# davawen/Simple-Raytracer

Hardware: AMD Instinct MI355X
Metric: Mray/s at 1920x1080x1024spp (higher is better)
Workload: dtype f32; 1 GPU; BASELINE configs[1]: 7-shape sphere scene 1920x1080 1024spp; width=1920, height=1080, spp=1024, bounces=10, triangles=12, partition=single GPU, gather=none, mode=parity (fp-contract off, IEEE div/sqrt; canvas bit-identical to the CPU oracle)

## Files before the change

include/srt_abi.h:

```cpp
#ifndef SRT_ABI_H
#define SRT_ABI_H

#include "srt_types.h"

#ifdef __cplusplus
extern "C" {
#endif

typedef struct srt_tracer srt_tracer;

enum {
	SRT_OK = 0,
	SRT_ERR_INVALID = 1,
	SRT_ERR_HIP = 2,
	SRT_ERR_STATE = 3
};

typedef struct srt_counters {
	uint64_t paths;
	uint64_t rays;
	uint64_t sky;
	uint64_t tri_tests;
	uint64_t tri_pass_u;
	uint64_t nan_pixels;
// ... 142 lines not shown
int srt_group_reset_denoise_history(srt_group *g);
int srt_group_resolve_denoised(srt_group *g, uint32_t ticks_stopped);
int srt_group_read_denoised(srt_group *g, float *rgba_out);
int srt_group_read_denoise_inputs(srt_group *g, float *normal_depth, float *albedo_hits, float *moments, uint32_t counts[2]);
int srt_group_read_denoise_history(srt_group *g, float *colour_count, float *moments, float *guide, srt_render_data *camera, int *valid);


int srt_render_pipelined(srt_tracer *t, const srt_render_data *options, uint32_t ticks_stopped, uint8_t *argb_out,
                         long long *frame_delivered);
int srt_pipeline_flush(srt_tracer *t, uint8_t *argb_out, long long *frame_delivered);



int srt_denoise_defaults(srt_denoise_params *out);
int srt_set_denoise(srt_tracer *t, const srt_denoise_params *params);
int srt_resolve_denoised(srt_tracer *t, uint32_t ticks_stopped);
int srt_read_denoised(srt_tracer *t, float *rgba_out);
int srt_read_denoise_inputs(srt_tracer *t, float *normal_depth, float *albedo_hits, float *moments, uint32_t counts[2]);



int srt_temporal_defaults(srt_temporal_params *out);
int srt_set_denoise_temporal(srt_tracer *t, const srt_temporal_params *params);
int srt_reset_denoise_history(srt_tracer *t);
int srt_read_denoise_history(srt_tracer *t, float *colour_count, float *moments, float *guide, srt_render_data *camera, int *valid);


enum { SRT_MOTION_STATIC = 0, SRT_MOTION_MOVED = 1, SRT_MOTION_NO_HISTORY = 2 };
#define SRT_MOTION_WORDS 22

int srt_set_denoise_object_motion(srt_tracer *t, int enable);
int srt_read_denoise_shape_ids(srt_tracer *t, uint32_t *current, uint32_t *history);
int srt_read_denoise_motion(srt_tracer *t, uint32_t *table, size_t capacity_shapes, size_t *n_shapes, int *any_moved);
int srt_motion_table_host(const srt_shape *h_shapes, size_t h_n_shapes, const srt_triangle *h_triangles, size_t h_n_triangles,
                          const srt_material *h_materials, size_t h_n_materials, const srt_scene_data *h_scene,
                          const srt_shape *c_shapes, size_t c_n_shapes, const srt_triangle *c_triangles, size_t c_n_triangles,
                          const srt_material *c_materials, size_t c_n_materials, const srt_scene_data *c_scene, uint32_t *table, int *keep);


enum { SRT_MOTION_DEFORMED = 3 };

int srt_set_denoise_vertex_motion(srt_tracer *t, int enable);
int srt_read_denoise_triangle_ids(srt_tracer *t, uint32_t *current, uint32_t *history);
int srt_read_denoise_vertex_tables(srt_tracer *t, float *current, float *history, size_t cap_rows, size_t *n_rows);
int srt_motion_table_deform_host(const srt_shape *h_shapes, size_t h_n_shapes, const srt_triangle *h_triangles, size_t h_n_triangles,
                                 const srt_material *h_materials, size_t h_n_materials, const srt_scene_data *h_scene,
                                 const srt_shape *c_shapes, size_t c_n_shapes, const srt_triangle *c_triangles, size_t c_n_triangles,
                                 const srt_material *c_materials, size_t c_n_materials, const srt_scene_data *c_scene, uint32_t *table, int *keep);


#define SRT_DEMOD_EPS 0.01f
int srt_set_denoise_demodulation(srt_tracer *t, int enable);
int srt_group_set_denoise_demodulation(srt_group *g, int enable);
int srt_last_filter_demodulated(const srt_tracer *t, int *demodulated);
int srt_group_last_filter_demodulated(const srt_group *g, int *demodulated);


int srt_set_denoise_spatial_variance(srt_tracer *t, uint32_t min_samples);
int srt_group_set_denoise_spatial_variance(srt_group *g, uint32_t min_samples);
int srt_last_filter_spatial_variance(const srt_tracer *t, int *ran);
int srt_group_last_filter_spatial_variance(const srt_group *g, int *ran);


int srt_set_denoise_history_illumination(srt_tracer *t, int enable);
int srt_group_set_denoise_history_illumination(srt_group *g, int enable);
int srt_last_setup_history_illumination(srt_tracer *t);
int srt_group_last_setup_history_illumination(srt_group *g);


int srt_set_denoise_history_clamp(srt_tracer *t, float gamma);
int srt_group_set_denoise_history_clamp(srt_group *g, float gamma);
int srt_last_setup_history_clamp(srt_tracer *t);
int srt_group_last_setup_history_clamp(srt_group *g);
int srt_read_denoise_history_bounds(srt_tracer *t, float *mean_weight, float *sigma_taps);


int srt_set_textures(srt_tracer *t, const srt_texture_desc *descs, size_t n);
int srt_set_material_textures(srt_tracer *t, const srt_material_texture *bindings, size_t n_materials);
int srt_set_triangle_uvs(srt_tracer *t, const float *uv, size_t n_triangles);
int srt_set_triangle_materials(srt_tracer *t, const int32_t *materials, size_t n_triangles);
int srt_triangle_materials_check_host(const int32_t *materials, size_t n, size_t scene_triangles, size_t n_materials);
int srt_last_trace_textured(const srt_tracer *t, int *textured);
int srt_last_trace_class(const srt_tracer *t, int *scene_class);
int srt_bernoulli_threshold_host(float p, uint64_t *threshold);
int srt_plane_frame_host(const float normal[3], float T[3], float B[3]);
int srt_texture_check_host(const srt_texture_desc *descs, size_t n_textures, const srt_material_texture *bindings, size_t n_bindings,
                           long long uv_triangles, size_t scene_triangles);

int srt_selftest_math(srt_tracer *t, uint32_t stride, uint64_t out[16]);

int srt_selftest_rare_lanes(srt_tracer *t, int what, const uint32_t *in, uint32_t waves, uint32_t *out_new, uint32_t *out_ref, uint64_t *mismatches);

const char *srt_version(void);

#ifdef __cplusplus
}
#endif

#endif
```

simple-raytracer_amd/csrc/device_intersect.h:

```cpp
#ifndef SRT_DEVICE_INTERSECT_H
#define SRT_DEVICE_INTERSECT_H

#include "device_math.h"
#include "trace_regions.h"

namespace {

#define SRT_AS_CONST __attribute__((address_space(4)))
struct Blk16 {
	float v[16];
};
struct Tri2 {
	float v[18];
};
template <int N, int ALIGN>
__device__ __forceinline__ void ld_uniform(const float *p, float (&out)[N]) {
	const SRT_AS_CONST float *c = (const SRT_AS_CONST float *)__builtin_assume_aligned(p, ALIGN);
#pragma unroll
	for (int i = 0; i < N; i++) out[i] = c[i];
}
__device__ __forceinline__ Blk16 ld_blk16(const float *p) {
	Blk16 b;
	ld_uniform<16, 64>(p, b.v);
	return b;
// ... 40 lines not shown
		for (int i = 0; i < N; i++) dd[i] = disc[i];
		sqrt_rsq_n<N, false>(dd, sq);
#pragma unroll
		for (int i = 0; i < N; i++) {
			const uint32_t k = min(dm_f2u(bq[i] - sq[i]), dm_f2u(bq[i] + sq[i]));
			take_if_closer(dm_u2f(k), idx0 + i, tmin, best);
		}
	}
}

__device__ __forceinline__ void test_planes2(const Blk16 &b, uint32_t count, f3 org, f3 dir, int idx0, float &tmin, int &best) {
#pragma unroll
	for (int i = 0; i < 2; i++) {
		if (i == 1 && count < 2u) break;
		f3 n = mk(b.v[8 * i + 4], b.v[8 * i + 5], b.v[8 * i + 6]);
		float denom = dot3(n, dir);
		float t = dot3(n, mk(b.v[8 * i] - org.x, b.v[8 * i + 1] - org.y, b.v[8 * i + 2] - org.z)) / denom;
		bool hit = !(t < 0.0f);
		if (hit && t < tmin) {
			tmin = t;
			best = idx0 + i;
		}
	}
}

template <int N>
__device__ __forceinline__ void test_spheres_cam(const float4 *__restrict__ cam, f3 dir, unsigned long long actm, int idx0, float &tmin, int &best) {
	float bq[4], disc[4];
	bool slow = is_neg_zero(tmin);
#pragma unroll
	for (int i = 0; i < N; i++) {
		const float4 lc = cam[i];
		bq[i] = dot3(mk(lc.x, lc.y, lc.z), dir);
		disc[i] = bq[i] * bq[i] - lc.w;
		slow = slow || dm_fabs(disc[i]) < 0x1p-96f;
	}
	if (__builtin_expect(any64(slow), 0)) {
#pragma unroll
		for (int i = 0; i < N; i++) {
			const float sq = __builtin_sqrtf(disc[i]);
			float t = bq[i] - sq;
			if (t < 0.0f) t = bq[i] + sq;
			if (!(disc[i] < 0.0f) && !(t < 0.0f) && t < tmin) tmin = t, best = idx0 + i;
		}
	} else {
#pragma unroll
		for (int i = 0; i < N; i++) {
			if ((ballot64(disc[i] >= 0.0f) & actm) != 0ull) {
				const float sq = sqrt_rsq(disc[i]);
				const uint32_t k = min(dm_f2u(bq[i] - sq), dm_f2u(bq[i] + sq));
				take_if_closer(dm_u2f(k), idx0 + i, tmin, best);
			}
		}
	}
}
__device__ __forceinline__ void test_planes2_cam(const float4 *__restrict__ blk, uint32_t count, f3 dir, int idx0, float &tmin, int &best) {
#pragma unroll
	for (int i = 0; i < 2; i++) {
		if (i == 1 && count < 2u) break;
		const float4 nq = blk[2 * i + 1];
		const float num = reinterpret_cast<const float *>(blk + 2 * i)[3];
		const float denom = dot3(mk(nq.x, nq.y, nq.z), dir);
		const float t = num / denom;
		const bool hit = !(t < 0.0f);
		if (hit && t < tmin) {
			tmin = t;
			best = idx0 + i;
		}
	}
}
template <uint32_t K>
__device__ __forceinline__ void cam_records_of_block(float4 *__restrict__ blk, float4 *__restrict__ cam, f3 org, int lane) {
	if constexpr ((K & 3u) == SRT_SHAPE_SPHERE + 1u) {
		if (lane < 4) {
			const float4 s = blk[lane];
			const f3 L = mk(s.x - org.x, s.y - org.y, s.z - org.z);
			const float c = dot3(L, L) - s.w;
			cam[lane] = make_float4(L.x, L.y, L.z, c);
		}
	} else if constexpr ((K & 3u) == SRT_SHAPE_PLANE + 1u) {
		if (lane < 2) {
			const float4 pq = blk[2 * lane], nq = blk[2 * lane + 1];
			reinterpret_cast<float *>(blk + 2 * lane)[3] = dot3(mk(nq.x, nq.y, nq.z), mk(pq.x - org.x, pq.y - org.y, pq.z - org.z));
		}
	}
}
__device__ __forceinline__ bool test_aabb(float lx, float ly, float lz, float hx, float hy, float hz, f3 org, f3 inv, float tmax) {
	float t0 = 0.0f, t1 = tmax;
	float a1 = (lx - org.x) * inv.x, a2 = (hx - org.x) * inv.x;
	t0 = dm_max(t0, dm_min(a1, a2));
	t1 = dm_min(t1, dm_max(a1, a2));
	a1 = (ly - org.y) * inv.y, a2 = (hy - org.y) * inv.y;
	t0 = dm_max(t0, dm_min(a1, a2));
	t1 = dm_min(t1, dm_max(a1, a2));
	a1 = (lz - org.z) * inv.z, a2 = (hz - org.z) * inv.z;
	t0 = dm_max(t0, dm_min(a1, a2));
	t1 = dm_min(t1, dm_max(a1, a2));
	return t0 < t1;
}

template <bool COUNT_TRIS>
__device__ __forceinline__ bool moller_trumbore(float v0x, float v0y, float v0z, float e1x, float e1y, float e1z, float e2x, float e2y,
                                                float e2z, f3 org, f3 dir, bool counted, float &t, uint32_t &n_tri_u SRT_RC_PARAM) {
	f3 e1 = mk(e1x, e1y, e1z), e2 = mk(e2x, e2y, e2z);
	f3 h = cross3(dir, e2);
	float a = dot3(e1, h);
	f3 sv = mk(org.x - v0x, org.y - v0y, org.z - v0z);
	float sh = dot3(sv, h);
	float aa = dm_fabs(a), ash = dm_fabs(sh);
	bool reject = (a == 0.0f) || (ash > aa * 1.001f) || ((sh * a < 0.0f) && (ash >= aa * 0.001f));
	bool ok = false;
	if (!reject) {
		SRT_REGION(EXTEND_TRI_EXACT);
		f3 q = cross3(sv, e1);
		float dv = dot3(dir, q);
		bool reject2 = false;
		if (!COUNT_TRIS) reject2 = ((dv * a < 0.0f) && (dm_fabs(dv) >= aa * 0.001f)) || (dm_fabs(sh + dv) > aa * 1.01f);
		if (!reject2) {
			SRT_REGION(EXTEND_TRI_DIV);
			float f = 1.0f / a;
			float u = f * sh;
			ok = !(u < 0.0f || u > 1.0f);
			if (COUNT_TRIS) n_tri_u += (ok && counted) ? 1u : 0u;
			float v = f * dv;
			ok = ok && !(v < 0.0f || u + v > 1.0f);
			t = f * dot3(e2, q);
			ok = ok && t > 0.0f;
		}
	}
	return ok;
}

template <bool COUNT_TRIS>
__device__ __forceinline__ void test_triangle(float v0x, float v0y, float v0z, float e1x, float e1y, float e1z, float e2x, float e2y,
                                              float e2z, f3 org, f3 dir, int idx, uint32_t j, uint32_t count, float &tmin, int &best,
                                              uint32_t &best_tri, uint32_t &n_tri_u SRT_RC_PARAM) {
	float t = 0.0f;
	if (moller_trumbore<COUNT_TRIS>(v0x, v0y, v0z, e1x, e1y, e1z, e2x, e2y, e2z, org, dir, j < count, t, n_tri_u SRT_RC_ARG) && t < tmin) {
		tmin = t;
		best = idx;
		best_tri = j;
	}
}


template <bool COUNT_TRIS>
__device__ __forceinline__ void test_pair(const Tri2 &t, f3 org, f3 dir, int idx, uint32_t j, uint32_t count, float &tmin, int &best,
                                          uint32_t &best_tri, uint32_t &n_tri_u SRT_RC_PARAM) {
	test_triangle<COUNT_TRIS>(t.v[0], t.v[1], t.v[2], t.v[3], t.v[4], t.v[5], t.v[6], t.v[7], t.v[8], org, dir, idx, j, count, tmin, best, best_tri,
	                          n_tri_u SRT_RC_ARG);
	test_triangle<COUNT_TRIS>(t.v[9], t.v[10], t.v[11], t.v[12], t.v[13], t.v[14], t.v[15], t.v[16], t.v[17], org, dir, idx, j + 1u, count, tmin,
	                          best, best_tri, n_tri_u SRT_RC_ARG);
}

template <bool COUNT_TRIS>
__device__ __forceinline__ void test_triangles(const float *__restrict__ wtris, uint32_t first, uint32_t count, f3 org, f3 dir, int idx,
                                               float &tmin, int &best, uint32_t &best_tri, uint32_t &n_tri_u SRT_RC_PARAM) {
	const float *__restrict__ blk = wtris + (size_t)first * SRT_WTRI_FLOATS;
	const uint32_t npair = ((count + 3u) >> 2) << 1;
	Tri2 a = ld_tri2(blk);
	for (uint32_t b = 0; b < npair; b += 2) {
		SRT_REGION(EXTEND_TRI_LOOP);
		const Tri2 c = ld_tri2(blk + 18u * (b + 1u));
		test_pair<COUNT_TRIS>(a, org, dir, idx, 2u * b, count, tmin, best, best_tri, n_tri_u SRT_RC_ARG);
		a = ld_tri2(blk + 18u * (b + 2u));
		test_pair<COUNT_TRIS>(c, org, dir, idx, 2u * b + 2u, count, tmin, best, best_tri, n_tri_u SRT_RC_ARG);
// ... 131 lines not shown
```

simple-raytracer_amd/csrc/device_types.h:

```cpp
#ifndef SRT_DEVICE_TYPES_H
#define SRT_DEVICE_TYPES_H

#include <stddef.h>
#include <stdint.h>

#include "../../include/srt_types.h"

struct ShapeRun {
	int32_t type;
	uint32_t first_shape;
	uint32_t count;
	uint32_t data_off;
};
struct BlockGroup {
	uint32_t code;
	uint32_t first[3];
};
static_assert(sizeof(BlockGroup) == 16, "BlockGroup 16 B");

struct WinnerRec {
	int32_t type;
	int32_t material;
	float vx, vy, vz, w;
	uint32_t first_wtri;
	float inv_w;
};
static_assert(sizeof(WinnerRec) == 32, "WinnerRec 32 B");

#define SRT_WTRI_FLOATS 9

typedef srt_bvh_node BvhNode;
#define SRT_BVH_FIRST_DWORD 11
#define SRT_BVH_TRI_FLOATS 9
#define SRT_BVH_LEAF_J 28
#define SRT_BVH_NONE 0xffffffffu
#define SRT_BVH_LEAF_BIT 0x80000000u
#define SRT_BVH_INDEX_MASK 0x0fffffffu
#define SRT_BVH_INDEX_MAX 0x01ffffffu
#define SRT_BVH_KEY_INF 0x7f800000u
#define SRT_BVH_TAG_MASK 31u
#define SRT_BVH_TAG_LEAF 16u
#define SRT_BVH_TAG(ref, slot) ((((ref) >> 31) << 4) | ((((ref) >> 28) & 3u) << 2) | (slot))
#define SRT_BVH_STACK_CAP 64
#ifndef SRT_BVH_LEAF_MAX
#define SRT_BVH_LEAF_MAX 3
#endif

#define SRT_REGION_MAX 56
#ifdef SRT_REGION_COUNT
#define SRT_WAVE_CTR_STRIDE (16 + 2 * SRT_REGION_MAX)
#else
#define SRT_WAVE_CTR_STRIDE 16
#endif
#define SRT_WAVE_CTR_SLOTS 8192

enum { SRT_CTR_RAYS = 0, SRT_CTR_SKY, SRT_CTR_TRI, SRT_CTR_TRI_PASS_U, SRT_CTR_NAN, SRT_CTR_PATHS, SRT_CTR_QUEUE, SRT_CTR_WATCHDOG, SRT_CTR_QUEUE2, SRT_CTR_COUNT };

#define SRT_MF_NO_SPECULAR 1
#define SRT_MF_PLAIN_COLORS 2

#define SRT_BLK_CODE(type, count) ((uint32_t)((type) + 1) | ((uint32_t)(count) << 2))
#define SRT_GROUP_CODE(b0, b1, b2) ((b0) | ((b1) << 8) | ((b2) << 16))
#define SRT_GC_PPS SRT_GROUP_CODE(SRT_BLK_CODE(SRT_SHAPE_PLANE, 2), SRT_BLK_CODE(SRT_SHAPE_PLANE, 1), SRT_BLK_CODE(SRT_SHAPE_SPHERE, 4))
#define SRT_GC_SSS SRT_GROUP_CODE(SRT_BLK_CODE(SRT_SHAPE_SPHERE, 4), SRT_BLK_CODE(SRT_SHAPE_SPHERE, 4), SRT_BLK_CODE(SRT_SHAPE_SPHERE, 4))
#define SRT_GC_PPP SRT_GROUP_CODE(SRT_BLK_CODE(SRT_SHAPE_PLANE, 2), SRT_BLK_CODE(SRT_SHAPE_PLANE, 2), SRT_BLK_CODE(SRT_SHAPE_PLANE, 2))
#define SRT_SCENE_CLASS_LIST(X) \
	X(1, SRT_GC_PPS, true)      \
	X(2, SRT_GC_PPS, false)     \
	X(3, SRT_GC_SSS, true)      \
	X(4, SRT_GC_PPP, true)
#define SRT_SCENE_CLASS_GENERAL 0
static constexpr inline uint32_t srt_class_cam_records(uint32_t code) {
	return ((code & 3u) == SRT_SHAPE_SPHERE + 1u ? 4u : 0u) + (((code >> 8) & 3u) == SRT_SHAPE_SPHERE + 1u ? 4u : 0u) +
	       (((code >> 16) & 3u) == SRT_SHAPE_SPHERE + 1u ? 4u : 0u);
}
static constexpr inline size_t srt_class_cam_lds_bytes(uint32_t code) { return 16u * (size_t)srt_class_cam_records(code); }

static inline size_t srt_scene_lds_bytes(size_t num_shapes, size_t num_materials, int num_models, size_t num_runs) {
	size_t scene = num_shapes * sizeof(WinnerRec) + num_materials * sizeof(srt_material);
	if (num_models == 0) scene += num_runs * (sizeof(BlockGroup) + 192);
	return scene <= 4608 ? scene : 0;
}

struct TraceParams {
	srt_render_data rd;
	srt_scene_data sd;
	const BlockGroup *runs;
	const float *run_data;
	const WinnerRec *winners;
	int32_t num_runs;
	int32_t num_materials;
	uint32_t lds_bytes;
	int32_t scene_class;
	const srt_shape *shapes;
	const srt_triangle *triangles;
	const srt_material *materials;
	const float *wtris;
	const float *sky;
	float *canvas;
	float *radiance;
	unsigned long long *counters;
	unsigned long long *wave_counters;
	unsigned long long *queue;
	unsigned long long total_items;
	uint32_t batch_samples;
	uint32_t first_sample;
	uint32_t job_items;
	uint32_t stage_off;
	int32_t sky_w, sky_h;
	float f_width, f_height, f_sky_w, f_sky_h;
	int32_t sun_focus_int;
	int32_t material_flags;
	int32_t num_models;
	int32_t rank, world, rows_per_block, owned_rows;
	int32_t use_bvh;
	const float *bvh_blocks;
	float *scan_queue;
	float inv_f_width, inv_f_height;
	uint32_t width_magic, width_shift;
	uint32_t rpb_magic, rpb_shift;
	uint32_t nbs_magic16;
	uint32_t pool_blocks;
	int32_t unit_materials;
	int32_t all_materials_ok;
};

static inline void srt_magic_u31(uint32_t d, uint32_t *magic, uint32_t *shift) {
	uint32_t l = 0;
	while (l < 32 && ((uint64_t)1 << l) < d) l++;
	*shift = l;
	*magic = (uint32_t)((((uint64_t)1 << 32) * (((uint64_t)1 << l) - d)) / d + 1);
}

struct PrepassParams {
	const srt_shape *shapes;
	const srt_triangle *triangles;
	const uint32_t *wtri_offset;
	float *wtris;
	int32_t num_shapes;
	uint32_t num_triangles;
	const uint32_t *order;
	const uint32_t *dest;
};

struct ReduceParams {
	const float *radiance;
	float *running;
	float *canvas;
	unsigned long long *counters;
	uint32_t num_pixels;
	uint32_t batch_samples;
	int32_t num_samples;
	uint32_t first_batch, last_batch;
	unsigned long long *queue_reset;
// ... 52 lines not shown
void srt_launch_features_ids_tex(const TexFeatureParams &p, uint32_t *shape_ids, void *stream);
void srt_launch_features_tris_tex(const TexFeatureParams &p, uint32_t *shape_ids, uint32_t *tri_ids, void *stream);

void srt_launch_trace(TraceParams p, bool count_triangles, int num_waves, void *stream);
void srt_launch_reduce(const ReduceParams &p, void *stream);
void srt_launch_reduce_moments(const ReduceParams &p, void *stream);
void srt_launch_features(const FeatureParams &p, void *stream);
void srt_launch_features_ids(const FeatureParams &p, uint32_t *shape_ids, void *stream);
void srt_launch_features_tris(const FeatureParams &p, uint32_t *shape_ids, uint32_t *tri_ids, void *stream);
int srt_trace_waves_per_simd(int has_models, int use_bvh);
int srt_trace_has_scene_classes();
int srt_trace_resident_waves_per_cu(const TraceParams &p, bool count_triangles);
int srt_scan_suspend_min(void);
int srt_sub_job_items(int has_models, int use_bvh);
#define SRT_SQ_CAP 192
#define SRT_PK_CAP 256
#define SRT_SCAN_QUEUE_FLOATS (2 * 20 * SRT_SQ_CAP + 15 * SRT_PK_CAP)
#define SRT_POOL_BLOCKS 8192
#define SRT_POOL_CTL_WORDS (16 + 2 * SRT_POOL_BLOCKS)
#define SRT_POOL_REC_FLOATS ((size_t)2 * SRT_POOL_BLOCKS * 20 * 64)
#define SRT_SCAN_SET_FLOATS(waves, pool) ((size_t)SRT_POOL_CTL_WORDS + ((pool) ? SRT_POOL_REC_FLOATS : (size_t)0) + (size_t)(waves) * SRT_SCAN_QUEUE_FLOATS)
void srt_launch_prepass(const PrepassParams &p, uint64_t total_wtris, void *stream);

struct RefitModel {
	uint32_t shape;
	uint32_t first_record;
	uint32_t num_records;
	uint32_t first_tile;
};
struct RefitCostRange {
	uint32_t first_block, num_blocks;
};
struct RefitParams {
	const srt_shape *shapes;
	const srt_triangle *triangles;
	const uint32_t *order, *dest;
	const RefitModel *models;
	uint32_t *extents;
	float *boxes;
	uint32_t *blocks;
	const uint32_t *sched;
};
#define SRT_REFIT_EXT_LO_INIT 0xff7fffffu
#define SRT_REFIT_EXT_HI_INIT 0x00800000u
int srt_launch_refit_extents(const RefitParams &p, uint32_t num_models, uint32_t max_records, void *stream);
int srt_launch_refit_leaves(const RefitParams &p, uint32_t num_models, uint32_t max_records, void *stream);
int srt_launch_refit_level(const RefitParams &p, uint32_t first, uint32_t count, void *stream);
int srt_launch_refit_cost(const float *boxes, const uint8_t *weights, const RefitCostRange *ranges, double *sums, uint32_t num_models, uint32_t max_blocks, void *stream);
#define SRT_BUILD_TILE 1024u
#define SRT_BUILD_SORT_PASSES 4
struct BuildParams {
	const srt_shape *shapes;
	const srt_triangle *triangles;
	const RefitModel *models;
	const uint32_t *extents;
	uint32_t *keys[2];
	uint32_t *vals[2];
	uint32_t *table;
	uint32_t *order;
	const uint32_t *range_first;
	uint32_t *ranges;
};
#define SRT_BUILD_TILES(records) (((uint32_t)(records) + SRT_BUILD_TILE - 1u) / SRT_BUILD_TILE)
int srt_launch_build_keys(const BuildParams &p, uint32_t num_models, uint32_t max_records, void *stream);
int srt_launch_build_sort(const BuildParams &p, uint32_t num_models, uint32_t max_records, void *stream);
#define SRT_BUILD_LOCAL 1024u
#define SRT_BUILD_MEDIAN_MAX_LEVELS 15u
#define SRT_BUILD_MEDIAN_KEY_BITS 17u
#ifdef __HIPCC__
#define SRT_BUILD_HD __host__ __device__
#else
#define SRT_BUILD_HD
#endif
static inline SRT_BUILD_HD uint32_t srt_build_median_levels(uint32_t n) {
	uint32_t levels = 0;
	while (levels <= SRT_BUILD_MEDIAN_MAX_LEVELS && n > (SRT_BUILD_LOCAL << levels)) levels++;
	return levels;
}
static inline SRT_BUILD_HD uint32_t srt_build_median_passes(uint32_t level) { return (SRT_BUILD_MEDIAN_KEY_BITS + level + 7u) / 8u; }
int srt_launch_build_median(const BuildParams &p, uint32_t num_models, uint32_t max_records, void *stream);
void srt_launch_resolve(const ResolveParams &p, void *stream);
void srt_launch_selftest(unsigned long long *out16, uint32_t stride, void *stream);
void srt_launch_selftest_rare(int what, const uint32_t *in, uint32_t waves, uint32_t *out_new, uint32_t *out_ref, unsigned long long *mismatches, void *stream);

#endif
```

simple-raytracer_amd/csrc/kernels.hip:

```cpp
#include <hip/hip_runtime.h>

#include "detmath.h"
#include "device_types.h"
#include "device_math.h"
#include "device_intersect.h"
#include "device_shading.h"

#if SRT_TEXTURED
#define SRT_TRACE_PARAMS TexTraceParams
#define SRT_FEATURE_PARAMS TexFeatureParams
#define srt_trace_kernel srt_trace_tex_kernel
#define srt_features_kernel srt_features_tex_kernel
#define srt_features_ids_kernel srt_features_ids_tex_kernel
#define srt_features_tris_kernel srt_features_tris_tex_kernel
#define srt_launch_trace srt_launch_trace_tex
#define srt_trace_resident_waves_per_cu srt_trace_tex_resident_waves_per_cu
#define srt_launch_features srt_launch_features_tex
#define srt_launch_features_ids srt_launch_features_ids_tex
#define srt_launch_features_tris srt_launch_features_tris_tex
int srt_trace_lds_floats(int has_models, int use_bvh);
#else
#define SRT_TRACE_PARAMS TraceParams
#define SRT_FEATURE_PARAMS FeatureParams
#endif
// ... 12 lines not shown
#endif
#ifndef SRT_HQ_CAP
#define SRT_HQ_CAP 64
#endif
#ifndef SRT_HQ_CAP_MODELS
#define SRT_HQ_CAP_MODELS 64
#endif
#ifndef SRT_SCAN_SUSPEND_MIN
#define SRT_SCAN_SUSPEND_MIN 128
#endif
#ifndef SRT_SCAN_FULL
#define SRT_SCAN_FULL 64
#endif
#ifndef SRT_HQ_CAP_BVH
#define SRT_HQ_CAP_BVH 64
#endif
#ifndef SRT_RING_CAP
#define SRT_RING_CAP 64
#endif
#ifndef SRT_REFILL_MIN
#define SRT_REFILL_MIN 32
#endif

#ifdef SRT_PHASE_CLOCK
#define SRT_CLK_DECL unsigned long long clk_t[8] = {0, 0, 0, 0, 0, 0, 0, 0}, clk_last = __builtin_amdgcn_s_memtime(), clk_start = clk_last
#define SRT_CLK(i)                                                  \
	do {                                                            \
		const unsigned long long now_ = __builtin_amdgcn_s_memtime(); \
		clk_t[i] += now_ - clk_last;                                \
		clk_last = now_;                                            \
	} while (0)
#else
#define SRT_CLK_DECL
#define SRT_CLK(i)
#endif

namespace {
__device__ __forceinline__ void store_radiance(float *__restrict__ radiance, uint32_t item, f3 c) {
	typedef float f3v __attribute__((ext_vector_type(3)));
	f3v v;
	v.x = c.x, v.y = c.y, v.z = c.z;
	float *g = radiance + 3ull * item;
	asm volatile("global_store_dwordx3 %0, %1, off sc1" : : "v"(g), "v"(v) : "memory");
}

__device__ __forceinline__ bool in_mask(unsigned long long m) { return __builtin_amdgcn_inverse_ballot_w64(m); }
__device__ __forceinline__ uint32_t popc64(unsigned long long m) { return (uint32_t)__builtin_popcountll(m); }
__device__ __forceinline__ uint32_t lane_rank(unsigned long long m) {
	return __builtin_amdgcn_mbcnt_hi((uint32_t)(m >> 32), __builtin_amdgcn_mbcnt_lo((uint32_t)m, 0u));
}
__device__ __forceinline__ unsigned long long lanes_below(uint32_t n) { return n >= 64u ? ~0ull : ((1ull << n) - 1ull); }

__device__ __forceinline__ void resolve_ring(const TraceParams &p, const float *__restrict__ ring, uint32_t n, int lane SRT_RC_PARAM) {
	asm volatile("s_waitcnt lgkmcnt(0)" ::: "memory");
	if ((uint32_t)lane < n) {
		SRT_REGION(SKY_RESOLVE);
		constexpr uint32_t RC = SRT_RING_CAP;
		const f3 d = mk(ring[0 * RC + lane], ring[1 * RC + lane], ring[2 * RC + lane]);
		f3 m = mk(ring[3 * RC + lane], ring[4 * RC + lane], ring[5 * RC + lane]);
		f3 c = mk(ring[6 * RC + lane], ring[7 * RC + lane], ring[8 * RC + lane]);
		const uint32_t item = dm_f2u(ring[9 * RC + lane]);
		m = m * sky_box(p, d);
		c = c + m;
		store_radiance(p.radiance, item, c);
	}
	asm volatile("" ::: "memory");
}
}

#ifndef SRT_TRACE_WAVES_PER_SIMD
#define SRT_TRACE_WAVES_PER_SIMD 5
#endif
#ifndef SRT_TRACE_WAVES_PER_SIMD_MODELS
#define SRT_TRACE_WAVES_PER_SIMD_MODELS 5
#endif
#ifndef SRT_TRACE_WAVES_PER_SIMD_BVH
#define SRT_TRACE_WAVES_PER_SIMD_BVH 5
#endif

constexpr uint32_t hq_fields(bool has_models) { return has_models ? 17u : 16u; }

struct GeneralScene {
	static constexpr bool FAST = false, NO_SPEC = false;
	static constexpr uint32_t CODE = 0;
};
template <uint32_t CODE_, bool NO_SPEC_>
struct OneGroupScene {
	static constexpr bool FAST = true, NO_SPEC = NO_SPEC_;
	static constexpr uint32_t CODE = CODE_;
};
template <uint32_t K>
__device__ __forceinline__ void test_block_of_class(const Blk16 &b, int base, f3 org, f3 dir, float &tmin, int &best) {
	if constexpr ((K & 3u) == SRT_SHAPE_SPHERE + 1u) {
		if constexpr (((K >> 2) & 7u) <= 2u) test_spheres<2>(b, org, dir, base, tmin, best);
		else test_spheres<4>(b, org, dir, base, tmin, best);
	} else if constexpr ((K & 3u) == SRT_SHAPE_PLANE + 1u) {
		test_planes2(b, (K >> 2) & 7u, org, dir, base, tmin, best);
	}
}
template <uint32_t K>
__device__ __forceinline__ void test_block_of_class_cam(const float4 *__restrict__ blk, const float4 *__restrict__ cam, int base, f3 dir, unsigned long long actm, float &tmin, int &best) {
	if constexpr ((K & 3u) == SRT_SHAPE_SPHERE + 1u) {
		if constexpr (((K >> 2) & 7u) <= 2u) test_spheres_cam<2>(cam, dir, actm, base, tmin, best);
		else test_spheres_cam<4>(cam, dir, actm, base, tmin, best);
	} else if constexpr ((K & 3u) == SRT_SHAPE_PLANE + 1u) {
		test_planes2_cam(blk, (K >> 2) & 7u, dir, base, tmin, best);
	}
}

template <bool COUNT_TRIS, bool USE_LDS, bool HAS_MODELS, bool USE_BVH>
__global__ __launch_bounds__(64, USE_BVH ? SRT_TRACE_WAVES_PER_SIMD_BVH : HAS_MODELS ? SRT_TRACE_WAVES_PER_SIMD_MODELS : SRT_TRACE_WAVES_PER_SIMD) void srt_trace_kernel(const SRT_TRACE_PARAMS p) {
	using SC = GeneralScene;
#include "trace_body.inc"
}

#if !SRT_TEXTURED && !SRT_DIAG_ON && !defined(SRT_DUMMY_KIND) && !defined(SRT_DEV_KNOBS) && SRT_RING_CAP == 64
#define SRT_SCENE_CLASSES 1
template <uint32_t CODE, bool NO_SPEC>
__global__ __launch_bounds__(64, 6) void srt_trace_scene_kernel(const TraceParams p) {
	constexpr bool COUNT_TRIS = false, USE_LDS = true, HAS_MODELS = false, USE_BVH = false;
	using SC = OneGroupScene<CODE, NO_SPEC>;
#include "trace_body.inc"
}
#else
#define SRT_SCENE_CLASSES 0
#endif

template <bool HAS_MODELS, bool USE_BVH>
__global__ __launch_bounds__(64) void srt_features_kernel(const SRT_FEATURE_PARAMS fp) {
#define SRT_FEATURES_IDS 0
#include "features_body.inc"
#undef SRT_FEATURES_IDS
}

template <bool HAS_MODELS, bool USE_BVH>
__global__ __launch_bounds__(64) void srt_features_ids_kernel(const SRT_FEATURE_PARAMS fp, uint32_t *__restrict__ shape_ids) {
#define SRT_FEATURES_IDS 1
#include "features_body.inc"
#undef SRT_FEATURES_IDS
}

template <bool HAS_MODELS, bool USE_BVH>
__global__ __launch_bounds__(64) void srt_features_tris_kernel(const SRT_FEATURE_PARAMS fp, uint32_t *__restrict__ shape_ids, uint32_t *__restrict__ tri_ids) {
#define SRT_FEATURES_IDS 2
#include "features_body.inc"
#undef SRT_FEATURES_IDS
}

#if !SRT_TEXTURED
int srt_trace_waves_per_simd(int has_models, int use_bvh) {
	return !has_models ? SRT_TRACE_WAVES_PER_SIMD : use_bvh ? SRT_TRACE_WAVES_PER_SIMD_BVH : SRT_TRACE_WAVES_PER_SIMD_MODELS;
}
int srt_scan_suspend_min(void) { return SRT_SCAN_SUSPEND_MIN; }
int srt_sub_job_items(int has_models, int use_bvh) { return !has_models ? SRT_SUB_PLAIN : use_bvh ? SRT_SUB_BVH : SRT_SUB_MODELS; }

int srt_trace_lds_floats(int has_models, int use_bvh) {
	int n = 10 * SRT_RING_CAP + (int)hq_fields(has_models) * (has_models ? (use_bvh ? SRT_HQ_CAP_BVH : SRT_HQ_CAP_MODELS) : SRT_HQ_CAP);
#ifdef SRT_REGION_COUNT
	n += 2 * SRT_REGION_MAX;
#endif
	return n;
}
int srt_trace_has_scene_classes() { return SRT_SCENE_CLASSES; }
#endif

namespace {
typedef void (*TraceKernel)(const SRT_TRACE_PARAMS);
TraceKernel pick_trace_kernel(bool models, bool use_bvh, bool use_lds, bool count_triangles) {
	if (!models) return use_lds ? srt_trace_kernel<false, true, false, false> : srt_trace_kernel<false, false, false, false>;
	if (use_bvh) {
		if (use_lds) return count_triangles ? srt_trace_kernel<true, true, true, true> : srt_trace_kernel<false, true, true, true>;
		return count_triangles ? srt_trace_kernel<true, false, true, true> : srt_trace_kernel<false, false, true, true>;
	}
	if (use_lds) return count_triangles ? srt_trace_kernel<true, true, true, false> : srt_trace_kernel<false, true, true, false>;
	return count_triangles ? srt_trace_kernel<true, false, true, false> : srt_trace_kernel<false, false, true, false>;
}
size_t scene_lds_bytes(const TraceParams &p) {
	return srt_scene_lds_bytes((size_t)p.sd.num_shapes, (size_t)p.num_materials, p.num_models, (size_t)p.num_runs);
}
TraceKernel pick_trace_kernel(const SRT_TRACE_PARAMS &p, bool use_lds, bool count_triangles) {
#if SRT_SCENE_CLASSES
	switch (p.scene_class) {
#define SRT_SCENE_CLASS_CASE(number, code, no_spec) \
	case number: return srt_trace_scene_kernel<code, no_spec>;
		SRT_SCENE_CLASS_LIST(SRT_SCENE_CLASS_CASE)
#undef SRT_SCENE_CLASS_CASE
	default: break;
	}
#endif
	return pick_trace_kernel(p.num_models > 0, p.use_bvh != 0, use_lds, count_triangles);
}
size_t trace_lds_bytes(const SRT_TRACE_PARAMS &p, size_t scene_lds) {
	size_t need = scene_lds + (size_t)srt_trace_lds_floats(p.num_models > 0, p.use_bvh) * sizeof(float);
#if SRT_SCENE_CLASSES
	switch (p.scene_class) {
#define SRT_SCENE_CLASS_CASE(number, code, no_spec) \
	case number: need += srt_class_cam_lds_bytes(code); break;
		SRT_SCENE_CLASS_LIST(SRT_SCENE_CLASS_CASE)
#undef SRT_SCENE_CLASS_CASE
	default: break;
	}
#endif
	return need;
}
}

int srt_trace_resident_waves_per_cu(const SRT_TRACE_PARAMS &p, bool count_triangles) {
	const size_t scene_lds = scene_lds_bytes(p);
	const size_t need = trace_lds_bytes(p, scene_lds);
	int blocks = 0;
	if (hipOccupancyMaxActiveBlocksPerMultiprocessor(&blocks, pick_trace_kernel(p, scene_lds != 0, count_triangles), 64, need) != hipSuccess ||
	    blocks <= 0) {
		(void)hipGetLastError();
		blocks = 4 * srt_trace_waves_per_simd(p.num_models > 0, p.use_bvh);
	}
	return blocks;
}

void srt_launch_trace(SRT_TRACE_PARAMS p, bool count_triangles, int num_waves, void *stream) {
	if (p.total_items == 0 || num_waves <= 0) return;
	dim3 grid((unsigned)num_waves), block(64);
	const size_t scene_lds = scene_lds_bytes(p);
	p.lds_bytes = (uint32_t)scene_lds;
	p.stage_off = (uint32_t)(scene_lds / sizeof(float4));
	const size_t need = trace_lds_bytes(p, scene_lds);
	hipLaunchKernelGGL(pick_trace_kernel(p, scene_lds != 0, count_triangles), grid, block, need, (hipStream_t)stream, p);
}

void srt_launch_features(const SRT_FEATURE_PARAMS &p, void *stream) {
	if (p.num_pixels == 0 || p.feature_samples == 0) return;
	typedef void (*FeatureKernel)(const SRT_FEATURE_PARAMS);
	const bool models = p.tp.num_models > 0, bvh = p.tp.use_bvh != 0;
	const FeatureKernel k = !models ? srt_features_kernel<false, false> : bvh ? srt_features_kernel<true, true> : srt_features_kernel<true, false>;
	hipLaunchKernelGGL(k, dim3((p.num_pixels + 63u) / 64u), dim3(64), 0, (hipStream_t)stream, p);
}

void srt_launch_features_ids(const SRT_FEATURE_PARAMS &p, uint32_t *shape_ids, void *stream) {
	if (p.num_pixels == 0 || p.feature_samples == 0) return;
	typedef void (*FeatureKernel)(const SRT_FEATURE_PARAMS, uint32_t *);
	const bool models = p.tp.num_models > 0, bvh = p.tp.use_bvh != 0;
	const FeatureKernel k = !models ? srt_features_ids_kernel<false, false> : bvh ? srt_features_ids_kernel<true, true> : srt_features_ids_kernel<true, false>;
	hipLaunchKernelGGL(k, dim3((p.num_pixels + 63u) / 64u), dim3(64), 0, (hipStream_t)stream, p, shape_ids);
}

void srt_launch_features_tris(const SRT_FEATURE_PARAMS &p, uint32_t *shape_ids, uint32_t *tri_ids, void *stream) {
	if (p.num_pixels == 0 || p.feature_samples == 0) return;
	typedef void (*FeatureKernel)(const SRT_FEATURE_PARAMS, uint32_t *, uint32_t *);
	const bool models = p.tp.num_models > 0, bvh = p.tp.use_bvh != 0;
	const FeatureKernel k = !models ? srt_features_tris_kernel<false, false> : bvh ? srt_features_tris_kernel<true, true> : srt_features_tris_kernel<true, false>;
	hipLaunchKernelGGL(k, dim3((p.num_pixels + 63u) / 64u), dim3(64), 0, (hipStream_t)stream, p, shape_ids, tri_ids);
}
```

simple-raytracer_amd/csrc/scene_prep.cpp:

```cpp
#include "scene_prep.h"

#include <algorithm>
#include <chrono>
#include <cmath>
#include <cstdio>
#include <cstring>
#include <deque>
#include <utility>

uint64_t bernoulli_threshold(float pr) {
	uint64_t lo = 0, hi = (uint64_t)1 << 32;
	while (lo < hi) {
		const uint64_t mid = (lo + hi) >> 1;
		const float u = (float)(uint32_t)mid * 2.3283064365386963e-10f;
		if (pr > u) lo = mid + 1;
		else hi = mid;
	}
	return lo;
}

int prepare_scene(const AccelPolicy &policy, BvhCache *&cache, int scan_suspend_min, std::string &err, ScenePrep &sp, const srt_shape *shapes, size_t n_shapes,
                  const srt_triangle *triangles, size_t n_triangles, const srt_material *materials, size_t n_materials, const srt_scene_data *scene) {
	auto fail = [&err](int code, const char *msg) {
		err = msg;
		return code;
	};
	if (!scene) return fail(SRT_ERR_INVALID, "srt_update_scene: scene is NULL");
	if ((n_shapes && !shapes) || (n_triangles && !triangles) || (n_materials && !materials))
		return fail(SRT_ERR_INVALID, "srt_update_scene: NULL array with non-zero count");
	if (n_shapes > 0x7fffffffu || n_triangles > 0xffffffffu) return fail(SRT_ERR_INVALID, "srt_update_scene: too many records");

	std::vector<ShapeRun> runs;
	std::vector<float> &data = sp.data;
	std::vector<WinnerRec> &winners = sp.winners;
	winners.assign(n_shapes ? n_shapes : 1, WinnerRec());
	std::vector<uint32_t> &offs = sp.offs;
	offs.assign(n_shapes ? n_shapes : 1, 0u);
	uint64_t &total_wtris = sp.total_wtris, &max_tris = sp.max_tris;
	int &num_models = sp.num_models;
	const bool use_bvh = sp.use_bvh = policy.accel == SRT_ACCEL_BVH;
	std::vector<uint32_t> &bvh_blocks = sp.bvh_blocks;
	std::vector<uint32_t> &bvh_order = sp.bvh_order, &bvh_dest = sp.bvh_dest;
	uint64_t bvh_leaves = 0, bvh_depth = 0, bvh_reused = 0, bvh_refitted = 0, bvh_canonical_nodes = 0;
	std::deque<BvhCacheEntry> fresh;
	std::vector<std::pair<bool, size_t>> plan;
	std::vector<std::pair<uint64_t, uint64_t>> range_hashes;
	std::vector<std::pair<const BvhCacheEntry *, uint32_t>> stale_plan;
	if (use_bvh && !cache) cache = new BvhCache();
	if (cache)
		for (BvhCacheEntry &e : cache->entries) e.claimed = false;
	if (!use_bvh && cache) cache->entries.clear();
	const auto build_t0 = std::chrono::steady_clock::now();
	auto range_hash = [&](const srt_model &m) {
		for (const auto &rh : range_hashes)
			if (rh.first == (((uint64_t)m.triangle_index << 32) | m.num_triangles)) return rh.second;
		const uint64_t th = hash_triangles(triangles + m.triangle_index, m.num_triangles);
		range_hashes.emplace_back(((uint64_t)m.triangle_index << 32) | m.num_triangles, th);
		return th;
	};
	auto find_same_triangles = [&](const srt_model &m, uint64_t th) {
		BvhCacheEntry *kept = nullptr;
		for (BvhCacheEntry &e : cache->entries) {
			if (e.claimed || e.count != m.num_triangles || e.tri_hash != th) continue;
			const bool exact = e.same_transform(m);
			if (!exact && kept) continue;
			if (!e.same_triangles(m, triangles, th)) continue;
			kept = &e;
			if (exact) break;
		}
		return kept;
	};
	const bool deform_on = use_bvh && policy.deform.mode == SRT_DEFORM_REFIT;
	struct Match {
		BvhCacheEntry *ent = nullptr;
		bool deformed = false;
	};
	std::vector<Match> matched;
	uint64_t deform_kept = 0, deform_rebuilt = 0;
	if (deform_on) {
		matched.assign(n_shapes, Match());
		auto wants_entry = [&](size_t i) {
			const srt_model &m = shapes[i].shape.model;
			return shapes[i].type == SRT_SHAPE_MODEL && m.num_triangles > 0 && (uint64_t)m.triangle_index + m.num_triangles <= n_triangles;
		};
		for (size_t i = 0; i < n_shapes; i++) {
			if (!wants_entry(i)) continue;
			const srt_model &m = shapes[i].shape.model;
			if ((matched[i].ent = find_same_triangles(m, range_hash(m)))) matched[i].ent->claimed = true;
		}
		for (size_t i = 0; i < n_shapes; i++) {
			if (!wants_entry(i) || matched[i].ent) continue;
			const srt_model &m = shapes[i].shape.model;
			BvhCacheEntry *kept = nullptr;
			for (BvhCacheEntry &e : cache->entries) {
				if (e.claimed || e.count != m.num_triangles || e.triangle_index != m.triangle_index) continue;
				if (!kept || e.same_transform(m)) kept = &e;
				if (e.same_transform(m)) break;
			}
			if (kept) kept->claimed = true, matched[i].ent = kept, matched[i].deformed = true;
		}
	}
// ... 89 lines not shown
						memcpy(ent->transform, m.transform, sizeof ent->transform);
						bvh_refitted++;
					}
					plan.emplace_back(true, (size_t)(kept - cache->entries.data()));
				} else {
					fresh.emplace_back();
					ent = &fresh.back();
					device_built = policy.build.mode == SRT_BUILD_DEVICE && m.num_triangles >= policy.build.min_triangles;
					if (device_built) *ent = cache->balanced_topology(m.num_triangles);
					else ent->build(m, triangles);
					ent->count = m.num_triangles;
					ent->triangle_index = m.triangle_index;
					ent->tri_hash = th;
					memcpy(ent->transform, m.transform, sizeof ent->transform);
					ent->tris.assign(triangles + m.triangle_index, triangles + m.triangle_index + m.num_triangles);
					plan.emplace_back(false, fresh.size() - 1);
				}
				const uint32_t b0 = (uint32_t)(bvh_blocks.size() / 32), r0 = (uint32_t)total_wtris;
				const BvhBuilder::Wide &wd = ent->wide;
				if ((uint64_t)b0 + wd.blocks.size() / 32 > SRT_BVH_INDEX_MAX) return fail(SRT_ERR_INVALID, "srt_update_scene: too many BVH blocks");
				if (wd.need > SRT_BVH_STACK_CAP) return fail(SRT_ERR_INVALID, "srt_update_scene: BVH deeper than the walk's stack");
				bvh_blocks.insert(bvh_blocks.end(), wd.blocks.begin(), wd.blocks.end());
				for (uint32_t ib : wd.inner) bvh_blocks[32 * (size_t)(b0 + ib) + SRT_BVH_FIRST_DWORD] += b0;
				bvh_dest.resize(r0 + (size_t)m.num_triangles);
				for (uint32_t r = 0; r < m.num_triangles; r++) bvh_dest[r0 + r] = wd.dest[r] + (b0 << 2);
				bvh_canonical_nodes += ent->nodes.size();
				bvh_order.insert(bvh_order.end(), ent->order.begin(), ent->order.end());
				link = wd.root == SRT_BVH_NONE ? SRT_BVH_NONE : wd.root + b0;
				if (ent->stale) {
					ent->wide.ensure_schedule();
					sp.refit_models.push_back({(uint32_t)i, r0, m.num_triangles, 0u});
					stale_plan.emplace_back(ent, b0);
					if (m.num_triangles > sp.refit_max_records) sp.refit_max_records = m.num_triangles;
					if (device_built) {
						sp.build_models.push_back({(uint32_t)i, r0, m.num_triangles, sp.build_tiles});
						sp.build_tiles += SRT_BUILD_TILES(m.num_triangles);
						sp.build_entry.push_back(plan.size() - 1);
						if (m.num_triangles > sp.build_max_records) sp.build_max_records = m.num_triangles;
					}
					if (deform_on) {
						const uint32_t nb = (uint32_t)(wd.blocks.size() / 32);
						sp.refit_cost_ranges.push_back({b0, nb});
						sp.refit_cost_entry.push_back(plan.size() - 1);
						sp.refit_cost_built.push_back(ent->cost_built);
						sp.refit_cost_fresh.push_back(device_built ? 1 : 0);
						sp.refit_weights.resize((size_t)b0 + nb, 0);
						for (const BvhBuilder::Wide::Job &j : wd.jobs) sp.refit_weights[b0 + j.self] = (uint8_t)j.nk;
						for (uint32_t d : wd.dest) sp.refit_weights[b0 + (d >> 2)]++;
					}
				} else if (deform_on) {
					sp.deform_worst_ratio = std::max(sp.deform_worst_ratio, BvhBuilder::cost_ratio(ent->cost_now, ent->cost_built));
				}
				bvh_leaves += ent->leaves;
				if (ent->depth > bvh_depth) bvh_depth = ent->depth;
			}
			data.insert(data.end(), {m.bounding_min.x, m.bounding_min.y, m.bounding_min.z, u2f(link), m.bounding_max.x, m.bounding_max.y,
			                         m.bounding_max.z, u2f(use_bvh ? 0u : m.num_triangles)});
			wr.first_wtri = (uint32_t)total_wtris;
			offs[i] = (uint32_t)total_wtris;
			total_wtris += use_bvh ? (uint64_t)m.num_triangles : (((uint64_t)m.num_triangles + 3u) & ~3ull);
			if (m.num_triangles > max_tris) max_tris = m.num_triangles;
			num_models++;
		}
	}
	pad_run();
	std::vector<BlockGroup> &groups = sp.groups;
	groups.assign((runs.size() + 2) / 3, BlockGroup());
	uint32_t n_big = 0;
	for (size_t b = 0; b < runs.size(); b++) {
		BlockGroup &g = groups[b / 3];
		if (b % 3 == 0) memset(&g, 0, sizeof g);
		const uint32_t big = runs[b].data_off >> 31;
		g.code |= (((uint32_t)runs[b].type + 1u) | (runs[b].count << 2) | (big << 5) | ((big ? (n_big++ & 1u) : 0u) << 6)) << (8 * (b % 3));
		g.first[b % 3] = runs[b].first_shape;
	}
	data.resize(groups.size() * 48 + 16, 0.0f);
	sp.one_group_code = 0;
	if (groups.size() == 1 && num_models == 0) {
		uint32_t next = 0;
		bool packed = true;
		for (size_t b = 0; b < runs.size(); b++) packed = packed && runs[b].first_shape == next, next += runs[b].count;
		if (packed && next == n_shapes) sp.one_group_code = groups[0].code;
	}
	if (!stale_plan.empty()) {
		size_t top = 0;
		for (const auto &st : stale_plan) top = std::max(top, st.first->wide.level_off.size());
		sp.refit_levels.assign(1, 0u);
		for (size_t h = 1; h < top; h++) {
			for (const auto &st : stale_plan) {
				const BvhBuilder::Wide &wd = st.first->wide;
				if (h >= wd.level_off.size()) continue;
				for (uint32_t k = wd.level_off[h - 1]; k < wd.level_off[h]; k++) sp.refit_sched.push_back(wd.sched[k] + st.second);
			}
			sp.refit_levels.push_back((uint32_t)sp.refit_sched.size());
		}
		for (size_t k = 0; k < sp.build_models.size(); k++)
			sp.build_extents.insert(sp.build_extents.end(), {SRT_REFIT_EXT_LO_INIT, SRT_REFIT_EXT_LO_INIT, SRT_REFIT_EXT_LO_INIT, SRT_REFIT_EXT_HI_INIT, SRT_REFIT_EXT_HI_INIT, SRT_REFIT_EXT_HI_INIT});
		for (size_t k = 0; k < stale_plan.size(); k++)
			sp.refit_extents.insert(sp.refit_extents.end(), {SRT_REFIT_EXT_LO_INIT, SRT_REFIT_EXT_LO_INIT, SRT_REFIT_EXT_LO_INIT, SRT_REFIT_EXT_HI_INIT, SRT_REFIT_EXT_HI_INIT, SRT_REFIT_EXT_HI_INIT});
	}
	const uint64_t build_us =
	    (uint64_t)std::chrono::duration_cast<std::chrono::microseconds>(std::chrono::steady_clock::now() - build_t0).count();

	std::vector<srt_material> &dev_mats = sp.dev_mats;
	dev_mats.assign(materials, materials + n_materials);
	auto schlick_r0 = [](float mu) {
		float r0 = (float)((1.0 - (double)mu) / (1.0 + (double)mu));
		return r0 * r0;
	};
	bool unit_materials = true;
	for (const auto &m : dev_mats)
		if (bernoulli_threshold(m.metallic) >> 32 || bernoulli_threshold(m.specular) >> 32 || bernoulli_threshold(m.transmittance) >> 32) unit_materials = false;
	sp.unit_materials = unit_materials;
	{
		bool no_specular = unit_materials, plain = true;
		for (const auto &m : dev_mats) {
			if (bernoulli_threshold(m.specular) != 0) no_specular = false;
			for (float c : {m.color.x, m.color.y, m.color.z})
				if (!std::isfinite(c) || (c == 0.0f && std::signbit(c))) plain = false;
		}
		sp.material_flags = (no_specular ? SRT_MF_NO_SPECULAR : 0) | (plain ? SRT_MF_PLAIN_COLORS : 0);
	}
	for (auto &m : dev_mats) {
		if (unit_materials) {
			const uint32_t tm = (uint32_t)bernoulli_threshold(m.metallic), ts = (uint32_t)bernoulli_threshold(m.specular), tt = (uint32_t)bernoulli_threshold(m.transmittance);
			memcpy(&m.metallic, &tm, 4), memcpy(&m.specular, &ts, 4), memcpy(&m.transmittance, &tt, 4);
		}
		const float inv_ior = 1.0f / m.refraction_index;
		m._pad[0] = inv_ior;
		m._pad[1] = schlick_r0(inv_ior);
		m.color._pad = schlick_r0(m.refraction_index);
	}
	sp.bvh_info[0] = bvh_canonical_nodes, sp.bvh_info[1] = bvh_leaves, sp.bvh_info[2] = bvh_depth, sp.bvh_info[3] = use_bvh ? build_us : 0;
	sp.bvh_info[4] = use_bvh ? plan.size() - bvh_reused - bvh_refitted : 0, sp.bvh_info[5] = bvh_reused, sp.bvh_info[6] = bvh_refitted;
	sp.deform_info[0] = deform_kept, sp.deform_info[1] = deform_rebuilt;
	if (deform_on) sp.refit_weights.resize(bvh_blocks.size() / 32, 0);
	if (use_bvh) {
		std::vector<BvhCacheEntry> next_cache;
		next_cache.reserve(plan.size());
		for (const auto &pl : plan) next_cache.push_back(std::move(pl.first ? cache->entries[pl.second] : fresh[pl.second]));
		cache->entries = std::move(next_cache);
	}
	sp.all_materials_ok = true;
	for (size_t i = 0; i < n_shapes; i++)
		if (shapes[i].material < 0) sp.all_materials_ok = false;
	return SRT_OK;
}

extern "C" int srt_bernoulli_threshold_host(float p, uint64_t *threshold_out) {
	if (!threshold_out) return SRT_ERR_INVALID;
	*threshold_out = bernoulli_threshold(p);
	return SRT_OK;
}
```

simple-raytracer_amd/csrc/scene_prep.h:

```cpp
#ifndef SRT_SCENE_PREP_H
#define SRT_SCENE_PREP_H

#include <string>
#include <vector>

#include "bvh_host.h"

struct ScenePrep {
	std::vector<BlockGroup> groups;
	std::vector<float> data;
	std::vector<WinnerRec> winners;
	std::vector<uint32_t> offs, bvh_blocks, bvh_order, bvh_dest;
	std::vector<srt_material> dev_mats;
	uint64_t total_wtris = 0, max_tris = 0;
	int num_models = 0;
	bool use_bvh = false, unit_materials = false, all_materials_ok = true;
	int material_flags = 0;
	uint32_t one_group_code = 0;
	uint64_t bvh_info[7] = {0, 0, 0, 0, 0, 0, 0};
	std::vector<RefitModel> refit_models;
	std::vector<uint32_t> refit_extents, refit_sched, refit_levels;
	uint32_t refit_max_records = 0;
	uint64_t deform_info[2] = {0, 0};
	std::vector<RefitCostRange> refit_cost_ranges;
	std::vector<uint8_t> refit_weights;
	std::vector<size_t> refit_cost_entry;
	std::vector<double> refit_cost_built;
	double deform_worst_ratio = 0.0;
	std::vector<uint8_t> refit_cost_fresh;
	std::vector<RefitModel> build_models;
	std::vector<uint32_t> build_extents;
	std::vector<size_t> build_entry;
	uint32_t build_max_records = 0, build_tiles = 0;
};

struct BuildPolicy {
	int mode = SRT_BUILD_HOST;
	uint32_t min_triangles = 0;
	int order = SRT_BUILD_ORDER_MORTON;
};

struct DeformPolicy {
	int mode = SRT_DEFORM_REBUILD;
	float rebuild_ratio = 0.0f;
};

struct AccelPolicy {
	int accel = SRT_ACCEL_NONE;
	int refit = SRT_REFIT_HOST;
	DeformPolicy deform;
	BuildPolicy build;
};

int prepare_scene(const AccelPolicy &policy, BvhCache *&cache, int scan_suspend_min, std::string &err, ScenePrep &sp, const srt_shape *shapes, size_t n_shapes,
                  const srt_triangle *triangles, size_t n_triangles, const srt_material *materials, size_t n_materials, const srt_scene_data *scene);

uint64_t bernoulli_threshold(float pr);

#endif
```

simple-raytracer_amd/csrc/selftest.hip:

```cpp
#include <hip/hip_runtime.h>

#include "device_math.h"
#include "device_shading.h"

namespace {
__device__ __forceinline__ bool same_float(float a, float b) { return (a != a && b != b) || dm_f2u(a) == dm_f2u(b); }
__device__ __forceinline__ unsigned long long canon_bits(float a) { return (a != a) ? 0x7fc00000ull : (unsigned long long)dm_f2u(a); }
__device__ __forceinline__ uint32_t mix32(uint32_t &h) {
	h = h * 747796405u + 2891336453u;
	uint32_t r = ((h >> ((h >> 28) + 4u)) ^ h) * 277803737u;
	return (r >> 22) ^ r;
}
__device__ __forceinline__ float rand_float_exp(uint32_t &h, uint32_t lo, uint32_t span) {
	const uint32_t m = mix32(h), e = lo + mix32(h) % span;
	return dm_u2f((m & 0x807fffffu) | (e << 23));
}
__device__ __forceinline__ bool same_f3(f3 a, f3 b) { return same_float(a.x, b.x) && same_float(a.y, b.y) && same_float(a.z, b.z); }
}

struct SelftestSizes {
	float w[8], inv_w[8];
};
__global__ __launch_bounds__(256) void srt_selftest_kernel(unsigned long long *out, uint32_t stride, const SelftestSizes sz) {
	unsigned long long bad_sqrt = 0, bad_log = 0, bad_cos = 0, s_log = 0, s_cos = 0, s_sqrt = 0, s_atan = 0, s_pow = 0;
	unsigned long long bad_div = 0, bad_norm = 0, bad_rn = 0, bad_fold = 0, bad_rsq = 0, bad_cam = 0, bad_sign = 0, bad_powi = 0;
	const int pw_n = 1 + (int)(blockIdx.x & 31u);
	const unsigned long long total = (0x100000000ull + stride - 1) / stride;
	for (unsigned long long i = blockIdx.x * (unsigned long long)blockDim.x + threadIdx.x; i < total;
	     i += (unsigned long long)gridDim.x * blockDim.x) {
		const uint32_t r = (uint32_t)(i * stride);
		const float asbits = dm_u2f(r);
		bad_sqrt += same_float(sqrt_ieee(asbits), __builtin_sqrtf(asbits)) ? 0 : 1;
		const float u = (float)r * 2.3283064365386963e-10f;
		const float lg = dm_logf(u);
		bad_log += same_float(log_unit(u), lg) ? 0 : 1;
		const float th = 6.28318548f * u;
		const float cs = dm_cosf(th);
		bad_cos += same_float(cos_2pi(th), cs) ? 0 : 1;
		s_log += canon_bits(lg);
		s_cos += canon_bits(cs);
		s_sqrt += canon_bits(dm_sqrtf(u));
		s_atan += canon_bits(dm_atan2pif(u - 0.5f, 0.37f - u));
		s_pow += canon_bits(dm_powf(u, 25.0f));
		const float cnt = (float)r;
		bad_fold += (same_float(log_count(cnt), log_unit(u)) && same_float((6.28318548f * 2.3283064365386963e-10f) * cnt, th)) ? 0 : 1;
		const float arg = -2.0f * lg;
		{
			float rho = sqrt_rsq_zero_ok(-2.0f * log_unit_biased<159, false>(cnt));
			rho = cnt == 0.0f ? DM_INF_F : rho;
			bad_rn += same_float(rho, __builtin_sqrtf(arg)) ? 0 : 1;
		}
		bad_sign += same_float(sign_fast(asbits), dm_sign(asbits)) ? 0 : 1;
		bad_powi += (same_float(powi_uniform(u, pw_n), dm_powi(u, pw_n)) && same_float(powi_uniform(-u, pw_n), dm_powi(-u, pw_n)) &&
		             same_float(powi_uniform(asbits, pw_n), dm_powi(asbits, pw_n)))
		                ? 0
		                : 1;
		if (r >= 0x0f800000u && r < 0x7f800000u) bad_rsq += same_float(sqrt_rsq(asbits), __builtin_sqrtf(asbits)) ? 0 : 1;
		{
			const float W = sz.w[r & 7u];
			const float a = (float)((r >> 3) % (uint32_t)W) + u;
			bad_cam += same_float(div_by_rcp(a, W, sz.inv_w[r & 7u]), a / W) ? 0 : 1;
		}
		uint32_t h = r ^ 0x9e3779b9u;
		f3 a = mk(rand_float_exp(h, 127 - 64, 118), rand_float_exp(h, 127 - 64, 118), rand_float_exp(h, 127 - 64, 118));
		if ((r & 15u) == 3u) a.x = 0.0f;
		if ((r & 31u) == 5u) a.y = -0.0f;
		if ((r & 0xfffu) == 7u) a.z = dm_u2f(mix32(h));
		float b = rand_float_exp(h, 127 - 44, 88);
		if ((r & 0xffffu) == 11u) b = dm_u2f(0x7fc00000u | (mix32(h) & 0x3fffffu));
		bad_div += same_f3(div3(a, b), a / b) ? 0 : 1;
		{
			const float ab = dm_fabs(b);
			const float y = (ab >= 0x1p-40f && ab <= 0x1p40f) ? 1.0f / b : 0.0f;
			bad_div += same_f3(div3_by_rcp(a, b, y), a / b) ? 0 : 1;
		}
		const f3 nv = normalize3(mk(u - 0.5f, 0.37f - u, (float)(r & 0xffffu) * 1e-3f - 30.0f));
		bad_norm += canon_bits(nv.x) + canon_bits(nv.y) + canon_bits(nv.z);
	}
	atomicAdd(&out[0], bad_sqrt);
	atomicAdd(&out[1], bad_log);
	atomicAdd(&out[2], bad_cos);
	atomicAdd(&out[3], s_log);
	atomicAdd(&out[4], s_cos);
	atomicAdd(&out[5], s_sqrt);
	atomicAdd(&out[6], s_atan);
	atomicAdd(&out[7], s_pow);
	atomicAdd(&out[8], bad_div);
	atomicAdd(&out[9], bad_norm);
	atomicAdd(&out[10], bad_rn);
	atomicAdd(&out[11], bad_fold);
	atomicAdd(&out[12], bad_rsq);
	atomicAdd(&out[13], bad_cam);
	atomicAdd(&out[14], bad_sign);
	atomicAdd(&out[15], bad_powi);
}

void srt_launch_selftest(unsigned long long *out, uint32_t stride, void *stream) {
	SelftestSizes sz;
	const float w[8] = {1920.f, 1080.f, 256.f, 3840.f, 2160.f, 960.f, 37.f, 16777216.f};
	for (int i = 0; i < 8; i++) sz.w[i] = w[i], sz.inv_w[i] = 1.0f / w[i];
	hipLaunchKernelGGL(srt_selftest_kernel, dim3(2048), dim3(256), 0, (hipStream_t)stream, out, stride, sz);
}

__global__ __launch_bounds__(64) void srt_selftest_rare_kernel(int what, const uint32_t *__restrict__ in, uint32_t *__restrict__ out_new,
                                                               uint32_t *__restrict__ out_ref, unsigned long long *mismatches) {
	const size_t lane = (size_t)blockIdx.x * 64u + threadIdx.x;
	const uint32_t *__restrict__ w = in + lane * 8u;
	f3 a = mk(0.0f, 0.0f, 0.0f), b = a;
	uint32_t ta = 0u, tb = 0u;
	if (what == 0) {
		uint32_t sa = w[0], sb = w[0];
		a = random_normal3(sa), b = random_normal3_lane(sb);
		ta = sa, tb = sb;
	} else {
		const f3 v = mk(dm_u2f(w[0]), dm_u2f(w[1]), dm_u2f(w[2]));
		const float d = dm_u2f(w[3]);
		a = mul_sign_wave(v, d), b = v * sign_fast(d);
	}
	const uint32_t ra[4] = {dm_f2u(a.x), dm_f2u(a.y), dm_f2u(a.z), ta}, rb[4] = {dm_f2u(b.x), dm_f2u(b.y), dm_f2u(b.z), tb};
	unsigned long long bad = 0;
#pragma unroll
	for (int k = 0; k < 4; k++) {
		out_new[lane * 4u + k] = ra[k], out_ref[lane * 4u + k] = rb[k];
		bad += ra[k] != rb[k] ? 1u : 0u;
	}
	if (bad) atomicAdd(mismatches, bad);
}

void srt_launch_selftest_rare(int what, const uint32_t *in, uint32_t waves, uint32_t *out_new, uint32_t *out_ref, unsigned long long *mismatches, void *stream) {
	if (waves == 0) return;
	hipLaunchKernelGGL(srt_selftest_rare_kernel, dim3(waves), dim3(64), 0, (hipStream_t)stream, what, in, out_new, out_ref, mismatches);
}
```

simple-raytracer_amd/csrc/srt_abi.hip:

```cpp
#include <hip/hip_runtime.h>

#include <cstdlib>
#include <cstring>
#include <new>
#include <string>
#include <vector>

#include "../../include/srt_abi.h"
#include "detmath.h"
#include "device_types.h"

#include "scene_prep.h"
#include "srt_internal.h"
#include "trace_plan.h"

namespace {

thread_local std::string g_create_error;

int num_blocks(int height, int rpb) { return (height + rpb - 1) / rpb; }

int clear_canvas_impl(srt_tracer *t) {
	const int rc = srt_temporal_commit(t);
	if (rc) return rc;
// ... 244 lines not shown

static int upload_scene_begin(srt_tracer *t, const ScenePrep &sp, const srt_shape *shapes, size_t n_shapes, const srt_triangle *triangles,
                              size_t n_triangles, size_t n_materials) {
	const std::vector<BlockGroup> &groups = sp.groups;
	const std::vector<float> &data = sp.data;
	const std::vector<WinnerRec> &winners = sp.winners;
	const std::vector<uint32_t> &offs = sp.offs, &bvh_blocks = sp.bvh_blocks, &bvh_order = sp.bvh_order, &bvh_dest = sp.bvh_dest;
	const std::vector<srt_material> &dev_mats = sp.dev_mats;
	const bool use_bvh = sp.use_bvh;
	const uint64_t total_wtris = sp.total_wtris, max_tris = sp.max_tris;
	const int num_models = sp.num_models;
	if (const int trc = srt_texture_check_scene(t, n_triangles, n_materials)) return trc;
	SRT_HIP(t, hipSetDevice(t->device));
	SRT_HIP(t, hipStreamSynchronize(t->stream));
	srt_texture_scene(t, shapes, n_shapes, n_triangles);
	SRT_HIP(t, t->shapes.reserve(n_shapes));
	SRT_HIP(t, t->runs.reserve(groups.size()));
	SRT_HIP(t, t->run_data.reserve(data.size()));
	SRT_HIP(t, t->winners.reserve(n_shapes));
	SRT_HIP(t, t->wtri_offset.reserve(n_shapes));
	SRT_HIP(t, t->triangles.reserve(n_triangles));
	SRT_HIP(t, t->materials.reserve(n_materials));
	if (use_bvh) {
		SRT_HIP(t, t->bvh_blocks.reserve(bvh_blocks.size()));
		SRT_HIP(t, t->bvh_order.reserve(bvh_order.size()));
		SRT_HIP(t, t->bvh_dest.reserve(bvh_dest.size()));
		if (!bvh_blocks.empty())
			SRT_HIP(t, hipMemcpyAsync(t->bvh_blocks.ptr, bvh_blocks.data(), bvh_blocks.size() * sizeof(uint32_t), hipMemcpyHostToDevice, t->stream));
		if (!bvh_order.empty()) {
			SRT_HIP(t, hipMemcpyAsync(t->bvh_order.ptr, bvh_order.data(), bvh_order.size() * sizeof(uint32_t), hipMemcpyHostToDevice, t->stream));
			SRT_HIP(t, hipMemcpyAsync(t->bvh_dest.ptr, bvh_dest.data(), bvh_dest.size() * sizeof(uint32_t), hipMemcpyHostToDevice, t->stream));
		}
	} else {
		SRT_HIP(t, t->wtris.reserve((size_t)total_wtris * SRT_WTRI_FLOATS + 64));
	}
	if (n_shapes) {
		SRT_HIP(t, hipMemcpyAsync(t->shapes.ptr, shapes, n_shapes * sizeof(srt_shape), hipMemcpyHostToDevice, t->stream));
		SRT_HIP(t, hipMemcpyAsync(t->winners.ptr, winners.data(), n_shapes * sizeof(WinnerRec), hipMemcpyHostToDevice, t->stream));
		SRT_HIP(t, hipMemcpyAsync(t->wtri_offset.ptr, offs.data(), n_shapes * sizeof(uint32_t), hipMemcpyHostToDevice, t->stream));
	}
	if (!groups.empty())
		SRT_HIP(t, hipMemcpyAsync(t->runs.ptr, groups.data(), groups.size() * sizeof(BlockGroup), hipMemcpyHostToDevice, t->stream));
	SRT_HIP(t, hipMemcpyAsync(t->run_data.ptr, data.data(), data.size() * sizeof(float), hipMemcpyHostToDevice, t->stream));
	if (n_triangles)
		SRT_HIP(t, hipMemcpyAsync(t->triangles.ptr, triangles, n_triangles * sizeof(srt_triangle), hipMemcpyHostToDevice, t->stream));
	if (n_materials)
		SRT_HIP(t, hipMemcpyAsync(t->materials.ptr, dev_mats.data(), n_materials * sizeof(srt_material), hipMemcpyHostToDevice, t->stream));

	if (const int brc = srt_accel_before_prepass(t, sp)) return brc;
	if (num_models > 0 && total_wtris > 0) {
		if (!use_bvh) SRT_HIP(t, hipMemsetAsync(t->wtris.ptr, 0, ((size_t)total_wtris * SRT_WTRI_FLOATS + 64) * sizeof(float), t->stream));
		for (size_t base = 0; base < n_shapes; base += 65535) {
			PrepassParams pp;
			pp.shapes = t->shapes.ptr + base;
			pp.triangles = t->triangles.ptr;
			pp.wtri_offset = t->wtri_offset.ptr + base;
			pp.wtris = use_bvh ? reinterpret_cast<float *>(t->bvh_blocks.ptr) : t->wtris.ptr;
			pp.order = use_bvh ? t->bvh_order.ptr : nullptr;
			pp.dest = use_bvh ? t->bvh_dest.ptr : nullptr;
			size_t cnt = n_shapes - base;
			pp.num_shapes = (int32_t)(cnt > 65535 ? 65535 : cnt);
			pp.num_triangles = (uint32_t)n_triangles;
			srt_launch_prepass(pp, max_tris, t->stream);
		}
		SRT_HIP(t, hipGetLastError());
	}
	return srt_accel_behind_prepass(t, sp);
}

static int upload_scene_end(srt_tracer *t, const ScenePrep &sp, size_t n_shapes, size_t n_materials, const srt_scene_data *scene) {
	SRT_HIP(t, hipSetDevice(t->device));
	SRT_HIP(t, hipStreamSynchronize(t->stream));
	t->sd = *scene;
	t->sd.num_shapes = (int32_t)n_shapes;
	t->num_models = sp.num_models;
	t->scan_tris = sp.use_bvh ? 0 : sp.total_wtris;
	t->bvh_active = sp.use_bvh && sp.num_models > 0;
	t->bvh_num_blocks = sp.use_bvh ? sp.bvh_blocks.size() / 32 : 0;
	for (int k = 0; k < 7; k++) t->bvh_info[k] = sp.bvh_info[k];
	t->all_materials_ok = sp.all_materials_ok;
	t->unit_materials = sp.unit_materials;
	t->material_flags = sp.material_flags;
	t->one_group_code = sp.one_group_code;
	t->num_runs = (int)sp.groups.size();
	t->num_materials = n_materials;
	t->scene_set = true;
	return srt_texture_sync(t);
}

static int prepare_scene_of(srt_tracer *t, ScenePrep &sp, const srt_shape *shapes, size_t n_shapes, const srt_triangle *triangles, size_t n_triangles,
                            const srt_material *materials, size_t n_materials, const srt_scene_data *scene) {
	std::string err;
	if (const int crc = srt_accel_deform_consume(t, t->bvh_cache)) return crc;
	if (const int brc = srt_accel_build_consume(t, t->bvh_cache)) return brc;
	const int rc = prepare_scene(t->policy, t->bvh_cache, srt_scan_suspend_min(), err, sp, shapes, n_shapes, triangles, n_triangles, materials, n_materials, scene);
	return rc == SRT_OK ? SRT_OK : fail(t, rc, err);
}

static int update_scene_impl(srt_tracer *t, const srt_shape *shapes, size_t n_shapes, const srt_triangle *triangles, size_t n_triangles,
                             const srt_material *materials, size_t n_materials, const srt_scene_data *scene) {
	if (!t) return SRT_ERR_INVALID;
	ScenePrep sp;
	int rc = prepare_scene_of(t, sp, shapes, n_shapes, triangles, n_triangles, materials, n_materials, scene);
	if (rc == SRT_OK) rc = upload_scene_begin(t, sp, shapes, n_shapes, triangles, n_triangles, n_materials);
	if (rc == SRT_OK) rc = upload_scene_end(t, sp, n_shapes, n_materials, scene);
	return rc;
}

int srt_update_scene_many(srt_tracer *const *members, size_t n_members, const srt_shape *shapes, size_t n_shapes, const srt_triangle *triangles,
                          size_t n_triangles, const srt_material *materials, size_t n_materials, const srt_scene_data *scene, size_t *failed_member) {
	if (failed_member) *failed_member = 0;
	if (!members || n_members == 0 || !members[0]) return SRT_ERR_INVALID;
	try {
		ScenePrep sp;
		int rc = prepare_scene_of(members[0], sp, shapes, n_shapes, triangles, n_triangles, materials, n_materials, scene);
		if (rc != SRT_OK) return rc;
		size_t begun = 0;
		for (; begun < n_members && rc == SRT_OK; begun++) {
			if (failed_member) *failed_member = begun;
			members[begun]->policy = members[0]->policy;
			rc = upload_scene_begin(members[begun], sp, shapes, n_shapes, triangles, n_triangles, n_materials);
		}
		if (rc != SRT_OK) {
			for (size_t i = 0; i + 1 < begun; i++) (void)upload_scene_end(members[i], sp, n_shapes, n_materials, scene);
			return rc;
		}
		for (size_t i = 0; i < n_members; i++) {
			if (failed_member) *failed_member = i;
			const int r = upload_scene_end(members[i], sp, n_shapes, n_materials, scene);
			if (r != SRT_OK && rc == SRT_OK) rc = r;
		}
		return rc;
	} catch (const std::bad_alloc &) {
		return fail(members[0], SRT_ERR_INVALID, "out of host memory");
	} catch (...) {
		return SRT_ERR_INVALID;
	}
}

int srt_clear_canvas(srt_tracer *t) {
	if (!t) return SRT_ERR_INVALID;
	SRT_HIP(t, hipSetDevice(t->device));
	return clear_canvas_impl(t);
}

static int scene_class(const srt_tracer *t, const srt_render_data *options, bool textured) {
	if (!srt_trace_has_scene_classes()) return SRT_SCENE_CLASS_GENERAL;
	if (!t->scene_set || t->num_models != 0 || t->num_runs != 1 || t->one_group_code == 0) return SRT_SCENE_CLASS_GENERAL;
	if (srt_scene_lds_bytes((size_t)t->sd.num_shapes, t->num_materials, 0, 1) == 0) return SRT_SCENE_CLASS_GENERAL;
	if (!t->all_materials_ok || !t->unit_materials) return SRT_SCENE_CLASS_GENERAL;
	if (options->num_bounces <= 0 || options->show_normals || textured || t->count_tris) return SRT_SCENE_CLASS_GENERAL;
	const bool no_spec = (t->material_flags & (SRT_MF_NO_SPECULAR | SRT_MF_PLAIN_COLORS)) == (SRT_MF_NO_SPECULAR | SRT_MF_PLAIN_COLORS);
#define SRT_SCENE_CLASS_MATCH(number, code, class_no_spec) \
	if (t->one_group_code == (code) && no_spec == class_no_spec) return number;
	SRT_SCENE_CLASS_LIST(SRT_SCENE_CLASS_MATCH)
#undef SRT_SCENE_CLASS_MATCH
	return SRT_SCENE_CLASS_GENERAL;
}

int srt_last_trace_class(const srt_tracer *t, int *scene_class_out) {
	if (!t || !scene_class_out) return SRT_ERR_INVALID;
	*scene_class_out = t->last_trace_class;
	return SRT_OK;
}

int srt_trace(srt_tracer *t, const srt_render_data *options) { return srt_trace_fused(t, options, nullptr, 0u); }


struct Dispatch {
	bool textured, timed, denoise;
	size_t pixels;
	int ns;
	uint8_t *fused_argb;
	uint32_t batch, n_batches;
	size_t radiance_stride;
	int slots;
	bool scan_queue;
	size_t scan_set_floats;
	uint32_t pool_blocks;
};

static int launch_resolve(srt_tracer *t, const float *canvas, uint32_t num_pixels, uint32_t ticks_stopped, uint8_t *argb) {
	ResolveParams rp;
	rp.canvas = canvas;
	rp.argb = argb;
	rp.num_steps = ticks_stopped;
	rp.num_pixels = num_pixels;
	srt_launch_resolve(rp, t->stream);
	SRT_HIP(t, hipGetLastError());
	return SRT_OK;
}

static TraceParams trace_params_of(const srt_tracer *t, const srt_render_data *options, bool textured) {
	TraceParams p;
	memset(&p, 0, sizeof p);
	p.rd = *options;
	if (t->scene_set) {
		p.sd = t->sd;
	} else {
		memset(&p.sd, 0, sizeof p.sd);
	}
	p.runs = t->runs.ptr;
	p.run_data = t->run_data.ptr;
	p.winners = t->winners.ptr;
	p.num_runs = t->scene_set ? t->num_runs : 0;
	p.num_materials = t->scene_set ? (int32_t)t->num_materials : 0;
	p.shapes = t->shapes.ptr;
	p.triangles = t->triangles.ptr;
	p.materials = t->materials.ptr;
	p.wtris = t->wtris.ptr;
	p.sky = t->sky.ptr;
	p.canvas = t->canvas;
	p.counters = t->counters.ptr;
	p.wave_counters = t->wave_counters.ptr;
	p.sky_w = t->sky_w;
	p.sky_h = t->sky_h;
	p.f_width = (float)options->width;
	p.f_height = (float)options->height;
	p.inv_f_width = 1.0f / p.f_width;
	p.inv_f_height = 1.0f / p.f_height;
	srt_magic_u31(options->width > 0 ? (uint32_t)options->width : 1u, &p.width_magic, &p.width_shift);
	srt_magic_u31(t->rows_per_block > 0 ? (uint32_t)t->rows_per_block : 1u, &p.rpb_magic, &p.rpb_shift);
	p.all_materials_ok = t->scene_set && t->all_materials_ok ? 1 : 0;
	p.unit_materials = t->scene_set && t->unit_materials ? 1 : 0;
	p.material_flags = t->scene_set ? t->material_flags : 0;
	p.scene_class = scene_class(t, options, textured);
	p.f_sky_w = (float)t->sky_w;
	p.f_sky_h = (float)t->sky_h;
	p.sun_focus_int = dm_pow_small_int(p.sd.sun_focus);
	p.num_models = t->num_models;
	p.use_bvh = t->bvh_active ? 1 : 0;
	p.bvh_blocks = reinterpret_cast<const float *>(t->bvh_blocks.ptr);
	p.rank = t->rank;
	p.world = t->world;
	p.rows_per_block = t->rows_per_block;
	p.owned_rows = t->owned_rows;
	return p;
}

static ReduceParams reduce_params_of(const srt_tracer *t, const Dispatch &d, uint32_t ticks_stopped) {
	ReduceParams rp;
	rp.radiance = t->radiance.ptr;
	rp.running = t->running.ptr;
	rp.canvas = t->canvas;
	rp.counters = t->counters.ptr;
	rp.num_pixels = (uint32_t)d.pixels;
	rp.num_samples = d.ns;
	rp.queue_reset = nullptr;
	rp.argb = nullptr;
	rp.num_steps = ticks_stopped;
	return rp;
}

static void launch_reduce(srt_tracer *t, ReduceParams &rp, bool denoise, uint8_t *argb) {
	if (denoise) {
		rp.moments = t->gd_on ? gd_moments(t) : t->dn_mom.ptr;
		srt_launch_reduce_moments(rp, t->stream);
	} else {
		rp.argb = argb;
		srt_launch_reduce(rp, t->stream);
	}
}

static int reserve_radiance(srt_tracer *t, Dispatch &d) {
	const size_t pixels = d.pixels;
	const int ns = d.ns;
	if (t->radiance_budget == 0) {
		size_t free_b = 0, total_b = 0;
		SRT_HIP(t, hipMemGetInfo(&free_b, &total_b));
		size_t budget = free_b / 2;
		const size_t cap = (size_t)96 << 30;
		if (budget > cap) budget = cap;
		if (t->radiance_budget_env) budget = t->radiance_budget_env;
		t->radiance_budget = budget;
	}
	const char *env_pairs = dev_env("SRT_SCAN_PAIRS");
	uint32_t batch = plan_batch(pixels, ns, t->radiance_budget, t->scan_tris, env_pairs ? atof(env_pairs) : 0.0, dev_int("SRT_FORCE_BATCH"));
	while (batch) {
		const size_t buffers = batch < (uint32_t)ns ? 2 : 1;
		hipError_t e = t->radiance.reserve(buffers * plan_radiance_stride(pixels, batch));
		if (e == hipSuccess) break;
		(void)hipGetLastError();
		if (e != hipErrorOutOfMemory || batch == 1)
			return fail(t, SRT_ERR_HIP, std::string("srt_trace: radiance buffer: ") + hipGetErrorString(e));
		batch = plan_batch_halved(batch);
		t->radiance_budget = pixels * 12 * (size_t)batch;
	}
	d.batch = batch;
	d.n_batches = plan_num_batches(ns, batch);
	d.radiance_stride = plan_radiance_stride(pixels, batch);
	if (d.n_batches > 1) SRT_HIP(t, t->running.reserve(pixels * 4));
	return SRT_OK;
}

static int wave_slots(srt_tracer *t, const TraceParams &p, bool textured) {
	int per_cu = textured ? srt_trace_tex_resident_waves_per_cu(srt_with_textures<TexTraceParams>(t, p), t->count_tris) : srt_trace_resident_waves_per_cu(p, t->count_tris);
	if (const char *env = dev_env("SRT_WAVES_PER_CU")) {
		const int v = atoi(env);
		if (v > 0 && v < per_cu) per_cu = v;
	}
	t->last_waves_per_cu = per_cu;
	const int slots = t->num_cus * per_cu;
	return slots > SRT_WAVE_CTR_SLOTS ? SRT_WAVE_CTR_SLOTS : slots;
}

static int reserve_scan_stacks(srt_tracer *t, Dispatch &d) {
	d.scan_queue = t->num_models > 0 && !t->bvh_active;
	const size_t scan_waves = plan_scan_waves(d.slots, d.pixels, d.batch);
	d.pool_blocks = d.scan_queue && !dev_env("SRT_NO_SCAN_POOL") ? (uint32_t)SRT_POOL_BLOCKS : 0u;
// ... 38 lines not shown
			int pr_low = 0, pr_high = 0;
			(void)hipDeviceGetStreamPriorityRange(&pr_low, &pr_high);
			const int pr = (k == 1 && pr_high < pr_low) ? pr_low - 1 : pr_low;
			SRT_HIP(t, hipStreamCreateWithPriority(&t->batch_stream[k], hipStreamNonBlocking, pr));
		}
		if (!t->ev_batch_traced[k]) SRT_HIP(t, hipEventCreateWithFlags(&t->ev_batch_traced[k], hipEventDisableTiming));
		if (!t->ev_batch_reduced[k]) SRT_HIP(t, hipEventCreateWithFlags(&t->ev_batch_reduced[k], hipEventDisableTiming));
	}
	if (!t->ev_batch_fork) SRT_HIP(t, hipEventCreateWithFlags(&t->ev_batch_fork, hipEventDisableTiming));
	SRT_HIP(t, hipEventRecord(t->ev_batch_fork, t->stream));
	for (int k = 0; k < 2; k++) SRT_HIP(t, hipStreamWaitEvent(t->batch_stream[k], t->ev_batch_fork, 0));
	return SRT_OK;
}

static int launch_batch(srt_tracer *t, const Dispatch &d, uint32_t b, TraceParams &p, ReduceParams &rp) {
	const bool overlap = d.n_batches > 1;
	const BatchSlice bs = plan_batch_slice(b, d.n_batches, d.pixels, d.ns, d.batch);
	const int par = bs.parity;
	hipStream_t ts = overlap ? t->batch_stream[par] : t->stream;
	p.radiance = t->radiance.ptr + (size_t)par * d.radiance_stride;
	p.queue = t->counters.ptr + (par ? SRT_CTR_QUEUE2 : SRT_CTR_QUEUE);
	p.wave_counters = t->wave_counters.ptr + (size_t)par * SRT_WAVE_CTR_SLOTS * SRT_WAVE_CTR_STRIDE;
	p.scan_queue = d.scan_queue ? t->scan_queue.ptr + (size_t)par * d.scan_set_floats : nullptr;
	p.pool_blocks = d.pool_blocks;
	if (overlap && b >= 2) SRT_HIP(t, hipStreamWaitEvent(ts, t->ev_batch_reduced[par], 0));
	p.batch_samples = bs.samples;
	p.first_sample = bs.first_sample;
	p.total_items = bs.total_items;
	const LaunchPlan lp = plan_launch(p.total_items, bs.samples, (unsigned long long)srt_sub_job_items(t->num_models > 0, t->bvh_active), t->num_cus, d.slots,
	                                  t->num_models > 0, t->bvh_active, dev_int("SRT_ITEMS_PER_WAVE"), dev_int("SRT_JOB_CAP_SUBS"));
	p.nbs_magic16 = lp.nbs_magic16;
	p.job_items = lp.job_items;
	if (t->queue_dirty[par]) SRT_HIP(t, hipMemsetAsync(p.queue, 0, sizeof(unsigned long long), ts));
	t->queue_dirty[par] = true;
	if (p.pool_blocks) SRT_HIP(t, hipMemsetAsync(p.scan_queue, 0, (size_t)SRT_POOL_CTL_WORDS * sizeof(uint32_t), ts));
	if (d.timed) SRT_HIP(t, hipEventRecord(t->ev_k[2 * b], ts));
	t->last_grid = lp.num_waves;
	if (d.textured) srt_launch_trace_tex(srt_with_textures<TexTraceParams>(t, p), t->count_tris, lp.num_waves, ts);
	else srt_launch_trace(p, t->count_tris, lp.num_waves, ts);
	SRT_HIP(t, hipGetLastError());
	if (d.timed) SRT_HIP(t, hipEventRecord(t->ev_k[2 * b + 1], ts));
	if (overlap) {
		SRT_HIP(t, hipEventRecord(t->ev_batch_traced[par], ts));
		SRT_HIP(t, hipStreamWaitEvent(t->stream, t->ev_batch_traced[par], 0));
	}
	t->ev_k_used = 2 * (size_t)(b + 1);
	rp.radiance = p.radiance;
	rp.batch_samples = bs.samples;
	rp.first_batch = (b == 0);
	rp.last_batch = (b == d.n_batches - 1);
	rp.queue_reset = p.queue;
	launch_reduce(t, rp, d.denoise, rp.last_batch ? d.fused_argb : nullptr);
	SRT_HIP(t, hipGetLastError());
	t->queue_dirty[par] = false;
	if (overlap) SRT_HIP(t, hipEventRecord(t->ev_batch_reduced[par], t->stream));
	return SRT_OK;
}

static int denoise_tail(srt_tracer *t, const Dispatch &d, const TraceParams &p, uint32_t ticks_stopped) {
	int rc = srt_denoise_after_trace(t, p, d.ns);
	if (rc == SRT_OK && d.fused_argb && t->dn_on) rc = srt_denoise_filter(t, ticks_stopped, d.fused_argb);
	if (rc) return rc;
	if (d.fused_argb && !t->dn_on) return launch_resolve(t, t->canvas, (uint32_t)d.pixels, ticks_stopped, d.fused_argb);
	return SRT_OK;
}

int srt_trace_fused(srt_tracer *t, const srt_render_data *options, uint8_t *fused_argb, uint32_t ticks_stopped) {
	if (!t) return SRT_ERR_INVALID;
	if (!options) return fail(t, SRT_ERR_INVALID, "srt_trace: options is NULL");
	if (options->width != t->width || options->height != t->height)
		return fail(t, SRT_ERR_INVALID, "srt_trace: options width/height differ from the handle's (no resize, tracer.hpp:61-66)");
	if (t->sky_w <= 0) return fail(t, SRT_ERR_STATE, "srt_trace: no skybox set (srt_set_skybox)");
	SRT_HIP(t, hipSetDevice(t->device));
	if (const int trc = srt_texture_sync(t)) return trc;
	Dispatch d{};
	d.textured = t->tex_active && !options->show_normals;
	t->last_trace_textured = d.textured;
	d.timed = !fused_argb || t->timers_in_render;
	d.denoise = t->dn_on || t->gd_on;
	d.pixels = owned_pixels(t);
	d.ns = options->num_samples;
	d.fused_argb = fused_argb;
	TraceParams p = trace_params_of(t, options, d.textured);
	t->last_trace_class = p.scene_class;
	if (const int rc = reserve_radiance(t, d)) return rc;
	d.slots = wave_slots(t, p, d.textured);
	if (const int rc = reserve_scan_stacks(t, d)) return rc;
	ReduceParams rp = reduce_params_of(t, d, ticks_stopped);
	if (const int rc = reserve_timer_events(t, d.n_batches)) return rc;
	t->ev_k_used = 0;
	if (d.timed) SRT_HIP(t, hipEventRecord(t->ev_t0, t->stream));
	if (d.n_batches == 0) {
		rp.batch_samples = 0;
		rp.first_batch = rp.last_batch = 1;
		launch_reduce(t, rp, d.denoise, fused_argb);
	}
	t->batches_overlapped = d.n_batches > 1;
	if (t->batches_overlapped)
		if (const int rc = fork_batch_streams(t)) return rc;
	for (uint32_t b = 0; b < d.n_batches; b++)
		if (const int rc = launch_batch(t, d, b, p, rp)) return rc;
	if (d.denoise)
		if (const int rc = denoise_tail(t, d, p, ticks_stopped)) return rc;
	if (d.timed) SRT_HIP(t, hipEventRecord(t->ev_t1, t->stream));
	t->have_trace_ev = d.timed;
	t->have_kernel_ev = d.timed && d.n_batches > 0;
	return SRT_OK;
}

static int resolve_impl(srt_tracer *t, const float *canvas, uint32_t num_pixels, uint32_t ticks_stopped, uint8_t *argb) {
	SRT_HIP(t, hipSetDevice(t->device));
	SRT_HIP(t, hipEventRecord(t->ev_r0, t->stream));
	if (const int rc = launch_resolve(t, canvas, num_pixels, ticks_stopped, argb)) return rc;
	SRT_HIP(t, hipEventRecord(t->ev_r1, t->stream));
	t->have_resolve_ev = true;
	return SRT_OK;
}

int srt_resolve(srt_tracer *t, uint32_t ticks_stopped) {
	if (!t) return SRT_ERR_INVALID;
	return resolve_impl(t, t->canvas, (uint32_t)owned_pixels(t), ticks_stopped, t->argb.ptr);
}

int srt_resolve_external(srt_tracer *t, const void *device_canvas, uint32_t num_pixels, uint32_t ticks_stopped,
                         void *device_argb) {
	if (!t) return SRT_ERR_INVALID;
	if (!device_canvas || !device_argb) return fail(t, SRT_ERR_INVALID, "srt_resolve_external: NULL buffer");
	return resolve_impl(t, static_cast<const float *>(device_canvas), num_pixels, ticks_stopped, static_cast<uint8_t *>(device_argb));
}

int srt_synchronize(srt_tracer *t) {
	if (!t) return SRT_ERR_INVALID;
	SRT_HIP(t, hipSetDevice(t->device));
	SRT_HIP(t, hipStreamSynchronize(t->stream));
	return SRT_OK;
}

int srt_render(srt_tracer *t, const srt_render_data *options, uint32_t ticks_stopped, uint8_t *argb_out) {
	if (!t) return SRT_ERR_INVALID;
	if (!argb_out) return fail(t, SRT_ERR_INVALID, "srt_render: argb_out is NULL");
	const int rc = srt_render_async(t, options, ticks_stopped, argb_out);
	if (rc) return rc;
	SRT_HIP(t, hipStreamSynchronize(t->stream));
	return SRT_OK;
}

int srt_render_async(srt_tracer *t, const srt_render_data *options, uint32_t ticks_stopped, uint8_t *argb_out) {
	if (!t) return SRT_ERR_INVALID;
	if (!argb_out) return fail(t, SRT_ERR_INVALID, "srt_render_async: argb_out is NULL");
	int rc = srt_trace_fused(t, options, t->argb.ptr, ticks_stopped);
	if (rc) return rc;
	t->have_resolve_ev = false;
	SRT_HIP(t, hipMemcpyAsync(argb_out, t->argb.ptr, owned_pixels(t) * 4, hipMemcpyDeviceToHost, t->stream));
	return SRT_OK;
}

int srt_read_canvas(srt_tracer *t, float *rgba_out) {
	if (!t) return SRT_ERR_INVALID;
	if (!rgba_out) return fail(t, SRT_ERR_INVALID, "srt_read_canvas: NULL");
	SRT_HIP(t, hipSetDevice(t->device));
	SRT_HIP(t, hipMemcpyAsync(rgba_out, t->canvas, owned_pixels(t) * 16, hipMemcpyDeviceToHost, t->stream));
	SRT_HIP(t, hipStreamSynchronize(t->stream));
	return SRT_OK;
}

int srt_read_argb(srt_tracer *t, uint8_t *argb_out) {
	if (!t) return SRT_ERR_INVALID;
// ... 126 lines not shown
}

int srt_bind_stream(srt_tracer *t, void *hip_stream) {
	if (!t) return SRT_ERR_INVALID;
	SRT_HIP(t, hipSetDevice(t->device));
	SRT_HIP(t, hipStreamSynchronize(t->stream));
	t->stream = hip_stream ? static_cast<hipStream_t>(hip_stream) : t->own_stream;
	return SRT_OK;
}

int srt_set_partition(srt_tracer *t, int rank, int world, int rows_per_block) {
	if (!t) return SRT_ERR_INVALID;
	if (world < 1 || rank < 0 || rank >= world || rows_per_block < 1)
		return fail(t, SRT_ERR_INVALID, "srt_set_partition: need 0 <= rank < world and rows_per_block >= 1");
	if (t->gd_on) return fail(t, SRT_ERR_STATE, "srt_set_partition: the handle's group has its denoiser on (srt_group_set_denoise(g, NULL) first)");
	if (world > 1 && t->tp_on) return fail(t, SRT_ERR_STATE, "srt_set_partition: temporal reprojection works on the full frame only (srt_set_denoise_temporal(t, NULL) first)");
	if (world > 1 && t->dn_on) return fail(t, SRT_ERR_STATE, "srt_set_partition: the denoiser works on the full frame only (srt_set_denoise(t, NULL) first)");
	SRT_HIP(t, hipSetDevice(t->device));
	SRT_HIP(t, hipStreamSynchronize(t->stream));
	const int padded = srt_partition_padded_rows(t->height, world, rows_per_block);
	const size_t need = (size_t)padded * t->width * 4;
	if (t->canvas == t->canvas_own.ptr) {
		SRT_HIP(t, t->canvas_own.reserve(need));
		t->canvas = t->canvas_own.ptr;
		t->canvas_bytes = t->canvas_own.cap * sizeof(float);
	} else if (t->canvas_bytes < need * sizeof(float)) {
		return fail(t, SRT_ERR_INVALID, "srt_set_partition: bound canvas too small for padded_rows*width*16");
	}
	SRT_HIP(t, t->argb.reserve((size_t)padded * t->width * 4));
	t->rank = rank;
	t->world = world;
	t->rows_per_block = rows_per_block;
	t->owned_rows = srt_partition_owned_rows(t->height, rank, world, rows_per_block);
	SRT_HIP(t, hipMemsetAsync(t->argb.ptr, 0, t->argb.cap, t->stream));
	return clear_canvas_impl(t);
}

int srt_selftest_math(srt_tracer *t, uint32_t stride, uint64_t out[16]) {
	if (!t) return SRT_ERR_INVALID;
	if (!out || stride == 0) return fail(t, SRT_ERR_INVALID, "srt_selftest_math: bad arguments");
	SRT_HIP(t, hipSetDevice(t->device));
	unsigned long long *d = nullptr;
	SRT_HIP(t, hipMalloc(reinterpret_cast<void **>(&d), 16 * sizeof(unsigned long long)));
	hipError_t e = hipMemsetAsync(d, 0, 16 * sizeof(unsigned long long), t->stream);
	if (e == hipSuccess) {
		srt_launch_selftest(d, stride, t->stream);
		e = hipGetLastError();
	}
	unsigned long long h[16] = {0};
	if (e == hipSuccess) e = hipMemcpyAsync(h, d, sizeof h, hipMemcpyDeviceToHost, t->stream);
	if (e == hipSuccess) e = hipStreamSynchronize(t->stream);
	(void)hipFree(d);
	if (e != hipSuccess) return fail(t, SRT_ERR_HIP, std::string("srt_selftest_math: ") + hipGetErrorString(e));
	for (int i = 0; i < 16; i++) out[i] = h[i];
	return SRT_OK;
}

int srt_selftest_rare_lanes(srt_tracer *t, int what, const uint32_t *in, uint32_t waves, uint32_t *out_new, uint32_t *out_ref, uint64_t *mismatches) {
	if (!t) return SRT_ERR_INVALID;
	if (!in || !out_new || !out_ref || !mismatches || what < 0 || what > 1 || waves == 0 || waves > 65536u)
		return fail(t, SRT_ERR_INVALID, "srt_selftest_rare_lanes: bad arguments");
	SRT_HIP(t, hipSetDevice(t->device));
	const size_t lanes = (size_t)waves * 64u, in_bytes = lanes * 8u * sizeof(uint32_t), out_bytes = lanes * 4u * sizeof(uint32_t);
	char *d = nullptr;
	SRT_HIP(t, hipMalloc(reinterpret_cast<void **>(&d), in_bytes + 2 * out_bytes + sizeof(unsigned long long)));
	uint32_t *d_in = reinterpret_cast<uint32_t *>(d), *d_new = reinterpret_cast<uint32_t *>(d + in_bytes), *d_ref = reinterpret_cast<uint32_t *>(d + in_bytes + out_bytes);
	unsigned long long *d_bad = reinterpret_cast<unsigned long long *>(d + in_bytes + 2 * out_bytes), h_bad = 0;
	hipError_t e = hipMemcpyAsync(d_in, in, in_bytes, hipMemcpyHostToDevice, t->stream);
	if (e == hipSuccess) e = hipMemsetAsync(d_new, 0, 2 * out_bytes + sizeof(unsigned long long), t->stream);
	if (e == hipSuccess) {
		srt_launch_selftest_rare(what, d_in, waves, d_new, d_ref, d_bad, t->stream);
		e = hipGetLastError();
	}
	if (e == hipSuccess) e = hipMemcpyAsync(out_new, d_new, out_bytes, hipMemcpyDeviceToHost, t->stream);
	if (e == hipSuccess) e = hipMemcpyAsync(out_ref, d_ref, out_bytes, hipMemcpyDeviceToHost, t->stream);
	if (e == hipSuccess) e = hipMemcpyAsync(&h_bad, d_bad, sizeof h_bad, hipMemcpyDeviceToHost, t->stream);
	if (e == hipSuccess) e = hipStreamSynchronize(t->stream);
	(void)hipFree(d);
	if (e != hipSuccess) return fail(t, SRT_ERR_HIP, std::string("srt_selftest_rare_lanes: ") + hipGetErrorString(e));
	*mismatches = h_bad;
	return SRT_OK;
}

int srt_debug_counters(srt_tracer *t, uint64_t out[18]) {
	if (!t || !out) return SRT_ERR_INVALID;
	SRT_HIP(t, hipSetDevice(t->device));
	std::vector<unsigned long long> w;
	if (const int rc = read_wave_counters(t, w, nullptr)) return rc;
	for (int k = 0; k < 18; k++) out[k] = 0;
	for (size_t i = 0; i < (size_t)2 * SRT_WAVE_CTR_SLOTS; i++) {
		for (int k = 0; k < 8; k++) out[k] += w[i * SRT_WAVE_CTR_STRIDE + k];
		for (int k = 8; k < 16; k++) out[k + 2] += w[i * SRT_WAVE_CTR_STRIDE + k];
	}
	out[8] = (uint64_t)t->last_waves_per_cu;
	out[9] = (uint64_t)t->last_grid;
	return SRT_OK;
}

int srt_debug_region_counters(srt_tracer *t, uint64_t *out, int capacity, int *written) {
	if (!t || !out || !written || capacity < 0) return SRT_ERR_INVALID;
	*written = 0;
#ifdef SRT_REGION_COUNT
	SRT_HIP(t, hipSetDevice(t->device));
	std::vector<unsigned long long> w;
	if (const int rc = read_wave_counters(t, w, nullptr)) return rc;
	const int n = capacity < 2 * SRT_REGION_MAX ? capacity : 2 * SRT_REGION_MAX;
	for (int k = 0; k < n; k++) out[k] = 0;
	for (size_t i = 0; i < (size_t)2 * SRT_WAVE_CTR_SLOTS; i++)
		for (int k = 0; k < n; k++) out[k] += w[i * SRT_WAVE_CTR_STRIDE + 16 + k];
	*written = n;
#endif
	return SRT_OK;
}

int srt_set_count_triangles(srt_tracer *t, int enable) {
	if (!t) return SRT_ERR_INVALID;
	t->count_tris = enable != 0;
	return SRT_OK;
}

}
```

simple-raytracer_amd/csrc/srt_internal.h:

```cpp
#ifndef SRT_INTERNAL_H
#define SRT_INTERNAL_H

#include <hip/hip_runtime.h>

#include <cstring>
#include <string>
#include <vector>

#include "../../include/srt_abi.h"
#include "device_types.h"
#include "scene_prep.h"

template <class T>
struct DevBuf {
	T *ptr = nullptr;
	size_t cap = 0;
	hipError_t reserve(size_t n) {
		if (n < 1) n = 1;
		if (n <= cap) return hipSuccess;
		if (ptr) (void)hipFree(ptr);
		ptr = nullptr;
		cap = 0;
		hipError_t e = hipMalloc(reinterpret_cast<void **>(&ptr), n * sizeof(T));
		if (e == hipSuccess) cap = n;
// ... 66 lines not shown
	DevBuf<float> refit_boxes;
	uint64_t refit_info[4] = {0, 0, 0, 0};
	TimedSpan refit_span;
	uint64_t deform_info[4] = {0, 0, 0, 0};
	DevBuf<RefitCostRange> deform_ranges;
	DevBuf<uint8_t> deform_weights;
	DevBuf<double> deform_sums;
	PinnedReadback<double> deform_sums_back;
	std::vector<size_t> deform_entry;
	std::vector<double> deform_built, deform_ratio;
	std::vector<uint8_t> deform_fresh;
	double deform_worst_host = 0.0;
	DevBuf<RefitModel> build_models;
	DevBuf<uint32_t> build_extents, build_keys[2], build_vals[2], build_table;
	DevBuf<uint32_t> build_ranges_dev;
	std::vector<uint32_t> build_ranges_host;
	uint64_t build_info[4] = {0, 0, 0, 0};
	PinnedReadback<uint32_t> build_order_back;
	std::vector<size_t> build_entry;
	std::vector<RefitModel> build_ranges;
	TimedSpan build_span;
	void release() {
		refit_models.release(), refit_extents.release(), refit_sched.release(), refit_boxes.release(), refit_span.release();
		deform_ranges.release(), deform_weights.release(), deform_sums.release(), deform_sums_back.release();
		build_models.release(), build_extents.release(), build_table.release(), build_ranges_dev.release();
		for (int k = 0; k < 2; k++) build_keys[k].release(), build_vals[k].release();
		build_order_back.release(), build_span.release();
	}
};

struct SrtCollect;

struct srt_tracer {
	int width = 0, height = 0, device = 0;
	SrtCollect *collect = nullptr;
	hipStream_t own_stream = nullptr, stream = nullptr;
	DevBuf<float> canvas_own;
	float *canvas = nullptr;
	size_t canvas_bytes = 0;
	DevBuf<uint8_t> argb;
	DevBuf<srt_shape> shapes;
	DevBuf<BlockGroup> runs;
	DevBuf<float> run_data;
	DevBuf<WinnerRec> winners;
	int num_runs = 0;
	size_t num_materials = 0;
	DevBuf<srt_triangle> triangles;
	DevBuf<srt_material> materials;
	DevBuf<float> wtris;
	DevBuf<uint32_t> wtri_offset;
	DevBuf<float> sky;
	DevBuf<uint32_t> bvh_blocks;
	DevBuf<uint32_t> bvh_order, bvh_dest;
	AccelPolicy policy;
	bool bvh_active = false;
	uint64_t bvh_info[7] = {0, 0, 0, 0, 0, 0, 0};
	size_t bvh_num_blocks = 0;
	AccelDevice upkeep;
	struct BvhCache *bvh_cache = nullptr;
	DevBuf<unsigned long long> counters;
	DevBuf<unsigned long long> wave_counters;
	DevBuf<float> scan_queue;
	DevBuf<float> radiance;
	DevBuf<float> running;
	size_t radiance_budget = 0;
	size_t radiance_budget_env = 0;
	int num_cus = 0;
	int last_waves_per_cu = 0, last_grid = 0;
	std::vector<hipEvent_t> ev_k;
	hipStream_t batch_stream[2] = {nullptr, nullptr};
	bool timers_in_render = false;
	bool queue_dirty[2] = {false, false};
	hipEvent_t ev_batch_traced[2] = {nullptr, nullptr}, ev_batch_reduced[2] = {nullptr, nullptr}, ev_batch_fork = nullptr;
	bool batches_overlapped = false;
	size_t ev_k_used = 0;
	float last_trace_kernel_ms = 0.f, last_reduce_ms = 0.f;
	int sky_w = 0, sky_h = 0;
	srt_scene_data sd{};
	int num_models = 0;
	bool all_materials_ok = false;
	bool unit_materials = false;
	int material_flags = 0;
	uint32_t one_group_code = 0;
	uint64_t scan_tris = 0;
	bool scene_set = false;
	bool count_tris = false;
	int rank = 0, world = 1, rows_per_block = 8, owned_rows = 0;
	bool dn_on = false;
	bool dn_filtered = false;
	srt_denoise_params dn{};
	uint32_t dn_T = 0, dn_P = 0, dn_F = 0;
	DevBuf<float> dn_nd, dn_ah, dn_mom;
	DevBuf<float> dn_guide;
	DevBuf<float> dn_col;
	int dn_out = 0;
	bool dn_demod = false;
	bool last_filter_demod = false;
	uint32_t dn_sv_min = 0;
	bool last_filter_sv = false;
	srt_render_data dn_cam{};
	bool tp_on = false;
	srt_temporal_params tp{};
	DevBuf<float> tp_set[2];
	int tp_cur = 0;
	bool tp_valid = false;
	bool tp_fresh = false;
	srt_render_data tp_cam{};
	bool tp_illum = false;
	bool last_setup_illum = false;
	float tp_clamp = 0.f;
	DevBuf<float> tp_bounds;
	bool tp_bounds_ran = false;
	bool last_setup_clamp = false;
	std::vector<uint8_t> scene_bytes;
	bool om_on = false;
	DevBuf<uint32_t> om_ids[2];
	int om_cur = 0;
	bool om_mixed = false;
	bool om_any_moved = false;
	std::vector<uint8_t> om_hist_scene;
	std::vector<uint32_t> om_table;
	DevBuf<uint32_t> om_table_dev;
	bool vm_on = false;
	bool om_any_deformed = false;
	DevBuf<uint32_t> vm_tri[2];
	DevBuf<float> vm_rows[2];
	std::vector<uint32_t> vm_first;
	DevBuf<uint32_t> vm_first_dev;
	uint64_t vm_scene_ver = 1, vm_ver[2] = {0, 0};
	bool gd_on = false;
	int gd_feature_samples = 0;
	DevBuf<float> gd_pack;
	float *gd_prev_canvas = nullptr;
	size_t gd_prev_bytes = 0;
	std::vector<TexDesc> tex_images;
	std::vector<srt_material_texture> tex_bindings;
	std::vector<float> tex_uv_host;
	bool tex_has_uvs = false;
	std::vector<int32_t> tex_tm_host;
	bool tex_has_tm = false;
	std::vector<PlaneFrame> tex_frames_host;
	size_t tex_scene_triangles = 0;
	DevBuf<float> tex_texels, tex_uvs;
	DevBuf<TexDesc> tex_descs;
	DevBuf<srt_material_texture> tex_bind_dev;
	DevBuf<PlaneFrame> tex_frames;
	DevBuf<int32_t> tex_tm;
	bool tex_dirty = false;
	bool tex_tm_active = false;
	bool tex_active = false;
	bool last_trace_textured = false;
	int last_trace_class = 0;
	hipEvent_t ev_t0 = nullptr, ev_t1 = nullptr, ev_r0 = nullptr, ev_r1 = nullptr;
	bool have_trace_ev = false, have_resolve_ev = false, have_kernel_ev = false;
	std::string err;
};

int srt_fail(srt_tracer *t, int code, const std::string &msg);
static inline int fail(srt_tracer *t, int code, const std::string &msg) { return srt_fail(t, code, msg); }
static inline size_t owned_pixels(const srt_tracer *t) { return (size_t)t->owned_rows * (size_t)t->width; }
static inline size_t full_pixels(const srt_tracer *t) { return (size_t)t->width * (size_t)t->height; }

static inline size_t gd_plane_pixels(int width, int height, int world, int rpb) { return (size_t)srt_partition_padded_rows(height, world, rpb) * (size_t)width; }
static inline size_t gd_slot_floats(size_t plane_pixels) { return 12 * plane_pixels + ((plane_pixels + 3) & ~(size_t)3); }
static inline float *gd_normal_depth(const srt_tracer *t) { return t->gd_pack.ptr + 4 * gd_plane_pixels(t->width, t->height, t->world, t->rows_per_block); }
static inline float *gd_albedo_hits(const srt_tracer *t) { return t->gd_pack.ptr + 8 * gd_plane_pixels(t->width, t->height, t->world, t->rows_per_block); }
static inline float *gd_moments(const srt_tracer *t) { return t->gd_pack.ptr + 12 * gd_plane_pixels(t->width, t->height, t->world, t->rows_per_block); }

#define SRT_HIP(t, call)                                                                              \
	do {                                                                                              \
		hipError_t e_ = (call);                                                                       \
		if (e_ != hipSuccess)                                                                         \
			return fail((t), SRT_ERR_HIP, std::string(#call) + ": " + hipGetErrorString(e_));         \
	} while (0)


void srt_collect_release(srt_tracer *t);
int srt_accel_deform_consume(srt_tracer *t, BvhCache *cache);
int srt_accel_build_consume(srt_tracer *t, BvhCache *cache);
int srt_accel_before_prepass(srt_tracer *t, const ScenePrep &sp);
int srt_accel_behind_prepass(srt_tracer *t, const ScenePrep &sp);
int srt_texture_check_scene(srt_tracer *t, size_t n_triangles, size_t n_materials);
void srt_texture_scene(srt_tracer *t, const srt_shape *shapes, size_t n_shapes, size_t n_triangles);
int srt_texture_sync(srt_tracer *t);
TexParams srt_texture_params(const srt_tracer *t);
void srt_texture_release(srt_tracer *t);
template <class Tex, class Base>
static inline Tex srt_with_textures(const srt_tracer *t, const Base &base) {
	Tex x;
	memset(&x, 0, sizeof x);
	static_cast<Base &>(x) = base;
	x.tx = srt_texture_params(t);
	return x;
}
int srt_denoise_clear(srt_tracer *t);
int srt_denoise_after_trace(srt_tracer *t, const TraceParams &p, int num_samples);
int srt_denoise_filter(srt_tracer *t, uint32_t ticks_stopped, uint8_t *argb);
void srt_denoise_count(srt_tracer *t, const srt_render_data &rd, int feature_samples);
int srt_denoise_member(srt_tracer *t, int feature_samples);
void srt_scene_bytes(std::vector<uint8_t> &bytes, const srt_shape *shapes, size_t n_shapes, const srt_triangle *triangles, size_t n_triangles,
                     const srt_material *materials, size_t n_materials, const srt_scene_data *scene);
struct TemporalStaged {
	const float4 *guide;
	const float4 *cc;
	const float2 *m;
};
int srt_temporal_setup(srt_tracer *t, float4 *col, uint32_t *argb, TemporalStaged *staged);
int srt_temporal_commit(srt_tracer *t);
void srt_temporal_drop(srt_tracer *t);
int srt_motion_update_scene(srt_tracer *t, const std::vector<uint8_t> &bytes, int rc);
int srt_vertex_table_sync(srt_tracer *t);
extern "C" int srt_trace_fused(srt_tracer *t, const srt_render_data *options, uint8_t *fused_argb, uint32_t ticks_stopped);
extern "C" int srt_update_scene_many(srt_tracer *const *members, size_t n_members, const srt_shape *shapes, size_t n_shapes, const srt_triangle *triangles,
                          size_t n_triangles, const srt_material *materials, size_t n_materials, const srt_scene_data *scene, size_t *failed_member);

#endif
```

simple-raytracer_amd/csrc/trace_body.inc:

```
	extern __shared__ float4 lds[];
	constexpr bool FAST = SC::FAST;
	static_assert(!FAST || (USE_LDS && !HAS_MODELS && !USE_BVH && !COUNT_TRIS), "scene classes exist for sphere / plane scenes staged in LDS");
	constexpr uint32_t FK0 = SC::CODE & 255u, FK1 = (SC::CODE >> 8) & 255u, FK2 = (SC::CODE >> 16) & 255u;
	constexpr int FN0 = (int)((FK0 >> 2) & 7u), FN1 = (int)((FK1 >> 2) & 7u), FN2 = (int)((FK2 >> 2) & 7u), FN = FN0 + FN1 + FN2;
	constexpr uint32_t SUB = USE_BVH ? SRT_SUB_BVH : HAS_MODELS ? SRT_SUB_MODELS : SRT_SUB_PLAIN;
	const int width = p.rd.width;
	const int lane = threadIdx.x;
	const int ns = p.rd.num_samples;
	const int nb = p.rd.num_bounces;
	const int n_shapes = FAST ? FN : p.sd.num_shapes;
	const bool all_materials_ok = FAST || p.all_materials_ok != 0;
	const bool unit_materials = FAST || p.unit_materials != 0;
	const bool no_specular = FAST ? SC::NO_SPEC : (p.material_flags & (SRT_MF_NO_SPECULAR | SRT_MF_PLAIN_COLORS)) == (SRT_MF_NO_SPECULAR | SRT_MF_PLAIN_COLORS);
	const BlockGroup *__restrict__ runs = p.runs;
	const float *__restrict__ run_data = p.run_data;
	const float *__restrict__ wtris = p.wtris;

	if (FAST) {
		const float4 *__restrict__ gw = reinterpret_cast<const float4 *>(p.winners);
		const float4 *__restrict__ gm = reinterpret_cast<const float4 *>(p.materials);
		const float4 *__restrict__ gd4 = reinterpret_cast<const float4 *>(p.run_data);
		static_assert(2 * FN <= 64, "one pass stages the winner records");
		if (lane < 2 * FN) lds[lane] = gw[lane];
		if (lane < 12) lds[2 * FN + lane] = gd4[lane];
		for (int i = threadIdx.x; i < 4 * p.num_materials; i += 64) lds[2 * FN + 12 + i] = gm[i];
		__syncthreads();
	} else if (USE_LDS) {
		const float4 *__restrict__ gw = reinterpret_cast<const float4 *>(p.winners);
		const float4 *__restrict__ gm = reinterpret_cast<const float4 *>(p.materials);
		for (int i = threadIdx.x; i < 2 * n_shapes; i += 64) lds[i] = gw[i];
		for (int i = threadIdx.x; i < 4 * p.num_materials; i += 64) lds[2 * n_shapes + i] = gm[i];
		if (!HAS_MODELS) {
			const float4 *__restrict__ gh4 = reinterpret_cast<const float4 *>(p.runs);
			const float4 *__restrict__ gd4 = reinterpret_cast<const float4 *>(p.run_data);
			float4 *__restrict__ dst = lds + 2 * n_shapes + 4 * p.num_materials;
			for (int i = threadIdx.x; i < p.num_runs; i += 64) dst[i] = gh4[i];
			for (int i = threadIdx.x; i < 12 * p.num_runs; i += 64) dst[p.num_runs + i] = gd4[i];
		}
		__syncthreads();
	}
	uint32_t gh_code = 0;
	int gh_f0 = 0, gh_f1 = 0, gh_f2 = 0;
	if (!FAST && USE_LDS && !HAS_MODELS && p.num_runs > 0) {
		const float4 hv = lds[2 * n_shapes + 4 * p.num_materials];
		gh_code = (uint32_t)__builtin_amdgcn_readfirstlane((int)f2u(hv.x));
		gh_f0 = __builtin_amdgcn_readfirstlane((int)f2u(hv.y)), gh_f1 = __builtin_amdgcn_readfirstlane((int)f2u(hv.z));
		gh_f2 = __builtin_amdgcn_readfirstlane((int)f2u(hv.w));
	}

	const uint32_t total_items = (uint32_t)p.total_items;
	const uint32_t nbs = p.batch_samples;
	const unsigned long long own_chunks_end = (unsigned long long)gridDim.x * p.job_items;
	uint32_t chunk_cur = 0, chunk_end = 0;
	if ((unsigned long long)blockIdx.x * p.job_items < (unsigned long long)total_items) {
		chunk_cur = blockIdx.x * p.job_items;
		chunk_end = (total_items - chunk_cur < p.job_items) ? total_items : chunk_cur + p.job_items;
	}
	bool queue_dry = (total_items == 0);
	uint32_t sj_next = 0, sj_end = 0, sj_off = 0, sj_qpix = 0;
	float *__restrict__ ring = reinterpret_cast<float *>(lds + p.stage_off);
	float *__restrict__ hq = ring + 10u * (uint32_t)SRT_RING_CAP;
	constexpr uint32_t HQ = USE_BVH ? SRT_HQ_CAP_BVH : HAS_MODELS ? SRT_HQ_CAP_MODELS : SRT_HQ_CAP;
	constexpr uint32_t CS1 = srt_class_cam_records(FK0), CS2 = srt_class_cam_records(FK0 | (FK1 << 8));
	float4 *__restrict__ cam_rec = reinterpret_cast<float4 *>(hq + hq_fields(HAS_MODELS) * HQ);
	if (FAST) {
		const auto &c = SRT_COLD(p);
		const f3 cam_org = mk(c.rd.camera_to_world[3].x, c.rd.camera_to_world[3].y, c.rd.camera_to_world[3].z);
		cam_records_of_block<FK0>(lds + 2 * FN, cam_rec, cam_org, lane);
		cam_records_of_block<FK1>(lds + 2 * FN + 4, cam_rec + CS1, cam_org, lane);
		cam_records_of_block<FK2>(lds + 2 * FN + 8, cam_rec + CS2, cam_org, lane);
		__syncthreads();
	}
	bool cam_phase = false;
	unsigned long long w_cam = 0;
#ifdef SRT_REGION_COUNT
	uint32_t *region_ctr = reinterpret_cast<uint32_t *>(hq + hq_fields(HAS_MODELS) * HQ);
	for (int i = lane; i < 2 * SRT_REGION_MAX; i += 64) region_ctr[i] = 0u;
	__syncthreads();
#endif
	constexpr bool SUSPEND = HAS_MODELS && !USE_BVH;
	constexpr uint32_t SQ = (uint32_t)SRT_SQ_CAP, PK = (uint32_t)SRT_PK_CAP;
	float *__restrict__ sq_base = SUSPEND ? const_cast<float *>((const float *)SRT_COLD(p).scan_queue) + (size_t)SRT_POOL_CTL_WORDS + (SRT_COLD(p).pool_blocks != 0u ? SRT_POOL_REC_FLOATS : (size_t)0) + (size_t)blockIdx.x * (size_t)SRT_SCAN_QUEUE_FLOATS : nullptr;
	float *__restrict__ pk = sq_base + 2u * 20u * SQ;
	uint32_t sq_count0 = 0, sq_count1 = 0, pk_count = 0;
	const bool use_pool = SUSPEND && SRT_COLD(p).pool_blocks != 0u;
	bool pool_leave = false, pool_last = false;
	uint32_t w_pool_taken = 0, w_pool_given = 0, w_pool_last_taken = 0;
	uint32_t ring_count = 0, hq_head = 0, hq_count = 0;

	f3 org = mk(0.f, 0.f, 0.f), dir = mk(0.f, 0.f, 0.f), mask = mk(1.f, 1.f, 1.f), color = mk(0.f, 0.f, 0.f);
	uint32_t seed = 0;
	uint32_t item = 0;
	int bounce = 0;
	int best = -1;
	uint32_t best_tri = 0;
	BvhStackEntry bvh_stack[USE_BVH ? SRT_BVH_STACK_CAP + 1 : 1];
	const float4 *__restrict__ bvh_blocks = reinterpret_cast<const float4 *>(p.bvh_blocks);
	unsigned long long actm = 0ull;
	unsigned long long resm = 0ull;
	float tmin = DM_INF_F;
	uint32_t pos = 0;
	unsigned long long w_rays = 0;
	uint32_t w_sky = 0, w_paths = 0, w_iter = 0, w_shade = 0;
	uint32_t w_scans = 0, w_scan_lanes = 0;
	uint32_t n_tri = 0, n_tri_u = 0;
	uint32_t idle_spins = 0;
	constexpr uint32_t SHADE_THR = ((uint32_t)SRT_SHADE_MIN - 1u) < HQ ? ((uint32_t)SRT_SHADE_MIN - 1u) : HQ;
	uint32_t shade_thr = queue_dry ? 0u : SHADE_THR;

	SRT_CLK_DECL;
	SRT_REGION(PROLOGUE);
	for (;;) {
		SRT_REGION(LOOP_HEAD);
		unsigned long long hitm = 0ull, missm = 0ull, finm = 0ull;
		uint32_t susp = 0u;
		int key = -1;
		if (SRT_DIAG_ON) w_iter++;
		SRT_CLK(6);
#ifdef SRT_DUMMY_KIND
#include "issue_probe.h"
#endif
		if (actm != 0ull) {
			constexpr bool MASKED = HAS_MODELS;
			if (!FAST && nb <= 0) {
				finm = actm;
			} else {
				w_rays += SUSPEND ? popc64(actm & ~resm) : popc64(actm);
				const bool resumed = SUSPEND ? in_mask(resm) : false;
				if (!MASKED || in_mask(actm)) {
					SRT_REGION(EXTEND_SETUP);
					{
						if (!SUSPEND || !resumed) {
							tmin = DM_INF_F;
							best = -1;
							best_tri = 0;
							pos = 0;
						}
						bool part = true;
						uint32_t sq_pushed0 = 0, sq_pushed1 = 0;
						f3 inv = mk(0.f, 0.f, 0.f);
						if (HAS_MODELS) inv = mk(1.0f / dir.x, 1.0f / dir.y, 1.0f / dir.z);

					auto test_block = [&](const Blk16 &b, uint32_t code, int base, uint32_t bidx, int slot) {
						const uint32_t type1 = code & 3u;
						const bool on = !SUSPEND || (part && bidx >= pos);
						if (type1 == SRT_SHAPE_SPHERE + 1u) {
							if (on) {
								if (((code >> 2) & 7u) <= 2u) {
									SRT_REGION_SLOT(EXTEND_SPHERES2, slot);
									test_spheres<2>(b, org, dir, base, tmin, best);
								} else {
									SRT_REGION_SLOT(EXTEND_SPHERES4, slot);
									test_spheres<4>(b, org, dir, base, tmin, best);
								}
							}
						} else if (type1 == SRT_SHAPE_PLANE + 1u) {
							if (on) {
								SRT_REGION_SLOT(EXTEND_PLANES, slot);
								test_planes2(b, (code >> 2) & 7u, org, dir, base, tmin, best);
							}
						} else if (HAS_MODELS && type1 == SRT_SHAPE_MODEL + 1u) {
							SRT_REGION_SLOT(EXTEND_MODEL, slot);
							const bool enter0 = on && test_aabb(b.v[0], b.v[1], b.v[2], b.v[4], b.v[5], b.v[6], org, inv, tmin);
							bool scan0 = enter0;
							if (SUSPEND && ((code >> 5) & 1u)) {
								const unsigned long long want = ballot64(enter0);
								const uint32_t n_want = (uint32_t)__popcll(want);
								const uint32_t sid = (code >> 6) & 1u;
								const uint32_t held = sid ? sq_count1 + sq_pushed1 : sq_count0 + sq_pushed0;
								const bool now = held + n_want > SQ || any64(enter0 && resumed && pos == bidx);
								if (!now) {
									if (enter0) {
										SRT_REGION(EXTEND_SUSPEND);
										float *__restrict__ sq = sq_base + sid * (20u * SQ);
										const uint32_t e = held + __builtin_amdgcn_mbcnt_hi((uint32_t)(want >> 32), __builtin_amdgcn_mbcnt_lo((uint32_t)want, 0u));
										sq[0 * SQ + e] = org.x, sq[1 * SQ + e] = org.y, sq[2 * SQ + e] = org.z;
										sq[3 * SQ + e] = dir.x, sq[4 * SQ + e] = dir.y, sq[5 * SQ + e] = dir.z;
										sq[6 * SQ + e] = mask.x, sq[7 * SQ + e] = mask.y, sq[8 * SQ + e] = mask.z;
										sq[9 * SQ + e] = color.x, sq[10 * SQ + e] = color.y, sq[11 * SQ + e] = color.z;
										sq[12 * SQ + e] = dm_u2f(seed), sq[13 * SQ + e] = dm_u2f((uint32_t)bounce), sq[14 * SQ + e] = dm_u2f(item);
										sq[15 * SQ + e] = tmin, sq[16 * SQ + e] = dm_u2f((uint32_t)best), sq[17 * SQ + e] = dm_u2f(best_tri);
										sq[18 * SQ + e] = dm_u2f(bidx);
										part = false;
										susp = 1u + sid;
									}
									if (sid) sq_pushed1 += n_want;
									else sq_pushed0 += n_want;
									scan0 = false;
								}
							}
							if (SUSPEND && !COUNT_TRIS && ((code >> 5) & 1u)) {
								const unsigned long long sb = ballot64(scan0);
								if (scan0) {
									w_scan_lanes++;
									if ((sb & ((1ull << lane) - 1ull)) == 0ull) w_scans++;
								}
							}
							if (scan0) {
								if (USE_BVH) {
									walk_bvh<COUNT_TRIS>(bvh_blocks, bvh_stack, f2u(b.v[3]), org, dir, base, tmin, best, best_tri, n_tri, n_tri_u SRT_RC_ARG);
								} else {
									if (COUNT_TRIS) n_tri += f2u(b.v[7]);
									test_triangles<COUNT_TRIS>(wtris, f2u(b.v[3]), f2u(b.v[7]), org, dir, base, tmin, best, best_tri, n_tri_u SRT_RC_ARG);
								}
							}
							if (((code >> 2) & 7u) > 1u && on && test_aabb(b.v[8], b.v[9], b.v[10], b.v[12], b.v[13], b.v[14], org, inv, tmin)) {
								if (USE_BVH) {
									walk_bvh<COUNT_TRIS>(bvh_blocks, bvh_stack, f2u(b.v[11]), org, dir, base + 1, tmin, best, best_tri, n_tri, n_tri_u SRT_RC_ARG);
								} else {
									if (COUNT_TRIS) n_tri += f2u(b.v[15]);
									test_triangles<COUNT_TRIS>(wtris, f2u(b.v[11]), f2u(b.v[15]), org, dir, base + 1, tmin, best, best_tri, n_tri_u SRT_RC_ARG);
								}
							}
						}
					};
					const int n_groups = FAST ? 0 : p.num_runs;
					if (FAST) {
						const float4 *__restrict__ lb = lds + 2 * FN;
						auto ld_lds = [&](int k) {
							Blk16 b;
							const float4 q0 = lb[4 * k], q1 = lb[4 * k + 1], q2 = lb[4 * k + 2], q3 = lb[4 * k + 3];
							b.v[0] = q0.x, b.v[1] = q0.y, b.v[2] = q0.z, b.v[3] = q0.w, b.v[4] = q1.x, b.v[5] = q1.y, b.v[6] = q1.z, b.v[7] = q1.w;
							b.v[8] = q2.x, b.v[9] = q2.y, b.v[10] = q2.z, b.v[11] = q2.w, b.v[12] = q3.x, b.v[13] = q3.y, b.v[14] = q3.z, b.v[15] = q3.w;
							return b;
						};
						if (cam_phase) {
							w_cam += (1ull << 36) + popc64(actm);
							test_block_of_class_cam<FK0>(lb, cam_rec, 0, dir, actm, tmin, best);
							if (FK1 != 0u) test_block_of_class_cam<FK1>(lb + 4, cam_rec + CS1, FN0, dir, actm, tmin, best);
							if (FK2 != 0u) test_block_of_class_cam<FK2>(lb + 8, cam_rec + CS2, FN0 + FN1, dir, actm, tmin, best);
						} else {
							test_block_of_class<FK0>(ld_lds(0), 0, org, dir, tmin, best);
							if (FK1 != 0u) test_block_of_class<FK1>(ld_lds(1), FN0, org, dir, tmin, best);
							if (FK2 != 0u) test_block_of_class<FK2>(ld_lds(2), FN0 + FN1, org, dir, tmin, best);
						}
					}
					for (int g = 0; g < n_groups; g++) {
						SRT_REGION(EXTEND_GROUP);
						float gh[4];
						ld_uniform<4, 16>(reinterpret_cast<const float *>(runs + g), gh);
						const uint32_t code = f2u(gh[0]);
						const float *__restrict__ gd = run_data + 48 * g;
						if (!HAS_MODELS && USE_LDS) {
							const float4 *__restrict__ lgh = lds + 2 * n_shapes + 4 * p.num_materials;
							const float4 *__restrict__ lb = lgh + n_groups + 12 * g;
							const uint32_t lcode = gh_code;
							const int f0 = gh_f0, f1 = gh_f1, f2 = gh_f2;
							auto ld_lds = [&](int k) {
								Blk16 b;
								const float4 q0 = lb[4 * k], q1 = lb[4 * k + 1], q2 = lb[4 * k + 2], q3 = lb[4 * k + 3];
								b.v[0] = q0.x, b.v[1] = q0.y, b.v[2] = q0.z, b.v[3] = q0.w, b.v[4] = q1.x, b.v[5] = q1.y, b.v[6] = q1.z, b.v[7] = q1.w;
								b.v[8] = q2.x, b.v[9] = q2.y, b.v[10] = q2.z, b.v[11] = q2.w, b.v[12] = q3.x, b.v[13] = q3.y, b.v[14] = q3.z, b.v[15] = q3.w;
								return b;
							};
							test_block(ld_lds(0), lcode & 255u, f0, 0u, 0);
							if ((lcode >> 8) & 255u) test_block(ld_lds(1), (lcode >> 8) & 255u, f1, 0u, 1);
							if ((lcode >> 16) & 255u) test_block(ld_lds(2), (lcode >> 16) & 255u, f2, 0u, 2);
							int ng = n_groups;
							asm volatile("" : "+s"(ng));
							if (ng > 1) {
								const float4 hv = lgh[g + 1 < n_groups ? g + 1 : 0];
								gh_code = (uint32_t)__builtin_amdgcn_readfirstlane((int)f2u(hv.x));
								gh_f0 = __builtin_amdgcn_readfirstlane((int)f2u(hv.y)), gh_f1 = __builtin_amdgcn_readfirstlane((int)f2u(hv.z));
								gh_f2 = __builtin_amdgcn_readfirstlane((int)f2u(hv.w));
							}
						} else if (!HAS_MODELS) {
							const Blk16 b0 = ld_blk16(gd), b1 = ld_blk16(gd + 16), b2 = ld_blk16(gd + 32);
							test_block(b0, code & 255u, (int)f2u(gh[1]), 0u, 0);
							test_block(b1, (code >> 8) & 255u, (int)f2u(gh[2]), 0u, 1);
							test_block(b2, (code >> 16) & 255u, (int)f2u(gh[3]), 0u, 2);
						} else {
							test_block(ld_blk16(gd), code & 255u, (int)f2u(gh[1]), 3u * g, 0);
							if ((code >> 8) & 255u) test_block(ld_blk16(gd + 16), (code >> 8) & 255u, (int)f2u(gh[2]), 3u * g + 1u, 1);
							if ((code >> 16) & 255u) test_block(ld_blk16(gd + 32), (code >> 16) & 255u, (int)f2u(gh[3]), 3u * g + 2u, 2);
						}
					}
					SRT_REGION(EXTEND_FINISH);
						if (!SUSPEND || part) {
							key = best;
							if (!all_materials_ok) {
								key = -1;
								if (best >= 0) key = USE_LDS ? (int)f2u(reinterpret_cast<const float *>(lds)[8 * best + 1]) : p.winners[best].material;
							}
							if (!MASKED) org = org + dir * tmin;
							else if (key >= 0) org = org + dir * tmin;
						}
					}
				}
				hitm = ballot64(key >= 0) & actm;
				missm = actm & ~hitm;
				if (SUSPEND) {
					const unsigned long long s0 = ballot64(susp == 1u), s1 = ballot64(susp == 2u);
					sq_count0 += popc64(s0), sq_count1 += popc64(s1);
					missm &= ~(s0 | s1);
					resm = 0ull;
				}
			}
			actm = 0ull;
		}

		SRT_CLK(0);
		if (missm != 0ull) {
			SRT_REGION(SKY_PUSH);
			constexpr uint32_t RC = SRT_RING_CAP;
			const uint32_t n_miss = popc64(missm);
			const uint32_t rank = lane_rank(missm);
			if (ring_count + n_miss > RC) {
				resolve_ring(p, ring, ring_count, lane SRT_RC_ARG);
				ring_count = 0;
// ... 438 lines not shown
				if (in_mask(takem)) {
					item = sj_next + r;
					off = sj_off + r;
					qpix = sj_qpix;
				}
				sj_next += take, sj_off += take;
				given += take;
				w_paths += take;
			}
			const unsigned long long gotm = ballot64(rank < given) & freem;
			actm |= gotm;
			if (FAST) cam_phase = n_act == 0u;
			if (in_mask(gotm)) {
				SRT_REGION(CAMERA);
				const auto &c = SRT_COLD(p);
				static_assert(SUB <= 128u, "off / nbs by the 16-bit reciprocal is exact for off < 256 and nbs < 128 only (tests/csrc/magic_check.cpp)");
				const uint32_t dq = (nbs >= SUB) ? (off >= nbs ? 1u : 0u) : (off * c.nbs_magic16) >> 16;
				const uint32_t q = qpix + dq;
				const uint32_t sample = c.first_sample + (off - dq * nbs);
				const uint32_t lrow = (__umulhi(q, c.width_magic) + q) >> c.width_shift;
				const int px = (int)(q - lrow * (uint32_t)width);
				int py = (int)lrow;
				if (c.world != 1) {
					const uint32_t lb = (__umulhi(lrow, c.rpb_magic) + lrow) >> c.rpb_shift;
					py = (int)((lb * (uint32_t)c.world + (uint32_t)c.rank) * (uint32_t)c.rows_per_block + (lrow - lb * (uint32_t)c.rows_per_block));
				}
				const uint32_t id = (uint32_t)px + (uint32_t)py * (uint32_t)width;
				seed = (sample + id * (uint32_t)ns) * c.rd.time * 5304u;
				float ndc_x = div_by_rcp((float)px + random_float(seed), c.f_width, c.inv_f_width);
				float ndc_y = div_by_rcp((float)py + random_float(seed), c.f_height, c.inv_f_height);
				float sx = ((2.f * ndc_x - 1.f) * c.rd.aspect_ratio) * c.rd.fov_scale;
				float sy = (1.f - 2.f * ndc_y) * c.rd.fov_scale;
				const f3 c0 = mk(c.rd.camera_to_world[0].x, c.rd.camera_to_world[0].y, c.rd.camera_to_world[0].z);
				const f3 c1 = mk(c.rd.camera_to_world[1].x, c.rd.camera_to_world[1].y, c.rd.camera_to_world[1].z);
				const f3 c2 = mk(c.rd.camera_to_world[2].x, c.rd.camera_to_world[2].y, c.rd.camera_to_world[2].z);
				org = mk(c.rd.camera_to_world[3].x, c.rd.camera_to_world[3].y, c.rd.camera_to_world[3].z);
				dir = normalize3(mat_cols_by_vec(c0, c1, c2, org, mk(sx, sy, -1.0f), 0.0f));
				mask = mk(1.f, 1.f, 1.f);
				color = mk(0.f, 0.f, 0.f);
				bounce = 0;
			}
		}

		SRT_CLK(5);
		SRT_REGION(LOOP_TAIL);
		if (queue_dry) {
			if (actm == 0ull && hq_count == 0u && (sq_count0 | sq_count1 | pk_count) == 0u) {
				if (!use_pool || pool_leave || pool_last) break;
				if (++idle_spins > (1u << 20)) {
					if (lane == 0) atomicAdd((unsigned long long *)SRT_COLD(p).counters + SRT_CTR_WATCHDOG, 1ull);
					break;
				}
			} else {
				idle_spins = 0;
			}
		}
	}
	SRT_REGION(EPILOGUE);
	if (ring_count != 0u) resolve_ring(p, ring, ring_count, lane SRT_RC_ARG);

	unsigned long long t3 = COUNT_TRIS ? n_tri : w_scans, t4 = COUNT_TRIS ? n_tri_u : w_scan_lanes;
	if (COUNT_TRIS || SUSPEND) {
		for (int off = 32; off > 0; off >>= 1) {
			t3 += __shfl_down(t3, off);
			t4 += __shfl_down(t4, off);
		}
	}
	if (lane == 0) {
		unsigned long long *__restrict__ w = (unsigned long long *)SRT_COLD(p).wave_counters + (size_t)blockIdx.x * SRT_WAVE_CTR_STRIDE;
		w[0] += w_rays;
		w[1] += w_sky;
		w[2] += w_paths;
		if (COUNT_TRIS) {
			w[3] += t3;
			w[4] += t4;
		} else if (SUSPEND) {
			w[8] += t3;
			w[9] += t4;
#ifndef SRT_PHASE_CLOCK
			w[10] += w_pool_taken, w[11] += w_pool_given, w[12] += (unsigned long long)w_pool_taken * w_pool_taken, w[13] += w_pool_last_taken;
#endif
		}
		if (FAST) w[5] += w_cam;
		w[6] += w_iter;
		w[7] += w_shade;
#ifdef SRT_PHASE_CLOCK
		for (int i = 0; i < 7; i++) w[8 + i] += clk_t[i];
		w[15] += __builtin_amdgcn_s_memtime() - clk_start;
#endif
	}
#ifdef SRT_REGION_COUNT
	__syncthreads();
	{
		unsigned long long *__restrict__ w = (unsigned long long *)SRT_COLD(p).wave_counters + (size_t)blockIdx.x * SRT_WAVE_CTR_STRIDE + 16;
		for (int i = lane; i < 2 * SRT_REGION_MAX; i += 64) w[i] += region_ctr[i];
	}
#endif
```

simple-raytracer_amd/tracer.py:

```python
import ctypes as C
from pathlib import Path

import numpy as np

from . import build as B
from . import records as R

PKG = Path(__file__).resolve().parent
import os

LIB_PATH = Path(os.environ["SRT_LIB"]) if os.environ.get("SRT_LIB") else PKG / "lib" / "libsrt_hip.so"

ABI_SYMBOLS = [
    "srt_create", "srt_destroy", "srt_last_error", "srt_set_skybox", "srt_update_scene", "srt_clear_canvas",
    "srt_render", "srt_render_async", "srt_trace", "srt_set_radiance_budget", "srt_resolve", "srt_resolve_external", "srt_synchronize", "srt_read_canvas", "srt_read_argb",
    "srt_get_counters", "srt_set_count_triangles", "srt_reset_counters", "srt_last_kernel_ms", "srt_set_kernel_timers", "srt_last_trace_kernel_ms", "srt_last_trace_launches",
    "srt_device_buffers", "srt_bind_canvas", "srt_bind_stream", "srt_set_partition",
    "srt_partition_owned_rows", "srt_partition_padded_rows", "srt_partition_global_row",
    "srt_partition_unpermute", "srt_selftest_math", "srt_selftest_rare_lanes", "srt_version", "srt_set_acceleration", "srt_acceleration_info", "srt_bvh_build_host", "srt_bvh_wide_host", "srt_debug_counters", "srt_debug_region_counters",
    "srt_comm_unique_id", "srt_comm_init", "srt_gather", "srt_resolve_gathered", "srt_gathered_buffers", "srt_read_gathered",
    "srt_group_create", "srt_group_destroy", "srt_group_last_error", "srt_group_size", "srt_group_tracer", "srt_group_set_skybox",
    "srt_group_set_acceleration", "srt_group_update_scene", "srt_group_clear_canvas", "srt_group_trace_and_gather", "srt_group_render",
    "srt_group_read_canvas", "srt_group_get_counters", "srt_render_pipelined", "srt_pipeline_flush", "srt_unpermute_device",
    "srt_denoise_defaults", "srt_set_denoise", "srt_resolve_denoised", "srt_read_denoised", "srt_read_denoise_inputs",
    "srt_temporal_defaults", "srt_set_denoise_temporal", "srt_reset_denoise_history", "srt_read_denoise_history",
    "srt_set_denoise_object_motion", "srt_read_denoise_shape_ids", "srt_read_denoise_motion", "srt_motion_table_host",
    "srt_set_denoise_vertex_motion", "srt_read_denoise_triangle_ids", "srt_read_denoise_vertex_tables", "srt_motion_table_deform_host",
    "srt_set_textures", "srt_set_material_textures", "srt_set_triangle_uvs", "srt_last_trace_textured", "srt_plane_frame_host",
    "srt_texture_check_host", "srt_group_set_textures", "srt_group_set_material_textures", "srt_group_set_triangle_uvs",
    "srt_last_trace_class", "srt_bernoulli_threshold_host",
    "srt_set_triangle_materials", "srt_group_set_triangle_materials", "srt_triangle_materials_check_host",
    "srt_group_set_denoise", "srt_group_set_denoise_temporal", "srt_group_reset_denoise_history", "srt_group_resolve_denoised",
    "srt_group_read_denoised", "srt_group_read_denoise_inputs", "srt_group_read_denoise_history", "srt_partition_planes_floats",
    "srt_unpermute_planes_device",
    "srt_set_denoise_demodulation", "srt_group_set_denoise_demodulation", "srt_last_filter_demodulated",
    "srt_group_last_filter_demodulated",
    "srt_set_denoise_spatial_variance", "srt_group_set_denoise_spatial_variance", "srt_last_filter_spatial_variance",
    "srt_group_last_filter_spatial_variance",
    "srt_set_denoise_history_illumination", "srt_group_set_denoise_history_illumination", "srt_last_setup_history_illumination",
    "srt_group_last_setup_history_illumination",
    "srt_set_denoise_history_clamp", "srt_group_set_denoise_history_clamp", "srt_last_setup_history_clamp",
    "srt_group_last_setup_history_clamp", "srt_read_denoise_history_bounds",
    "srt_bvh_refit_wide_host", "srt_set_acceleration_refit", "srt_group_set_acceleration_refit", "srt_acceleration_refit_info",
    "srt_last_refit_kernel_ms", "srt_read_bvh_blocks", "srt_bvh_wide_order_host",
    "srt_set_acceleration_deform", "srt_group_set_acceleration_deform", "srt_acceleration_deform_info",
    "srt_bvh_refit_deformed_wide_host", "srt_bvh_wide_cost_host",
    "srt_set_acceleration_build", "srt_group_set_acceleration_build", "srt_acceleration_build_info", "srt_last_build_kernel_ms",
    "srt_bvh_morton_order_host", "srt_bvh_morton_wide_host",
    "srt_set_acceleration_build_order", "srt_group_set_acceleration_build_order", "srt_bvh_median_order_host", "srt_bvh_median_wide_host",
]

ACCEL_NONE, ACCEL_BVH = 0, 1
REFIT_HOST, REFIT_DEVICE = 0, 1
DEFORM_REBUILD, DEFORM_REFIT = 0, 1
BUILD_HOST, BUILD_DEVICE = 0, 1
BUILD_ORDER_MORTON, BUILD_ORDER_MEDIAN = 0, 1
BUILD_LOCAL = 1024
MOTION_STATIC, MOTION_MOVED, MOTION_NO_HISTORY, MOTION_DEFORMED = 0, 1, 2, 3
MOTION_WORDS = 22
NO_SHAPE = 0xFFFFFFFF
FILTER_LINEAR, FILTER_NEAREST = 0, 1
MAX_TEXTURES = 64


class TextureDesc(C.Structure):
    _fields_ = [("rgba", C.c_void_p), ("width", C.c_int32), ("height", C.c_int32)]


def _texture_descs(images):
    keep = [np.ascontiguousarray(im, np.float32) for im in images]
    for im in keep:
        assert im.ndim == 3 and im.shape[2] == 4
    descs = (TextureDesc * max(len(keep), 1))()
    for k, im in enumerate(keep):
        descs[k].rgba, descs[k].width, descs[k].height = im.ctypes.data, im.shape[1], im.shape[0]
    return keep, descs


def _uv_array(uv):
    if uv is None:
        return None, 0
    uv = np.ascontiguousarray(uv, np.float32).reshape(-1, 3, 2)
    return uv, len(uv)


def _tm_array(tm):
    if tm is None:
        return None
    tm = np.ascontiguousarray(tm, np.int32).reshape(-1)
    return tm if len(tm) else None


def triangle_materials_check_host(materials, scene_triangles, n_materials):
    lib = load_library()
    tm = None if materials is None else np.ascontiguousarray(materials, np.int32).reshape(-1)
    return lib.srt_triangle_materials_check_host(_ptr(tm) if tm is not None else None, 0 if tm is None else len(tm), int(scene_triangles), int(n_materials))


def plane_frame_host(normal):
    lib = load_library()
    n = np.ascontiguousarray(normal, np.float32).reshape(3)
    T, B = np.zeros(3, np.float32), np.zeros(3, np.float32)
    return (T, B) if lib.srt_plane_frame_host(_ptr(n), _ptr(T), _ptr(B)) else None


def bernoulli_threshold_host(p):
    out = C.c_uint64(0)
    if load_library().srt_bernoulli_threshold_host(C.c_float(float(np.float32(p))), C.byref(out)):
        raise SrtError("srt_bernoulli_threshold_host failed")
    return int(out.value)


def texture_check_host(n_textures, bindings=None, uv_triangles=None, scene_triangles=0, images=None):
    lib = load_library()
    descs, keep = None, None
    if images is not None:
        keep = np.zeros(4, np.float32)
        descs = (TextureDesc * max(len(images), 1))()
        for k, (has_texels, w, h) in enumerate(images):
            descs[k].rgba, descs[k].width, descs[k].height = (keep.ctypes.data if has_texels else None), w, h
    b = R.as_records(bindings if bindings is not None else [], R.MATERIAL_TEXTURE)
    return lib.srt_texture_check_host(descs, n_textures, _ptr(b) if len(b) else None, len(b),
                                      -1 if uv_triangles is None else int(uv_triangles), scene_triangles)


def _motion_rows(table):
    table = np.ascontiguousarray(table, np.uint32).reshape(-1, MOTION_WORDS)
    f = table[:, 1:].copy().view(np.float32)
    return {"state": table[:, 0].astype(np.int64), "A": f[:, :12].reshape(-1, 3, 4), "B": f[:, 12:].reshape(-1, 3, 3)}


def motion_table_host(history, current, deform=False):
    lib = load_library()
    args, keep = [], []
    for shapes, triangles, materials, sd in (history, current):
        recs = [R.as_records(shapes, R.SHAPE), R.as_records(triangles, R.TRIANGLE), R.as_records(materials, R.MATERIAL)]
        sd = R.as_records(sd, R.SCENE_DATA)
        keep += recs + [sd]
        for r in recs:
            args += [_ptr(r) if len(r) else None, len(r)]
        args.append(_ptr(sd))
    n = len(keep[4])
    table = np.zeros((max(n, 1), MOTION_WORDS), np.uint32)
    kept = C.c_int(0)
    fn = lib.srt_motion_table_deform_host if deform else lib.srt_motion_table_host
    rc = fn(*args, _ptr(table), C.byref(kept))
    if rc:
        raise SrtError(f"srt_motion_table_host failed ({rc})")
    if not kept.value:
        return None
    out = _motion_rows(table[:n])
    if deform:
        out["first_row"] = table[:n, 1].astype(np.int64)
    return out


BVH_NODE = np.dtype({"names": ["lo", "skip", "hi", "leaf"], "formats": [(np.float32, (3,)), np.uint32, (np.float32, (3,)), np.uint32],
                     "offsets": [0, 12, 16, 28], "itemsize": 32})
BVH_END = 0xFFFFFFFF


def bvh_build_host(model_shape, triangles):
    lib = load_library()
    shape = np.zeros(1, R.SHAPE)
    shape[0] = model_shape
    tris = R.as_records(triangles, R.TRIANGLE)
    n = C.c_size_t(0)
    rc = lib.srt_bvh_build_host(_ptr(shape), _ptr(tris), len(tris), None, 0, None, 0, C.byref(n))
    if rc:
        raise SrtError(f"srt_bvh_build_host failed ({rc})")
    nodes = np.zeros(n.value, BVH_NODE)
    order = np.zeros(int(shape[0]["num_triangles"]), np.uint32)
    rc = lib.srt_bvh_build_host(_ptr(shape), _ptr(tris), len(tris), _ptr(nodes), len(nodes), _ptr(order), len(order), C.byref(n))
    if rc:
        raise SrtError(f"srt_bvh_build_host failed ({rc})")
    return nodes, order


BVH_NONE = 0xFFFFFFFF
BVH_LEAF_BIT = 0x80000000
BVH_INDEX_MASK = 0x0FFFFFFF
BVH_STACK_CAP = 64


def bvh_wide_host(model_shape, triangles, force_balanced=False):
    lib = load_library()
# ... 276 lines not shown
        lib.srt_group_last_error.restype = C.c_char_p
        lib.srt_group_size.argtypes = [vp]
        lib.srt_group_tracer.argtypes = [vp, i]
        lib.srt_group_tracer.restype = vp
        lib.srt_group_set_skybox.argtypes = [vp, vp, i, i]
        lib.srt_group_set_acceleration.argtypes = [vp, i]
        lib.srt_group_update_scene.argtypes = [vp, vp, sz, vp, sz, vp, sz, vp]
        lib.srt_group_clear_canvas.argtypes = [vp]
        lib.srt_group_trace_and_gather.argtypes = [vp, vp]
        lib.srt_group_render.argtypes = [vp, vp, C.c_uint32, vp]
        lib.srt_group_read_canvas.argtypes = [vp, vp]
        lib.srt_group_get_counters.argtypes = [vp, C.POINTER(Counters)]
        if hasattr(lib, "srt_group_set_denoise"):
            lib.srt_group_set_denoise.argtypes = [vp, C.POINTER(DenoiseParams)]
            lib.srt_group_set_denoise_temporal.argtypes = [vp, C.POINTER(TemporalParams)]
            lib.srt_group_reset_denoise_history.argtypes = [vp]
            lib.srt_group_resolve_denoised.argtypes = [vp, C.c_uint32]
            lib.srt_group_read_denoised.argtypes = [vp, vp]
            lib.srt_group_read_denoise_inputs.argtypes = [vp, vp, vp, vp, C.POINTER(C.c_uint32)]
            lib.srt_group_read_denoise_history.argtypes = [vp, vp, vp, vp, vp, C.POINTER(C.c_int)]
            lib.srt_partition_planes_floats.argtypes = [i, i, i, i]
            lib.srt_partition_planes_floats.restype = C.c_longlong
            lib.srt_unpermute_planes_device.argtypes = [vp, vp, vp, vp, vp, i, i, i, i]
        lib.srt_render_pipelined.argtypes = [vp, vp, C.c_uint32, vp, C.POINTER(C.c_longlong)]
        lib.srt_pipeline_flush.argtypes = [vp, vp, C.POINTER(C.c_longlong)]
    if hasattr(lib, "srt_set_denoise"):
        lib.srt_denoise_defaults.argtypes = [C.POINTER(DenoiseParams)]
        lib.srt_set_denoise.argtypes = [vp, C.POINTER(DenoiseParams)]
        lib.srt_resolve_denoised.argtypes = [vp, C.c_uint32]
        lib.srt_read_denoised.argtypes = [vp, vp]
        lib.srt_read_denoise_inputs.argtypes = [vp, vp, vp, vp, C.POINTER(C.c_uint32)]
    if hasattr(lib, "srt_set_denoise_temporal"):
        lib.srt_temporal_defaults.argtypes = [C.POINTER(TemporalParams)]
        lib.srt_set_denoise_temporal.argtypes = [vp, C.POINTER(TemporalParams)]
        lib.srt_reset_denoise_history.argtypes = [vp]
        lib.srt_read_denoise_history.argtypes = [vp, vp, vp, vp, vp, C.POINTER(C.c_int)]
    if hasattr(lib, "srt_set_denoise_object_motion"):
        lib.srt_set_denoise_object_motion.argtypes = [vp, C.c_int]
        lib.srt_read_denoise_shape_ids.argtypes = [vp, vp, vp]
        lib.srt_read_denoise_motion.argtypes = [vp, vp, sz, C.POINTER(sz), C.POINTER(C.c_int)]
        lib.srt_motion_table_host.argtypes = [vp, sz, vp, sz, vp, sz, vp] * 2 + [vp, C.POINTER(C.c_int)]
    if hasattr(lib, "srt_set_denoise_vertex_motion"):
        lib.srt_set_denoise_vertex_motion.argtypes = [vp, C.c_int]
        lib.srt_read_denoise_triangle_ids.argtypes = [vp, vp, vp]
        lib.srt_read_denoise_vertex_tables.argtypes = [vp, vp, vp, sz, C.POINTER(sz)]
        lib.srt_motion_table_deform_host.argtypes = [vp, sz, vp, sz, vp, sz, vp] * 2 + [vp, C.POINTER(C.c_int)]
    if hasattr(lib, "srt_set_denoise_demodulation"):
        lib.srt_set_denoise_demodulation.argtypes = [vp, C.c_int]
        lib.srt_group_set_denoise_demodulation.argtypes = [vp, C.c_int]
        lib.srt_last_filter_demodulated.argtypes = [vp, C.POINTER(C.c_int)]
        lib.srt_group_last_filter_demodulated.argtypes = [vp, C.POINTER(C.c_int)]
    if hasattr(lib, "srt_set_denoise_spatial_variance"):
        lib.srt_set_denoise_spatial_variance.argtypes = [vp, C.c_uint32]
        lib.srt_group_set_denoise_spatial_variance.argtypes = [vp, C.c_uint32]
        lib.srt_last_filter_spatial_variance.argtypes = [vp, C.POINTER(C.c_int)]
        lib.srt_group_last_filter_spatial_variance.argtypes = [vp, C.POINTER(C.c_int)]
    if hasattr(lib, "srt_set_denoise_history_illumination"):
        lib.srt_set_denoise_history_illumination.argtypes = [vp, C.c_int]
        lib.srt_group_set_denoise_history_illumination.argtypes = [vp, C.c_int]
        lib.srt_last_setup_history_illumination.argtypes = [vp]
        lib.srt_group_last_setup_history_illumination.argtypes = [vp]
    if hasattr(lib, "srt_set_denoise_history_clamp"):
        lib.srt_set_denoise_history_clamp.argtypes = [vp, C.c_float]
        lib.srt_group_set_denoise_history_clamp.argtypes = [vp, C.c_float]
        lib.srt_last_setup_history_clamp.argtypes = [vp]
        lib.srt_group_last_setup_history_clamp.argtypes = [vp]
        lib.srt_read_denoise_history_bounds.argtypes = [vp, vp, vp]
    if hasattr(lib, "srt_set_textures"):
        lib.srt_set_textures.argtypes = [vp, vp, sz]
        lib.srt_set_material_textures.argtypes = [vp, vp, sz]
        lib.srt_set_triangle_uvs.argtypes = [vp, vp, sz]
        lib.srt_last_trace_textured.argtypes = [vp, C.POINTER(C.c_int)]
        lib.srt_plane_frame_host.argtypes = [vp, vp, vp]
        lib.srt_texture_check_host.argtypes = [vp, sz, vp, sz, C.c_longlong, sz]
        lib.srt_group_set_textures.argtypes = [vp, vp, sz]
        lib.srt_group_set_material_textures.argtypes = [vp, vp, sz]
        lib.srt_group_set_triangle_uvs.argtypes = [vp, vp, sz]
    if hasattr(lib, "srt_set_triangle_materials"):
        lib.srt_set_triangle_materials.argtypes = [vp, vp, sz]
        lib.srt_group_set_triangle_materials.argtypes = [vp, vp, sz]
        lib.srt_triangle_materials_check_host.argtypes = [vp, sz, sz, sz]
    if hasattr(lib, "srt_last_trace_class"):
        lib.srt_last_trace_class.argtypes = [vp, C.POINTER(C.c_int)]
    if hasattr(lib, "srt_bernoulli_threshold_host"):
        lib.srt_bernoulli_threshold_host.argtypes = [C.c_float, C.POINTER(C.c_uint64)]
    return lib


def _ptr(a):
    return a.ctypes.data_as(C.c_void_p)


class _Denoise:

    def set_denoise(self, enable=True, **kw):
        if not enable:
            self._check(self._dn("set_denoise", None))
            return
        d = DenoiseParams()
        self._check(self.lib.srt_denoise_defaults(C.byref(d)))
        for k, v in kw.items():
            if k not in d.as_dict() or k == "enable":
                raise TypeError(f"set_denoise: unknown parameter {k}")
            setattr(d, k, v)
        self._check(self._dn("set_denoise", C.byref(d)))

    def resolve_denoised(self, ticks_stopped):
        self._check(self._dn("resolve_denoised", ticks_stopped))

    def read_denoised(self):
        out = np.zeros((self.height, self.width, 4), np.float32)
        self._check(self._dn("read_denoised", _ptr(out)))
        return out

    def read_denoise_inputs(self):
        nd = np.zeros((self.height, self.width, 4), np.float32)
        ah = np.zeros((self.height, self.width, 4), np.float32)
        m = np.zeros((self.height, self.width), np.float32)
        counts = (C.c_uint32 * 2)()
        self._check(self._dn("read_denoise_inputs", _ptr(nd), _ptr(ah), _ptr(m), counts))
        return {"normal_depth": nd, "albedo_hits": ah, "moments": m, "T": int(counts[0]), "P": int(counts[1])}

    def set_denoise_temporal(self, enable=True, **kw):
        if not enable:
            self._check(self._dn("set_denoise_temporal", None))
            return
        d = TemporalParams()
        self._check(self.lib.srt_temporal_defaults(C.byref(d)))
        for k, v in kw.items():
            if k not in ("history_limit", "normal_threshold", "depth_threshold"):
                raise TypeError(f"set_denoise_temporal: unknown parameter {k}")
            setattr(d, k, v)
        self._check(self._dn("set_denoise_temporal", C.byref(d)))

    def set_denoise_demodulation(self, enable=True):
        self._check(self._dn("set_denoise_demodulation", 1 if enable else 0))

    def last_filter_demodulated(self):
        out = C.c_int(0)
        self._check(self._dn("last_filter_demodulated", C.byref(out)))
        return bool(out.value)

    def set_denoise_spatial_variance(self, min_samples=8):
        self._check(self._dn("set_denoise_spatial_variance", int(min_samples)))

    def last_filter_spatial_variance(self):
        out = C.c_int(0)
        self._check(self._dn("last_filter_spatial_variance", C.byref(out)))
        return bool(out.value)

    def set_denoise_history_illumination(self, enable=True):
        self._check(self._dn("set_denoise_history_illumination", 1 if enable else 0))

    def last_setup_history_illumination(self):
        return bool(self._dn("last_setup_history_illumination"))

    def set_denoise_history_clamp(self, gamma=1.0):
        self._check(self._dn("set_denoise_history_clamp", float(gamma)))

    def last_setup_history_clamp(self):
        return bool(self._dn("last_setup_history_clamp"))

    def reset_denoise_history(self):
        self._check(self._dn("reset_denoise_history"))

    def read_denoise_history(self):
        cc = np.zeros((self.height, self.width, 4), np.float32)
        m = np.zeros((self.height, self.width, 2), np.float32)
        g = np.zeros((self.height, self.width, 2, 4), np.float32)
        cam = np.zeros((), R.RENDER_DATA)
        valid = C.c_int(0)
        self._check(self._dn("read_denoise_history", _ptr(cc), _ptr(m), _ptr(g), _ptr(cam), C.byref(valid)))
        return {"valid": bool(valid.value), "colour": cc[..., :3], "count": cc[..., 3], "m1": m[..., 0], "m2": m[..., 1], "guide": g,
                "camera": cam}


class Tracer(_Denoise):

    def __init__(self, width, height, device=0, lib=None):
        self.lib = lib if lib is not None else load_library()
        self._h = C.c_void_p()
        rc = self.lib.srt_create(width, height, device, C.byref(self._h))
        if rc:
            raise SrtError(self.lib.srt_last_error(None).decode())
        self.width, self.height = width, height
        self.options = R.render_data(width, height, num_samples=4, num_bounces=10)
        self.scene_data = R.scene_data(0)
        self.owned_rows = height

    def _check(self, rc):
        if rc:
            e = SrtError(self.lib.srt_last_error(self._h).decode())
            e.code = rc
            raise e

    def close(self):
        if getattr(self, "_h", None) is not None and self._h.value:
            self.lib.srt_destroy(self._h)
            self._h = C.c_void_p()

    def __del__(self):
        try:
            self.close()
        except Exception:
            pass

    def set_skybox(self, rgba):
        rgba = np.ascontiguousarray(rgba, np.float32)
        assert rgba.ndim == 3 and rgba.shape[2] == 4
        self._check(self.lib.srt_set_skybox(self._h, _ptr(rgba), rgba.shape[1], rgba.shape[0]))

    def set_textures(self, images):
        keep, descs = _texture_descs(images)
        self._check(self.lib.srt_set_textures(self._h, descs if keep else None, len(keep)))

    def set_material_textures(self, bindings):
        b = R.as_records(bindings if bindings is not None else [], R.MATERIAL_TEXTURE)
        self._check(self.lib.srt_set_material_textures(self._h, _ptr(b) if len(b) else None, len(b)))

    def set_triangle_uvs(self, uv):
        uv, n = _uv_array(uv)
        self._check(self.lib.srt_set_triangle_uvs(self._h, _ptr(uv) if uv is not None else None, n))

    def set_triangle_materials(self, materials):
        tm = _tm_array(materials)
        self._check(self.lib.srt_set_triangle_materials(self._h, _ptr(tm) if tm is not None else None, 0 if tm is None else len(tm)))

    def last_trace_textured(self):
        out = C.c_int(0)
        self._check(self.lib.srt_last_trace_textured(self._h, C.byref(out)))
        return bool(out.value)

    def last_trace_class(self):
        out = C.c_int(0)
        self._check(self.lib.srt_last_trace_class(self._h, C.byref(out)))
        return out.value

    def update_scene(self, shapes, triangles, materials):
        shapes = R.as_records(shapes, R.SHAPE)
        triangles = R.as_records(triangles, R.TRIANGLE)
        materials = R.as_records(materials, R.MATERIAL)
        sd = R.as_records(self.scene_data, R.SCENE_DATA)
        self._check(self.lib.srt_update_scene(self._h, _ptr(shapes), len(shapes), _ptr(triangles), len(triangles),
                                              _ptr(materials), len(materials), _ptr(sd)))
        self.scene_data["num_shapes"] = len(shapes)

    def clear_canvas(self):
        self._check(self.lib.srt_clear_canvas(self._h))

    def render(self, ticks_stopped, output=None):
        if output is None:
            output = np.zeros(self.owned_rows * self.width * 4, np.uint8)
        assert output.dtype == np.uint8 and output.size >= self.owned_rows * self.width * 4
        rd = R.as_records(self.options, R.RENDER_DATA)
        self._check(self.lib.srt_render(self._h, _ptr(rd), ticks_stopped, _ptr(output)))
        return output

    def render_async(self, ticks_stopped, output):
        assert output.dtype == np.uint8 and output.size >= self.owned_rows * self.width * 4
        rd = R.as_records(self.options, R.RENDER_DATA)
        self._check(self.lib.srt_render_async(self._h, _ptr(rd), ticks_stopped, _ptr(output)))

    def trace(self):
        rd = R.as_records(self.options, R.RENDER_DATA)
        self._check(self.lib.srt_trace(self._h, _ptr(rd)))

    def set_radiance_budget(self, nbytes):
        self._check(self.lib.srt_set_radiance_budget(self._h, nbytes))

    def resolve(self, ticks_stopped):
        self._check(self.lib.srt_resolve(self._h, ticks_stopped))

    def resolve_external(self, canvas_ptr, num_pixels, ticks_stopped, argb_ptr):
        self._check(self.lib.srt_resolve_external(self._h, C.c_void_p(canvas_ptr), num_pixels, ticks_stopped, C.c_void_p(argb_ptr)))

    def synchronize(self):
        self._check(self.lib.srt_synchronize(self._h))

    def read_canvas(self):
        out = np.zeros((self.owned_rows, self.width, 4), np.float32)
        self._check(self.lib.srt_read_canvas(self._h, _ptr(out)))
        return out

    def read_argb(self):
        out = np.zeros((self.owned_rows, self.width, 4), np.uint8)
        self._check(self.lib.srt_read_argb(self._h, _ptr(out)))
        return out

    def counters(self):
        c = Counters()
        self._check(self.lib.srt_get_counters(self._h, C.byref(c)))
        return c.as_dict()

    def debug_counters(self):
        out = (C.c_uint64 * 18)()
        self.lib.srt_debug_counters.argtypes = [C.c_void_p, C.POINTER(C.c_uint64)]
        self._check(self.lib.srt_debug_counters(self._h, out))
        v = [int(x) for x in out]
        return {"rays": v[0], "sky": v[1], "paths": v[2], "orphans": 0, "evictions": 0,
                "camera_phases": v[5] >> 36, "camera_phase_rays": v[5] & ((1 << 36) - 1),
                "iterations": v[6], "shade_phases": v[7], "waves_per_cu": v[8], "grid": v[9],
                "phase_cycles": dict(zip(("extend", "ring", "shade", "park", "deliver", "refill", "head", "kernel"), v[10:18])),
                "scans": v[10], "scan_lanes": v[11],
                "pool_taken": v[12], "pool_given": v[13], "pool_taken_sq": v[14], "pool_last_taken": v[15]}

    def debug_region_counters(self):
        out = (C.c_uint64 * 128)()
        n = C.c_int(0)
        self.lib.srt_debug_region_counters.argtypes = [C.c_void_p, C.POINTER(C.c_uint64), C.c_int, C.POINTER(C.c_int)]
        self._check(self.lib.srt_debug_region_counters(self._h, out, 128, C.byref(n)))
        return [(int(out[2 * i]), int(out[2 * i + 1])) for i in range(n.value // 2)]

    def reset_counters(self):
        self._check(self.lib.srt_reset_counters(self._h))

    def count_triangles(self, enable=True):
        self._check(self.lib.srt_set_count_triangles(self._h, 1 if enable else 0))

    def set_acceleration(self, mode):
        self._check(self.lib.srt_set_acceleration(self._h, int(mode)))

    def acceleration_info(self):
        out = (C.c_uint64 * 7)()
        self._check(self.lib.srt_acceleration_info(self._h, out))
        return dict(zip(("nodes", "leaves", "depth", "build_us", "models_built", "models_reused", "models_refitted"), (int(v) for v in out)))

    def set_acceleration_refit(self, mode):
        self._check(self.lib.srt_set_acceleration_refit(self._h, int(mode)))

    def set_acceleration_deform(self, mode, rebuild_ratio=0.0):
        self._check(self.lib.srt_set_acceleration_deform(self._h, int(mode), float(rebuild_ratio)))

    def acceleration_deform_info(self):
        out, worst = (C.c_uint64 * 4)(), C.c_double(0)
        self._check(self.lib.srt_acceleration_deform_info(self._h, out, C.byref(worst)))
        return {"models_kept": int(out[0]), "models_rebuilt": int(out[1]), "cost_launches": int(out[2]), "worst_ratio": worst.value}

    def set_acceleration_build(self, mode, min_triangles=0):
        self._check(self.lib.srt_set_acceleration_build(self._h, int(mode), int(min_triangles)))

    def set_acceleration_build_order(self, order):
        self._check(self.lib.srt_set_acceleration_build_order(self._h, int(order)))

    def acceleration_build_info(self):
        out = (C.c_uint64 * 4)()
        self._check(self.lib.srt_acceleration_build_info(self._h, out))
        return dict(zip(("models", "records", "launches"), (int(v) for v in out)))

    def last_build_kernel_ms(self):
        a = C.c_float()
        self._check(self.lib.srt_last_build_kernel_ms(self._h, C.byref(a)))
        return a.value

    def acceleration_refit_info(self):
        out = (C.c_uint64 * 4)()
        self._check(self.lib.srt_acceleration_refit_info(self._h, out))
        return dict(zip(("models", "inner_blocks", "launches"), (int(v) for v in out)))

    def last_refit_kernel_ms(self):
        a = C.c_float()
        self._check(self.lib.srt_last_refit_kernel_ms(self._h, C.byref(a)))
        return a.value

    def read_bvh_blocks(self):
        n = C.c_size_t(0)
        self._check(self.lib.srt_read_bvh_blocks(self._h, None, 0, C.byref(n)))
        blocks = np.zeros((n.value, 32), np.uint32)
        self._check(self.lib.srt_read_bvh_blocks(self._h, _ptr(blocks), len(blocks), C.byref(n)))
        return blocks

    def selftest_math(self, stride=1):
        out = (C.c_uint64 * 16)()
        self._check(self.lib.srt_selftest_math(self._h, stride, out))
        return [int(v) for v in out]

    def selftest_rare_lanes(self, what, words):
        words = np.ascontiguousarray(words, np.uint32)
        assert words.ndim == 2 and words.shape[1] == 8 and words.shape[0] % 64 == 0
        new, ref, bad = np.zeros((words.shape[0], 4), np.uint32), np.zeros((words.shape[0], 4), np.uint32), C.c_uint64()
        u32p = C.POINTER(C.c_uint32)
        self._check(self.lib.srt_selftest_rare_lanes(self._h, int(what), words.ctypes.data_as(u32p), words.shape[0] // 64,
                                                     new.ctypes.data_as(u32p), ref.ctypes.data_as(u32p), C.byref(bad)))
        return new, ref, int(bad.value)

    def set_kernel_timers(self, enable=True):
        self._check(self.lib.srt_set_kernel_timers(self._h, int(bool(enable))))

    def last_kernel_ms(self):
        a, b = C.c_float(), C.c_float()
        self._check(self.lib.srt_last_kernel_ms(self._h, C.byref(a), C.byref(b)))
        return a.value, b.value

    def last_trace_launches(self):
        n, o = C.c_int(0), C.c_int(0)
        self.lib.srt_last_trace_launches.argtypes = [C.c_void_p, C.POINTER(C.c_int), C.POINTER(C.c_int)]
        self._check(self.lib.srt_last_trace_launches(self._h, C.byref(n), C.byref(o)))
        return n.value, bool(o.value)

    def last_trace_kernel_ms(self):
        a = C.c_float()
        self._check(self.lib.srt_last_trace_kernel_ms(self._h, C.byref(a)))
        return a.value

    def device_buffers(self):
        cp, cb, ap, ab = C.c_void_p(), C.c_size_t(), C.c_void_p(), C.c_size_t()
        self._check(self.lib.srt_device_buffers(self._h, C.byref(cp), C.byref(cb), C.byref(ap), C.byref(ab)))
        return cp.value, cb.value, ap.value, ab.value

    def bind_canvas(self, device_ptr, nbytes):
        self._check(self.lib.srt_bind_canvas(self._h, C.c_void_p(device_ptr), nbytes))

    def bind_stream(self, hip_stream):
        self._check(self.lib.srt_bind_stream(self._h, C.c_void_p(hip_stream)))

    @staticmethod
    def comm_unique_id():
        buf = C.create_string_buffer(128)
        if load_library().srt_comm_unique_id(buf):
            raise SrtError(load_library().srt_last_error(None).decode())
        return buf.raw

    def comm_init(self, unique_id, rank, world):
        self._check(self.lib.srt_comm_init(self._h, C.c_char_p(unique_id), rank, world))

    def gather(self, root=0):
        self._check(self.lib.srt_gather(self._h, root))

    def resolve_gathered(self, ticks_stopped):
        self._check(self.lib.srt_resolve_gathered(self._h, ticks_stopped))

    def gathered_buffers(self):
        cp, ap = C.c_void_p(), C.c_void_p()
        self._check(self.lib.srt_gathered_buffers(self._h, C.byref(cp), C.byref(ap)))
        return cp.value, ap.value

    def read_gathered(self, canvas=True, argb=False):
        c = np.zeros((self.height, self.width, 4), np.float32) if canvas else None
        a = np.zeros((self.height, self.width, 4), np.uint8) if argb else None
        self._check(self.lib.srt_read_gathered(self._h, _ptr(c) if canvas else None, _ptr(a) if argb else None))
        return c, a

    def render_pipelined(self, ticks_stopped, output):
        assert output.dtype == np.uint8 and output.size >= self.owned_rows * self.width * 4
        rd = R.as_records(self.options, R.RENDER_DATA)
        n = C.c_longlong(-1)
        self._check(self.lib.srt_render_pipelined(self._h, _ptr(rd), ticks_stopped, _ptr(output), C.byref(n)))
        return n.value

    def pipeline_flush(self, output):
        n = C.c_longlong(-1)
        self._check(self.lib.srt_pipeline_flush(self._h, _ptr(output), C.byref(n)))
        return n.value

    def _dn(self, name, *args):
        return getattr(self.lib, "srt_" + name)(self._h, *args)

    def set_denoise_object_motion(self, enable=True):
        self._check(self.lib.srt_set_denoise_object_motion(self._h, 1 if enable else 0))

    def read_denoise_history_bounds(self):
        b0 = np.zeros((self.height, self.width, 4), np.float32)
        b1 = np.zeros((self.height, self.width, 4), np.float32)
        self._check(self.lib.srt_read_denoise_history_bounds(self._h, _ptr(b0), _ptr(b1)))
        return {"mu": b0[..., :3], "weight": b0[..., 3], "sigma": b1[..., :3], "taps": b1[..., 3]}

    def read_denoise_shape_ids(self):
# ... 172 lines not shown
```

Baseline: 95070 Mray/s.

## Add axis-aligned plane kernel variants with short-form division intersection

Detects at scene prep when every plane in a one-group scene is axis-aligned (unit normal along x, y or z) and dispatches a specialised kernel twin keyed by the plane axes. For those planes, the ray-plane t reduces to (p_axis - org_axis) / dir_axis, which skips the dot products. Camera-phase numerators are precomputed in LDS, and the division uses a refined-reciprocal short division. A wave-wide operand range check guards exactness for the bit-identical parity mode and falls back to the general path when the check fails. The cost is extra kernel instantiations, per-phase ballots and counters, and the risk that the short division does not match IEEE division.

```diff
diff --git a/include/srt_abi.h b/include/srt_abi.h
--- a/include/srt_abi.h
+++ b/include/srt_abi.h
@@ -248,6 +248,8 @@
 int srt_triangle_materials_check_host(const int32_t *materials, size_t n, size_t scene_triangles, size_t n_materials);
 int srt_last_trace_textured(const srt_tracer *t, int *textured);
 int srt_last_trace_class(const srt_tracer *t, int *scene_class);
+int srt_last_trace_plane_form(const srt_tracer *t, int *plane_form);
+int srt_plane_axis_code_host(const float normal[3], const float position[3], int *code);
 int srt_bernoulli_threshold_host(float p, uint64_t *threshold);
 int srt_plane_frame_host(const float normal[3], float T[3], float B[3]);
 int srt_texture_check_host(const srt_texture_desc *descs, size_t n_textures, const srt_material_texture *bindings, size_t n_bindings,
@@ -257,6 +259,9 @@
 
 int srt_selftest_rare_lanes(srt_tracer *t, int what, const uint32_t *in, uint32_t waves, uint32_t *out_new, uint32_t *out_ref, uint64_t *mismatches);
 
+int srt_selftest_plane_forms(srt_tracer *t, int what, const float planes[32], const float cam_org[3], const uint32_t *in, uint32_t waves,
+                             uint32_t *out_new, uint32_t *out_ref, uint32_t *fast, uint64_t *mismatches);
+
 const char *srt_version(void);
 
 #ifdef __cplusplus
diff --git a/simple-raytracer_amd/csrc/device_intersect.h b/simple-raytracer_amd/csrc/device_intersect.h
--- a/simple-raytracer_amd/csrc/device_intersect.h
+++ b/simple-raytracer_amd/csrc/device_intersect.h
@@ -146,6 +146,60 @@
 		if (lane < 2) {
 			const float4 pq = blk[2 * lane], nq = blk[2 * lane + 1];
 			reinterpret_cast<float *>(blk + 2 * lane)[3] = dot3(mk(nq.x, nq.y, nq.z), mk(pq.x - org.x, pq.y - org.y, pq.z - org.z));
+		}
+	}
+}
+#ifndef SRT_AXIS_SHORT_DIV
+#define SRT_AXIS_SHORT_DIV 1
+#endif
+template <int C>
+__device__ __forceinline__ float f3_at(f3 v) { return C == 0 ? v.x : C == 1 ? v.y : v.z; }
+template <uint32_t K, uint32_t AX>
+__device__ __forceinline__ void axis_numerators(const float *__restrict__ blk, f3 org, float *__restrict__ a) {
+	if constexpr ((K & 3u) == SRT_SHAPE_PLANE + 1u) {
+		constexpr int C0 = (int)(AX & 3u) - 1, C1 = (int)((AX >> 2) & 3u) - 1;
+		a[0] = blk[C0 < 0 ? 0 : C0] - f3_at<C0>(org);
+		if constexpr (((K >> 2) & 7u) > 1u) a[1] = blk[8 + (C1 < 0 ? 0 : C1)] - f3_at<C1>(org);
+	}
+}
+template <int N>
+__device__ __forceinline__ bool axis_operands_ok(const float *__restrict__ a, f3 dir) {
+	float mn = dm_fabs(a[0]), sm = dm_fabs(a[0]);
+#pragma unroll
+	for (int i = 1; i < N; i++) mn = __builtin_fminf(mn, dm_fabs(a[i])), sm = sm + dm_fabs(a[i]);
+	const float bx = dm_fabs(dir.x), by = dm_fabs(dir.y), bz = dm_fabs(dir.z);
+	const float mnb = __builtin_fminf(__builtin_fminf(bx, by), bz), smb = (bx + by) + bz;
+	return mn >= 0x1p-60f && sm <= 0x1p50f && mnb >= 0x1p-40f && smb <= 0x1p40f;
+}
+__device__ __forceinline__ float axis_div(float a, float b) {
+#if SRT_AXIS_SHORT_DIV
+	return div_core(a, b, rcp_refined(b));
+#else
+	return a / b;
+#endif
+}
+template <uint32_t AX>
+__device__ __forceinline__ void test_planes2_axis(const float *__restrict__ a, uint32_t count, f3 dir, int idx0, float &tmin, int &best) {
+#pragma unroll
+	for (int i = 0; i < 2; i++) {
+		if (i == 1 && count < 2u) break;
+		const float b = i == 0 ? f3_at<(int)(AX & 3u) - 1>(dir) : f3_at<(int)((AX >> 2) & 3u) - 1>(dir);
+		const float t = axis_div(a[i], b);
+		const bool hit = !(t < 0.0f);
+		if (hit && t < tmin) {
+			tmin = t;
+			best = idx0 + i;
+		}
+	}
+}
+template <uint32_t K, uint32_t AX>
+__device__ __forceinline__ void cam_axis_numerators(float4 *__restrict__ blk, f3 org, int lane) {
+	if constexpr ((K & 3u) == SRT_SHAPE_PLANE + 1u) {
+		if (lane < 2) {
+			const float4 pq = blk[2 * lane];
+			const int c = (int)((AX >> (2 * lane)) & 3u) - 1;
+			const float pk = c == 0 ? pq.x : c == 1 ? pq.y : pq.z, ok = c == 0 ? org.x : c == 1 ? org.y : org.z;
+			reinterpret_cast<float *>(blk + 2 * lane + 1)[3] = pk - ok;
 		}
 	}
 }
diff --git a/simple-raytracer_amd/csrc/device_types.h b/simple-raytracer_amd/csrc/device_types.h
--- a/simple-raytracer_amd/csrc/device_types.h
+++ b/simple-raytracer_amd/csrc/device_types.h
@@ -70,6 +70,26 @@
 	X(3, SRT_GC_SSS, true)      \
 	X(4, SRT_GC_PPP, true)
 #define SRT_SCENE_CLASS_GENERAL 0
+#define SRT_AXES_PPS_YXZ (2u | (1u << 2) | (3u << 4))
+#define SRT_SCENE_AXIS_LIST(X)               \
+	X(1, SRT_GC_PPS, true, SRT_AXES_PPS_YXZ) \
+	X(2, SRT_GC_PPS, false, SRT_AXES_PPS_YXZ)
+static constexpr inline bool srt_axes_buildable(uint32_t code, uint32_t axes) {
+	uint32_t used = 0, planes = 0;
+	for (uint32_t b = 0; b < 3; b++) {
+		const uint32_t k = (code >> (8 * b)) & 255u, n = (k >> 2) & 7u;
+		for (uint32_t i = 0; i < 2; i++) {
+			const uint32_t a = (axes >> (4 * b + 2 * i)) & 3u;
+			const bool plane = (k & 3u) == SRT_SHAPE_PLANE + 1u && i < n;
+			if (plane != (a != 0u)) return false;
+			if (plane) used |= 1u << a, planes++;
+		}
+	}
+	return planes != 0u && used == 14u && (axes >> 12) == 0u;
+}
+static constexpr inline int32_t srt_kernel_key(int scene_class, uint32_t plane_form) { return (int32_t)((uint32_t)scene_class | (plane_form << 8)); }
+static constexpr inline int srt_key_class(int32_t key) { return (int)((uint32_t)key & 255u); }
+static constexpr inline uint32_t srt_key_plane_form(int32_t key) { return (uint32_t)key >> 8; }
 static constexpr inline uint32_t srt_class_cam_records(uint32_t code) {
 	return ((code & 3u) == SRT_SHAPE_SPHERE + 1u ? 4u : 0u) + (((code >> 8) & 3u) == SRT_SHAPE_SPHERE + 1u ? 4u : 0u) +
 	       (((code >> 16) & 3u) == SRT_SHAPE_SPHERE + 1u ? 4u : 0u);
@@ -288,5 +308,7 @@
 void srt_launch_resolve(const ResolveParams &p, void *stream);
 void srt_launch_selftest(unsigned long long *out16, uint32_t stride, void *stream);
 void srt_launch_selftest_rare(int what, const uint32_t *in, uint32_t waves, uint32_t *out_new, uint32_t *out_ref, unsigned long long *mismatches, void *stream);
+void srt_launch_selftest_plane_forms(int what, const float *planes32, const float *cam_org3, const uint32_t *in, uint32_t waves, uint32_t *out_new, uint32_t *out_ref,
+                                     uint32_t *fast, unsigned long long *mismatches, void *stream);
 
 #endif
diff --git a/simple-raytracer_amd/csrc/kernels.hip b/simple-raytracer_amd/csrc/kernels.hip
--- a/simple-raytracer_amd/csrc/kernels.hip
+++ b/simple-raytracer_amd/csrc/kernels.hip
@@ -118,12 +118,13 @@
 
 struct GeneralScene {
 	static constexpr bool FAST = false, NO_SPEC = false;
-	static constexpr uint32_t CODE = 0;
+	static constexpr uint32_t CODE = 0, AXES = 0;
 };
-template <uint32_t CODE_, bool NO_SPEC_>
+template <uint32_t CODE_, bool NO_SPEC_, uint32_t AXES_ = 0>
 struct OneGroupScene {
 	static constexpr bool FAST = true, NO_SPEC = NO_SPEC_;
-	static constexpr uint32_t CODE = CODE_;
+	static constexpr uint32_t CODE = CODE_, AXES = AXES_;
+	static_assert(AXES_ == 0 || srt_axes_buildable(CODE_, AXES_), "an axis twin needs an axis for every plane, and all three axes in use");
 };
 template <uint32_t K>
 __device__ __forceinline__ void test_block_of_class(const Blk16 &b, int base, f3 org, f3 dir, float &tmin, int &best) {
@@ -144,6 +145,36 @@
 	}
 }
 
+__device__ __forceinline__ Blk16 ld_blk16_lds(const float4 *__restrict__ blk) {
+	Blk16 b;
+	const float4 q0 = blk[0], q1 = blk[1], q2 = blk[2], q3 = blk[3];
+	b.v[0] = q0.x, b.v[1] = q0.y, b.v[2] = q0.z, b.v[3] = q0.w, b.v[4] = q1.x, b.v[5] = q1.y, b.v[6] = q1.z, b.v[7] = q1.w;
+	b.v[8] = q2.x, b.v[9] = q2.y, b.v[10] = q2.z, b.v[11] = q2.w, b.v[12] = q3.x, b.v[13] = q3.y, b.v[14] = q3.z, b.v[15] = q3.w;
+	return b;
+}
+template <uint32_t K, uint32_t AX>
+__device__ __forceinline__ void test_block_of_class_axis(const float4 *__restrict__ blk, bool pass, const float *__restrict__ a, int base, f3 org, f3 dir, float &tmin, int &best) {
+	if constexpr ((K & 3u) == SRT_SHAPE_PLANE + 1u) {
+		if (__builtin_expect(pass, 1)) test_planes2_axis<AX>(a, (K >> 2) & 7u, dir, base, tmin, best);
+		else test_planes2(ld_blk16_lds(blk), (K >> 2) & 7u, org, dir, base, tmin, best);
+	} else {
+		test_block_of_class<K>(ld_blk16_lds(blk), base, org, dir, tmin, best);
+	}
+}
+template <uint32_t K, uint32_t AX>
+__device__ __forceinline__ void test_block_of_class_axis_cam(const float4 *__restrict__ blk, const float4 *__restrict__ cam, bool pass, int base, f3 dir, unsigned long long actm, float &tmin, int &best) {
+	if constexpr ((K & 3u) == SRT_SHAPE_PLANE + 1u) {
+		if (__builtin_expect(pass, 1)) {
+			const float a[2] = {reinterpret_cast<const float *>(blk + 1)[3], reinterpret_cast<const float *>(blk + 3)[3]};
+			test_planes2_axis<AX>(a, (K >> 2) & 7u, dir, base, tmin, best);
+		} else {
+			test_planes2_cam(blk, (K >> 2) & 7u, dir, base, tmin, best);
+		}
+	} else {
+		test_block_of_class_cam<K>(blk, cam, base, dir, actm, tmin, best);
+	}
+}
+
 template <bool COUNT_TRIS, bool USE_LDS, bool HAS_MODELS, bool USE_BVH>
 __global__ __launch_bounds__(64, USE_BVH ? SRT_TRACE_WAVES_PER_SIMD_BVH : HAS_MODELS ? SRT_TRACE_WAVES_PER_SIMD_MODELS : SRT_TRACE_WAVES_PER_SIMD) void srt_trace_kernel(const SRT_TRACE_PARAMS p) {
 	using SC = GeneralScene;
@@ -152,10 +183,10 @@
 
 #if !SRT_TEXTURED && !SRT_DIAG_ON && !defined(SRT_DUMMY_KIND) && !defined(SRT_DEV_KNOBS) && SRT_RING_CAP == 64
 #define SRT_SCENE_CLASSES 1
-template <uint32_t CODE, bool NO_SPEC>
+template <uint32_t CODE, bool NO_SPEC, uint32_t PLANE_FORM>
 __global__ __launch_bounds__(64, 6) void srt_trace_scene_kernel(const TraceParams p) {
 	constexpr bool COUNT_TRIS = false, USE_LDS = true, HAS_MODELS = false, USE_BVH = false;
-	using SC = OneGroupScene<CODE, NO_SPEC>;
+	using SC = OneGroupScene<CODE, NO_SPEC, PLANE_FORM>;
 #include "trace_body.inc"
 }
 #else
@@ -218,9 +249,13 @@
 #if SRT_SCENE_CLASSES
 	switch (p.scene_class) {
 #define SRT_SCENE_CLASS_CASE(number, code, no_spec) \
-	case number: return srt_trace_scene_kernel<code, no_spec>;
+	case number: return srt_trace_scene_kernel<code, no_spec, 0u>;
 		SRT_SCENE_CLASS_LIST(SRT_SCENE_CLASS_CASE)
 #undef SRT_SCENE_CLASS_CASE
+#define SRT_SCENE_AXIS_CASE(number, code, no_spec, axes) \
+	case srt_kernel_key(number, axes): return srt_trace_scene_kernel<code, no_spec, axes>;
+		SRT_SCENE_AXIS_LIST(SRT_SCENE_AXIS_CASE)
+#undef SRT_SCENE_AXIS_CASE
 	default: break;
 	}
 #endif
@@ -229,7 +264,7 @@
 size_t trace_lds_bytes(const SRT_TRACE_PARAMS &p, size_t scene_lds) {
 	size_t need = scene_lds + (size_t)srt_trace_lds_floats(p.num_models > 0, p.use_bvh) * sizeof(float);
 #if SRT_SCENE_CLASSES
-	switch (p.scene_class) {
+	switch (srt_key_class(p.scene_class)) {
 #define SRT_SCENE_CLASS_CASE(number, code, no_spec) \
 	case number: need += srt_class_cam_lds_bytes(code); break;
 		SRT_SCENE_CLASS_LIST(SRT_SCENE_CLASS_CASE)
diff --git a/simple-raytracer_amd/csrc/scene_prep.cpp b/simple-raytracer_amd/csrc/scene_prep.cpp
--- a/simple-raytracer_amd/csrc/scene_prep.cpp
+++ b/simple-raytracer_amd/csrc/scene_prep.cpp
@@ -17,6 +17,17 @@
 		else hi = mid;
 	}
 	return lo;
+}
+
+int srt_plane_axis_code(const float n[3], const float p[3]) {
+	int axis = 0;
+	for (int k = 0; k < 3; k++) {
+		if (!(fabsf(p[k]) <= 0x1p100f)) return 0;
+		if (n[k] == 0.0f) continue;
+		if (fabsf(n[k]) != 1.0f || axis != 0) return 0;
+		axis = k + 1;
+	}
+	return axis;
 }
 
 int prepare_scene(const AccelPolicy &policy, BvhCache *&cache, int scan_suspend_min, std::string &err, ScenePrep &sp, const srt_shape *shapes, size_t n_shapes,
@@ -272,6 +283,14 @@
 		for (size_t b = 0; b < runs.size(); b++) packed = packed && runs[b].first_shape == next, next += runs[b].count;
 		if (packed && next == n_shapes) sp.one_group_code = groups[0].code;
 	}
+	sp.plane_axes = 0;
+	if (sp.one_group_code != 0)
+		for (size_t b = 0; b < runs.size(); b++)
+			for (uint32_t i = 0; runs[b].type == SRT_SHAPE_PLANE && i < runs[b].count; i++) {
+				const srt_plane &pl = shapes[runs[b].first_shape + i].shape.plane;
+				const float n[3] = {pl.normal.x, pl.normal.y, pl.normal.z}, q[3] = {pl.position.x, pl.position.y, pl.position.z};
+				sp.plane_axes |= (uint32_t)srt_plane_axis_code(n, q) << (4 * b + 2 * i);
+			}
 	if (!stale_plan.empty()) {
 		size_t top = 0;
 		for (const auto &st : stale_plan) top = std::max(top, st.first->wide.level_off.size());
@@ -337,6 +356,12 @@
 	return SRT_OK;
 }
 
+extern "C" int srt_plane_axis_code_host(const float normal[3], const float position[3], int *code_out) {
+	if (!normal || !position || !code_out) return SRT_ERR_INVALID;
+	*code_out = srt_plane_axis_code(normal, position);
+	return SRT_OK;
+}
+
 extern "C" int srt_bernoulli_threshold_host(float p, uint64_t *threshold_out) {
 	if (!threshold_out) return SRT_ERR_INVALID;
 	*threshold_out = bernoulli_threshold(p);
diff --git a/simple-raytracer_amd/csrc/scene_prep.h b/simple-raytracer_amd/csrc/scene_prep.h
--- a/simple-raytracer_amd/csrc/scene_prep.h
+++ b/simple-raytracer_amd/csrc/scene_prep.h
@@ -17,6 +17,7 @@
 	bool use_bvh = false, unit_materials = false, all_materials_ok = true;
 	int material_flags = 0;
 	uint32_t one_group_code = 0;
+	uint32_t plane_axes = 0;
 	uint64_t bvh_info[7] = {0, 0, 0, 0, 0, 0, 0};
 	std::vector<RefitModel> refit_models;
 	std::vector<uint32_t> refit_extents, refit_sched, refit_levels;
@@ -56,5 +57,6 @@
                   const srt_triangle *triangles, size_t n_triangles, const srt_material *materials, size_t n_materials, const srt_scene_data *scene);
 
 uint64_t bernoulli_threshold(float pr);
+int srt_plane_axis_code(const float normal[3], const float position[3]);
 
 #endif
diff --git a/simple-raytracer_amd/csrc/selftest.hip b/simple-raytracer_amd/csrc/selftest.hip
--- a/simple-raytracer_amd/csrc/selftest.hip
+++ b/simple-raytracer_amd/csrc/selftest.hip
@@ -1,6 +1,7 @@
 #include <hip/hip_runtime.h>
 
 #include "device_math.h"
+#include "device_intersect.h"
 #include "device_shading.h"
 
 namespace {
@@ -131,3 +132,49 @@
 	if (waves == 0) return;
 	hipLaunchKernelGGL(srt_selftest_rare_kernel, dim3(waves), dim3(64), 0, (hipStream_t)stream, what, in, out_new, out_ref, mismatches);
 }
+
+struct PlaneFormsArgs {
+	float blk[32];
+	float cam_org[3];
+};
+__global__ __launch_bounds__(64) void srt_selftest_plane_forms_kernel(int what, const PlaneFormsArgs pl, const uint32_t *__restrict__ in, uint32_t *__restrict__ out_new,
+                                                                      uint32_t *__restrict__ out_ref, uint32_t *__restrict__ fast, unsigned long long *mismatches) {
+	constexpr uint32_t K0 = SRT_BLK_CODE(SRT_SHAPE_PLANE, 2), K1 = SRT_BLK_CODE(SRT_SHAPE_PLANE, 1);
+	constexpr uint32_t A0 = SRT_AXES_PPS_YXZ & 15u, A1 = (SRT_AXES_PPS_YXZ >> 4) & 15u;
+	const size_t lane = (size_t)blockIdx.x * 64u + threadIdx.x;
+	const uint32_t *__restrict__ w = in + lane * 8u;
+	const f3 org = what == 1 ? mk(pl.cam_org[0], pl.cam_org[1], pl.cam_org[2]) : mk(dm_u2f(w[0]), dm_u2f(w[1]), dm_u2f(w[2]));
+	const f3 dir = mk(dm_u2f(w[3]), dm_u2f(w[4]), dm_u2f(w[5]));
+	Blk16 b0, b1;
+#pragma unroll
+	for (int i = 0; i < 16; i++) b0.v[i] = pl.blk[i], b1.v[i] = pl.blk[16 + i];
+	float tmin_r = dm_u2f(w[6]), tmin_n = tmin_r;
+	int best_r = -1, best_n = -1;
+	test_planes2(b0, 2u, org, dir, 0, tmin_r, best_r);
+	test_planes2(b1, 1u, org, dir, 2, tmin_r, best_r);
+	float an[3];
+	axis_numerators<K0, A0>(b0.v, org, an);
+	axis_numerators<K1, A1>(b1.v, org, an + 2);
+	const bool pass = !any64(!axis_operands_ok<3>(an, dir));
+	if (pass) {
+		test_planes2_axis<A0>(an, 2u, dir, 0, tmin_n, best_n);
+		test_planes2_axis<A1>(an + 2, 1u, dir, 2, tmin_n, best_n);
+	} else {
+		test_planes2(b0, 2u, org, dir, 0, tmin_n, best_n);
+		test_planes2(b1, 1u, org, dir, 2, tmin_n, best_n);
+	}
+	out_new[lane * 2u] = dm_f2u(tmin_n), out_new[lane * 2u + 1u] = (uint32_t)best_n;
+	out_ref[lane * 2u] = dm_f2u(tmin_r), out_ref[lane * 2u + 1u] = (uint32_t)best_r;
+	if (threadIdx.x == 0) fast[blockIdx.x] = pass ? 1u : 0u;
+	const unsigned long long bad = (dm_f2u(tmin_n) != dm_f2u(tmin_r) ? 1u : 0u) + (best_n != best_r ? 1u : 0u);
+	if (bad) atomicAdd(mismatches, bad);
+}
+
+void srt_launch_selftest_plane_forms(int what, const float *planes32, const float *cam_org3, const uint32_t *in, uint32_t waves, uint32_t *out_new, uint32_t *out_ref,
+                                     uint32_t *fast, unsigned long long *mismatches, void *stream) {
+	if (waves == 0) return;
+	PlaneFormsArgs pl;
+	for (int i = 0; i < 32; i++) pl.blk[i] = planes32[i];
+	for (int i = 0; i < 3; i++) pl.cam_org[i] = cam_org3[i];
+	hipLaunchKernelGGL(srt_selftest_plane_forms_kernel, dim3(waves), dim3(64), 0, (hipStream_t)stream, what, pl, in, out_new, out_ref, fast, mismatches);
+}
diff --git a/simple-raytracer_amd/csrc/srt_abi.hip b/simple-raytracer_amd/csrc/srt_abi.hip
--- a/simple-raytracer_amd/csrc/srt_abi.hip
+++ b/simple-raytracer_amd/csrc/srt_abi.hip
@@ -350,6 +350,7 @@
 	t->unit_materials = sp.unit_materials;
 	t->material_flags = sp.material_flags;
 	t->one_group_code = sp.one_group_code;
+	t->plane_axes = sp.plane_axes;
 	t->num_runs = (int)sp.groups.size();
 	t->num_materials = n_materials;
 	t->scene_set = true;
@@ -426,9 +427,23 @@
 	return SRT_SCENE_CLASS_GENERAL;
 }
 
+static uint32_t plane_form_of(const srt_tracer *t, int scene_class) {
+#define SRT_SCENE_AXIS_MATCH(number, code, class_no_spec, axes) \
+	if (scene_class == number && t->plane_axes == (axes)) return axes;
+	SRT_SCENE_AXIS_LIST(SRT_SCENE_AXIS_MATCH)
+#undef SRT_SCENE_AXIS_MATCH
+	return 0u;
+}
+
 int srt_last_trace_class(const srt_tracer *t, int *scene_class_out) {
 	if (!t || !scene_class_out) return SRT_ERR_INVALID;
 	*scene_class_out = t->last_trace_class;
+	return SRT_OK;
+}
+
+int srt_last_trace_plane_form(const srt_tracer *t, int *plane_form_out) {
+	if (!t || !plane_form_out) return SRT_ERR_INVALID;
+	*plane_form_out = (int)t->last_trace_plane_form;
 	return SRT_OK;
 }
 
@@ -492,7 +507,10 @@
 	p.all_materials_ok = t->scene_set && t->all_materials_ok ? 1 : 0;
 	p.unit_materials = t->scene_set && t->unit_materials ? 1 : 0;
 	p.material_flags = t->scene_set ? t->material_flags : 0;
-	p.scene_class = scene_class(t, options, textured);
+	{
+		const int sc = scene_class(t, options, textured);
+		p.scene_class = srt_kernel_key(sc, plane_form_of(t, sc));
+	}
 	p.f_sky_w = (float)t->sky_w;
 	p.f_sky_h = (float)t->sky_h;
 	p.sun_focus_int = dm_pow_small_int(p.sd.sun_focus);
@@ -697,7 +715,8 @@
 	d.ns = options->num_samples;
 	d.fused_argb = fused_argb;
 	TraceParams p = trace_params_of(t, options, d.textured);
-	t->last_trace_class = p.scene_class;
+	t->last_trace_class = srt_key_class(p.scene_class);
+	t->last_trace_plane_form = srt_key_plane_form(p.scene_class);
 	if (const int rc = reserve_radiance(t, d)) return rc;
 	d.slots = wave_slots(t, p, d.textured);
 	if (const int rc = reserve_scan_stacks(t, d)) return rc;
@@ -990,6 +1009,35 @@
 	return SRT_OK;
 }
 
+int srt_selftest_plane_forms(srt_tracer *t, int what, const float planes[32], const float cam_org[3], const uint32_t *in, uint32_t waves, uint32_t *out_new,
+                             uint32_t *out_ref, uint32_t *fast, uint64_t *mismatches) {
+	if (!t) return SRT_ERR_INVALID;
+	if (!planes || !cam_org || !in || !out_new || !out_ref || !fast || !mismatches || what < 0 || what > 1 || waves == 0 || waves > 65536u)
+		return fail(t, SRT_ERR_INVALID, "srt_selftest_plane_forms: bad arguments");
+	SRT_HIP(t, hipSetDevice(t->device));
+	const size_t lanes = (size_t)waves * 64u, in_bytes = lanes * 8u * sizeof(uint32_t), out_bytes = lanes * 2u * sizeof(uint32_t), fast_bytes = (size_t)waves * sizeof(uint32_t);
+	char *d = nullptr;
+	SRT_HIP(t, hipMalloc(reinterpret_cast<void **>(&d), in_bytes + 2 * out_bytes + sizeof(unsigned long long) + fast_bytes));
+	uint32_t *d_in = reinterpret_cast<uint32_t *>(d), *d_new = reinterpret_cast<uint32_t *>(d + in_bytes), *d_ref = reinterpret_cast<uint32_t *>(d + in_bytes + out_bytes);
+	unsigned long long *d_bad = reinterpret_cast<unsigned long long *>(d + in_bytes + 2 * out_bytes), h_bad = 0;
+	uint32_t *d_fast = reinterpret_cast<uint32_t *>(d + in_bytes + 2 * out_bytes + sizeof(unsigned long long));
+	hipError_t e = hipMemcpyAsync(d_in, in, in_bytes, hipMemcpyHostToDevice, t->stream);
+	if (e == hipSuccess) e = hipMemsetAsync(d_new, 0, 2 * out_bytes + sizeof(unsigned long long) + fast_bytes, t->stream);
+	if (e == hipSuccess) {
+		srt_launch_selftest_plane_forms(what, planes, cam_org, d_in, waves, d_new, d_ref, d_fast, d_bad, t->stream);
+		e = hipGetLastError();
+	}
+	if (e == hipSuccess) e = hipMemcpyAsync(out_new, d_new, out_bytes, hipMemcpyDeviceToHost, t->stream);
+	if (e == hipSuccess) e = hipMemcpyAsync(out_ref, d_ref, out_bytes, hipMemcpyDeviceToHost, t->stream);
+	if (e == hipSuccess) e = hipMemcpyAsync(fast, d_fast, fast_bytes, hipMemcpyDeviceToHost, t->stream);
+	if (e == hipSuccess) e = hipMemcpyAsync(&h_bad, d_bad, sizeof h_bad, hipMemcpyDeviceToHost, t->stream);
+	if (e == hipSuccess) e = hipStreamSynchronize(t->stream);
+	(void)hipFree(d);
+	if (e != hipSuccess) return fail(t, SRT_ERR_HIP, std::string("srt_selftest_plane_forms: ") + hipGetErrorString(e));
+	*mismatches = h_bad;
+	return SRT_OK;
+}
+
 int srt_debug_counters(srt_tracer *t, uint64_t out[18]) {
 	if (!t || !out) return SRT_ERR_INVALID;
 	SRT_HIP(t, hipSetDevice(t->device));
diff --git a/simple-raytracer_amd/csrc/srt_internal.h b/simple-raytracer_amd/csrc/srt_internal.h
--- a/simple-raytracer_amd/csrc/srt_internal.h
+++ b/simple-raytracer_amd/csrc/srt_internal.h
@@ -172,6 +172,7 @@
 	bool unit_materials = false;
 	int material_flags = 0;
 	uint32_t one_group_code = 0;
+	uint32_t plane_axes = 0;
 	uint64_t scan_tris = 0;
 	bool scene_set = false;
 	bool count_tris = false;
@@ -241,6 +242,7 @@
 	bool tex_active = false;
 	bool last_trace_textured = false;
 	int last_trace_class = 0;
+	uint32_t last_trace_plane_form = 0;
 	hipEvent_t ev_t0 = nullptr, ev_t1 = nullptr, ev_r0 = nullptr, ev_r1 = nullptr;
 	bool have_trace_ev = false, have_resolve_ev = false, have_kernel_ev = false;
 	std::string err;
diff --git a/simple-raytracer_amd/csrc/trace_body.inc b/simple-raytracer_amd/csrc/trace_body.inc
--- a/simple-raytracer_amd/csrc/trace_body.inc
+++ b/simple-raytracer_amd/csrc/trace_body.inc
@@ -3,6 +3,7 @@
 	static_assert(!FAST || (USE_LDS && !HAS_MODELS && !USE_BVH && !COUNT_TRIS), "scene classes exist for sphere / plane scenes staged in LDS");
 	constexpr uint32_t FK0 = SC::CODE & 255u, FK1 = (SC::CODE >> 8) & 255u, FK2 = (SC::CODE >> 16) & 255u;
 	constexpr int FN0 = (int)((FK0 >> 2) & 7u), FN1 = (int)((FK1 >> 2) & 7u), FN2 = (int)((FK2 >> 2) & 7u), FN = FN0 + FN1 + FN2;
+	constexpr uint32_t AXES = SC::AXES, FA0 = AXES & 15u, FA1 = (AXES >> 4) & 15u, FA2 = (AXES >> 8) & 15u;
 	constexpr uint32_t SUB = USE_BVH ? SRT_SUB_BVH : HAS_MODELS ? SRT_SUB_MODELS : SRT_SUB_PLAIN;
 	const int width = p.rd.width;
 	const int lane = threadIdx.x;
@@ -69,7 +70,27 @@
 		cam_records_of_block<FK0>(lds + 2 * FN, cam_rec, cam_org, lane);
 		cam_records_of_block<FK1>(lds + 2 * FN + 4, cam_rec + CS1, cam_org, lane);
 		cam_records_of_block<FK2>(lds + 2 * FN + 8, cam_rec + CS2, cam_org, lane);
+		if constexpr (AXES != 0u) {
+			cam_axis_numerators<FK0, FA0>(lds + 2 * FN, cam_org, lane);
+			cam_axis_numerators<FK1, FA1>(lds + 2 * FN + 4, cam_org, lane);
+			cam_axis_numerators<FK2, FA2>(lds + 2 * FN + 8, cam_org, lane);
+		}
 		__syncthreads();
+	}
+	bool cam_nums_ok = false;
+	uint32_t w_axis_phases = 0, w_axis_failed = 0;
+	if constexpr (AXES != 0u) {
+		const float4 *__restrict__ lb = lds + 2 * FN;
+		float mn = DM_INF_F, sm = 0.0f;
+#pragma unroll
+		for (int b = 0; b < 3; b++)
+#pragma unroll
+			for (int i = 0; i < 2; i++)
+				if (((AXES >> (4 * b + 2 * i)) & 3u) != 0u) {
+					const float a = dm_fabs(reinterpret_cast<const float *>(lb + 4 * b + 2 * i + 1)[3]);
+					mn = __builtin_fminf(mn, a), sm = sm + a;
+				}
+		cam_nums_ok = !any64(!(mn >= 0x1p-60f && sm <= 0x1p50f));
 	}
 	bool cam_phase = false;
 	unsigned long long w_cam = 0;
@@ -224,7 +245,31 @@
 							b.v[8] = q2.x, b.v[9] = q2.y, b.v[10] = q2.z, b.v[11] = q2.w, b.v[12] = q3.x, b.v[13] = q3.y, b.v[14] = q3.z, b.v[15] = q3.w;
 							return b;
 						};
-						if (cam_phase) {
+						if constexpr (AXES != 0u) {
+							constexpr int NP0 = (FK0 & 3u) == SRT_SHAPE_PLANE + 1u ? FN0 : 0, NP1 = (FK1 & 3u) == SRT_SHAPE_PLANE + 1u ? FN1 : 0;
+							constexpr int NP2 = (FK2 & 3u) == SRT_SHAPE_PLANE + 1u ? FN2 : 0, NP = NP0 + NP1 + NP2;
+							w_axis_phases++;
+							if (cam_phase) {
+								w_cam += (1ull << 36) + popc64(actm);
+								const float one[1] = {1.0f};
+								const bool pass = cam_nums_ok && (ballot64(!axis_operands_ok<1>(one, dir)) & actm) == 0ull;
+								w_axis_failed += pass ? 0u : 1u;
+								test_block_of_class_axis_cam<FK0, FA0>(lb, cam_rec, pass, 0, dir, actm, tmin, best);
+								if (FK1 != 0u) test_block_of_class_axis_cam<FK1, FA1>(lb + 4, cam_rec + CS1, pass, FN0, dir, actm, tmin, best);
+								if (FK2 != 0u) test_block_of_class_axis_cam<FK2, FA2>(lb + 8, cam_rec + CS2, pass, FN0 + FN1, dir, actm, tmin, best);
+							} else {
+								const float *__restrict__ lbf = reinterpret_cast<const float *>(lb);
+								float an[NP > 0 ? NP : 1];
+								axis_numerators<FK0, FA0>(lbf, org, an);
+								axis_numerators<FK1, FA1>(lbf + 16, org, an + NP0);
+								axis_numerators<FK2, FA2>(lbf + 32, org, an + NP0 + NP1);
+								const bool pass = (ballot64(!axis_operands_ok<NP>(an, dir)) & actm) == 0ull;
+								w_axis_failed += pass ? 0u : 1u;
+								test_block_of_class_axis<FK0, FA0>(lb, pass, an, 0, org, dir, tmin, best);
+								if (FK1 != 0u) test_block_of_class_axis<FK1, FA1>(lb + 4, pass, an + NP0, FN0, org, dir, tmin, best);
+								if (FK2 != 0u) test_block_of_class_axis<FK2, FA2>(lb + 8, pass, an + NP0 + NP1, FN0 + FN1, org, dir, tmin, best);
+							}
+						} else if (cam_phase) {
 							w_cam += (1ull << 36) + popc64(actm);
 							test_block_of_class_cam<FK0>(lb, cam_rec, 0, dir, actm, tmin, best);
 							if (FK1 != 0u) test_block_of_class_cam<FK1>(lb + 4, cam_rec + CS1, FN0, dir, actm, tmin, best);
@@ -829,6 +874,7 @@
 #endif
 		}
 		if (FAST) w[5] += w_cam;
+		if constexpr (AXES != 0u) w[8] += w_axis_phases, w[9] += w_axis_failed;
 		w[6] += w_iter;
 		w[7] += w_shade;
 #ifdef SRT_PHASE_CLOCK
diff --git a/simple-raytracer_amd/tracer.py b/simple-raytracer_amd/tracer.py
--- a/simple-raytracer_amd/tracer.py
+++ b/simple-raytracer_amd/tracer.py
@@ -29,6 +29,7 @@
     "srt_set_textures", "srt_set_material_textures", "srt_set_triangle_uvs", "srt_last_trace_textured", "srt_plane_frame_host",
     "srt_texture_check_host", "srt_group_set_textures", "srt_group_set_material_textures", "srt_group_set_triangle_uvs",
     "srt_last_trace_class", "srt_bernoulli_threshold_host",
+    "srt_last_trace_plane_form", "srt_plane_axis_code_host", "srt_selftest_plane_forms",
     "srt_set_triangle_materials", "srt_group_set_triangle_materials", "srt_triangle_materials_check_host",
     "srt_group_set_denoise", "srt_group_set_denoise_temporal", "srt_group_reset_denoise_history", "srt_group_resolve_denoised",
     "srt_group_read_denoised", "srt_group_read_denoise_inputs", "srt_group_read_denoise_history", "srt_partition_planes_floats",
@@ -102,6 +103,15 @@
     n = np.ascontiguousarray(normal, np.float32).reshape(3)
     T, B = np.zeros(3, np.float32), np.zeros(3, np.float32)
     return (T, B) if lib.srt_plane_frame_host(_ptr(n), _ptr(T), _ptr(B)) else None
+
+
+def plane_axis_code_host(normal, position=(0.0, 0.0, 0.0)):
+    n = np.ascontiguousarray(normal, np.float32).reshape(3)
+    q = np.ascontiguousarray(position, np.float32).reshape(3)
+    out = C.c_int(-1)
+    if load_library().srt_plane_axis_code_host(_ptr(n), _ptr(q), C.byref(out)):
+        raise SrtError("srt_plane_axis_code_host failed")
+    return int(out.value)
 
 
 def bernoulli_threshold_host(p):
@@ -544,6 +554,11 @@
         lib.srt_triangle_materials_check_host.argtypes = [vp, sz, sz, sz]
     if hasattr(lib, "srt_last_trace_class"):
         lib.srt_last_trace_class.argtypes = [vp, C.POINTER(C.c_int)]
+    if hasattr(lib, "srt_last_trace_plane_form"):
+        lib.srt_last_trace_plane_form.argtypes = [vp, C.POINTER(C.c_int)]
+        lib.srt_plane_axis_code_host.argtypes = [vp, vp, C.POINTER(C.c_int)]
+        u32p = C.POINTER(C.c_uint32)
+        lib.srt_selftest_plane_forms.argtypes = [vp, i, vp, vp, u32p, C.c_uint32, u32p, u32p, u32p, C.POINTER(C.c_uint64)]
     if hasattr(lib, "srt_bernoulli_threshold_host"):
         lib.srt_bernoulli_threshold_host.argtypes = [C.c_float, C.POINTER(C.c_uint64)]
     return lib
@@ -693,6 +708,11 @@
         self._check(self.lib.srt_last_trace_textured(self._h, C.byref(out)))
         return bool(out.value)
 
+    def last_trace_plane_form(self):
+        out = C.c_int(-1)
+        self._check(self.lib.srt_last_trace_plane_form(self._h, C.byref(out)))
+        return int(out.value)
+
     def last_trace_class(self):
         out = C.c_int(0)
         self._check(self.lib.srt_last_trace_class(self._h, C.byref(out)))
@@ -764,6 +784,7 @@
                 "iterations": v[6], "shade_phases": v[7], "waves_per_cu": v[8], "grid": v[9],
                 "phase_cycles": dict(zip(("extend", "ring", "shade", "park", "deliver", "refill", "head", "kernel"), v[10:18])),
                 "scans": v[10], "scan_lanes": v[11],
+                "axis_phases": v[10], "axis_failed": v[11],
                 "pool_taken": v[12], "pool_given": v[13], "pool_taken_sq": v[14], "pool_last_taken": v[15]}
 
     def debug_region_counters(self):
@@ -844,6 +865,19 @@
         self._check(self.lib.srt_selftest_rare_lanes(self._h, int(what), words.ctypes.data_as(u32p), words.shape[0] // 64,
                                                      new.ctypes.data_as(u32p), ref.ctypes.data_as(u32p), C.byref(bad)))
         return new, ref, int(bad.value)
+
+    def selftest_plane_forms(self, what, planes, cam_org, words):
+        words = np.ascontiguousarray(words, np.uint32)
+        planes = np.ascontiguousarray(planes, np.float32).reshape(32)
+        cam_org = np.ascontiguousarray(cam_org, np.float32).reshape(3)
+        assert words.ndim == 2 and words.shape[1] == 8 and words.shape[0] % 64 == 0
+        waves = words.shape[0] // 64
+        new, ref = np.zeros((words.shape[0], 2), np.uint32), np.zeros((words.shape[0], 2), np.uint32)
+        fast, bad = np.zeros(waves, np.uint32), C.c_uint64()
+        u32p = C.POINTER(C.c_uint32)
+        self._check(self.lib.srt_selftest_plane_forms(self._h, int(what), _ptr(planes), _ptr(cam_org), words.ctypes.data_as(u32p), waves,
+                                                      new.ctypes.data_as(u32p), ref.ctypes.data_as(u32p), fast.ctypes.data_as(u32p), C.byref(bad)))
+        return new, ref, fast, int(bad.value)
 
     def set_kernel_timers(self, enable=True):
         self._check(self.lib.srt_set_kernel_timers(self._h, int(bool(enable))))
```

Result: faster. 98610 Mray/s (median of 6 runs) (+3.7%).
